# MarioCalvarro/circom_cvm

Measured on AMD Instinct MI355X. Metric: constraints simplified/sec (--O2) on 10M-constraint circuit; bit-exact .r1cs, higher is better.
Workload: dtype u64x4 (F_p, 256-bit Montgomery)

## Files before the change

### circom_cvm_amd/csrc/engine.hip

```cpp
#include <hip/hip_runtime.h>

#include <algorithm>
#include <atomic>
#include <chrono>
#include <condition_variable>
#include <cstdio>
#include <deque>
#include <mutex>
#include <map>
#include <memory>
#include <stdexcept>
#include <thread>
#include <string>
#include <unordered_map>
#include <unordered_set>
#include <functional>
#include <vector>

#include <cstring>
#include <fcntl.h>
#include <pthread.h>
#include <sched.h>
#include <unistd.h>
#include <rocprim/device/device_radix_sort.hpp>
// ... 120 lines not shown
static void launch(hipStream_t st, K kernel, uint64_t n, Args... args) {
  uint64_t blocks = (n + 255) / 256;
  if (blocks == 0) blocks = 1;
  if (blocks > 16384) blocks = 16384;
  hipLaunchKernelGGL(kernel, dim3((unsigned)blocks), dim3(256), 0, st, args...);
  HC(hipGetLastError());
}

struct KGroup {
  std::vector<hipEvent_t> ev;
  size_t n = 0;
  uint64_t bytes = 0;
  void mark(hipStream_t s) {
    if (n == ev.size()) {
      hipEvent_t e;
      HC(hipEventCreate(&e));
      ev.push_back(e);
    }
    HC(hipEventRecord(ev[n++], s));
  }
  template <class F>
  void run(hipStream_t s, uint64_t b, F &&f) {
    mark(s);
    f();
    mark(s);
    bytes += b;
  }
  void collect(double &ms, uint64_t &by, uint64_t &launches) {
    double t = 0;
    for (size_t i = 0; i + 1 < n; i += 2) {
      float m = 0;
      HC(hipEventSynchronize(ev[i + 1]));
      HC(hipEventElapsedTime(&m, ev[i], ev[i + 1]));
      t += m;
    }
    ms += t;
    by += bytes;
    launches += n ? 1 : 0;
    n = 0;
    bytes = 0;
  }
  void destroy() {
    for (hipEvent_t e : ev) (void)hipEventDestroy(e);
    ev.clear();
    n = 0;
  }
};

}
#include "comm.hpp"

using namespace rs;

enum Ev {
  kEvFill0, kEvFill1,
  kEvElim0, kEvElim1,
  kEvSmallFork,
  kEvTailPrep, kEvTailLoop,
  kEvTailEnd,
  kEvHead0, kEvHeadPrep, kEvHeadLoop, kEvHeadEnd,
  kEvHeadReady,
  kEvLane,
  kEvReplayFork, kEvReplayJoin,
  kEvNl0, kEvNl1,
  kEvCount
};
enum PinSlot {
  kPinPtr = 0,
  kPinCol = 3,
  kPinVal = 6,
  kPinL2w = 9,
  kPinWrite = 11,
  kPinLens = 13,
  kPinReplayMeta = 16,
  kPinReplayStage = 17,
  kPinRead = 18,
  kPinCluster = 19,
  kPinFlat = 20,
  kPinCount = 40
};

struct rs_engine {
  uint64_t pool_want = 0;
  int device = 0;
  uint32_t n_cu = 256;
  hipStream_t st = nullptr;
  hipStream_t srd = nullptr;
  hipStream_t st2 = nullptr;
  hipEvent_t ev[kEvCount] = {};
  Arena A;
  bool loaded = false;
  bool have_result = false;
  int fault_at = 0;
  FieldP F;
  uint64_t prime[4];
  uint32_t prime_id = 0;
  uint64_t S = 0, n_pub_out = 0, n_pub_in = 0, n_priv_in = 0;
  std::vector<uint32_t> forbidden;
  struct Blk {
    uint64_t *ptr = nullptr;
    uint32_t *key = nullptr;
    Fe *val = nullptr;
    uint64_t n = 0, nnz = 0;
  } ce, eq, lin, na, nb, nc;
  uint64_t out_n_dev = 0;
  uint64_t out_nnz[3] = {0, 0, 0};
  uint64_t n_wires = 0, npiw = 0;
  rs_stats stats{};
  std::unique_ptr<rs::Comm> comm;
  bool log_on = false;
  std::vector<uint32_t> log_from, log_key;
  std::vector<uint64_t> log_ptr, log_val;
  uint32_t *heap_k = nullptr;
  Fe *heap_v = nullptr;
  uint64_t heap_cap = 0;
  hipStream_t stc = nullptr;
  hipEvent_t ev_grp[4] = {};
  bool pending[4] = {false, false, false, false};
  int *h_vflag = nullptr;
  bool staged = false;
  const rs_input *hin = nullptr;
  unsigned long long *h_lvl = nullptr;
  hipEvent_t ev_lvl[4] = {};
  double h2d_wait_ms = 0;
  struct Pin {
    void *p = nullptr;
    size_t cap = 0;
  };
  Pin pin[kPinCount];
  rs_input flat_view{};
  rs_output view{};
  bool stream_out = false;
  bool snap_on = false;
  uint64_t snap_e[3] = {0, 0, 0};
  uint64_t out_ext[3] = {0, 0, 0};
  uint64_t nl_lo = 0, nl_hi = UINT64_MAX;
  uint64_t sh_cap[3] = {0, 0, 0};
  void *sh_ent = nullptr;
  bool sh_full = false;
  uint64_t sh_klo = 0, sh_khi = 0;
  uint64_t lc_snap_n = 0, lc_snap_base = 0;
  hipEvent_t ev_snap = nullptr, ev_snap0 = nullptr;
  uint64_t snap_cap[3] = {0, 0, 0};
  uint64_t snap_hint[3] = {0, 0, 0};
  void *snap_host[6] = {};
  struct SnapJob {
    void *dst;
    const void *src;
    size_t bytes;
    hipEvent_t ready;
  };
  hipEvent_t ev_snapq[6] = {};
  hipEvent_t ev_snaph[3] = {};
  hipEvent_t ev_fh[2] = {};
  hipEvent_t ev_nlc = nullptr;
  std::mutex snap_m;
  std::condition_variable snap_cv;
  std::deque<SnapJob> snap_q;
  bool snap_closed = true;
  std::thread snap_thread;
  cpu_set_t near_cpus;
  int near_n = 0;
  hipStream_t stx = nullptr;
  hipStream_t str = nullptr;
  hipStream_t ste = nullptr;
  hipStream_t stg = nullptr;
  hipEvent_t ev_gjoin = nullptr;
  hipEvent_t evt[2][5] = {};
  hipEvent_t evc[2] = {};
  hipEvent_t evgt[3] = {};
  hipEvent_t ev_sm[3] = {};
  hipEvent_t ev_chunk[8] = {};
  KGroup kg[3];
  int snap_rc = 0;
  bool csr_ready = false;
  DRows fin_parts[3] = {}, fin_xq[2][3] = {};
  uint64_t out_njump[3] = {0, 0, 0};
  const uint32_t *fin_keep_ids = nullptr, *fin_x_ids[2] = {nullptr, nullptr};
  uint64_t fin_keep = 0, fin_xn[2] = {0, 0}, fin_gen = 0;
};

namespace rs {

enum UpPart { kUpAll = 0, kUpKeys = 1, kUpVals = 2 };

struct RowSplit {
  std::vector<uint64_t> lo, e;
};
static RowSplit split_rows(const rs_lc &src, int W, const char *name) {
  RowSplit sp;
  const uint64_t n = src.n_rows, nnz = n ? src.nnz : 0;
  sp.lo.assign(W + 1, 0);
  sp.e.assign(W + 1, 0);
  sp.lo[W] = n;
  sp.e[W] = nnz;
  if (n && (src.ptr[0] != 0 || src.ptr[n] != nnz))
    throw RsError(RS_E_INVALID, std::string(name) + " block: bad row pointers (ptr[0] != 0 or ptr[n_rows] != nnz)");
  for (int q = 1; q < W; ++q) {
    const uint64_t want = (unsigned __int128)nnz * q / W;
    uint64_t a = sp.lo[q - 1], b = n;
    while (a < b) {
      const uint64_t m = a + (b - a) / 2;
      if (src.ptr[m] < want) a = m + 1; else b = m;
    }
    sp.lo[q] = a;
    sp.e[q] = src.ptr[a];
    if (sp.e[q] < sp.e[q - 1] || sp.e[q] > nnz)
      throw RsError(RS_E_INVALID, std::string(name) + " block: bad row pointers (decreasing)");
  }
  return sp;
}
static void upload_block(rs_engine *E, const rs_lc &src, rs_engine::Blk &dst, const char *name, int part = kUpAll) {
  if (src.n_rows && !src.ptr) throw RsError(RS_E_INVALID, std::string(name) + ": rows without a ptr array");
  if (src.nnz && (!src.col || !src.val)) throw RsError(RS_E_INVALID, std::string(name) + ": entries without col/val");
  if (src.n_rows > 0xfffffff0ull || src.nnz > (1ull << 40)) throw RsError(RS_E_INVALID, std::string(name) + ": block too large");
  dst.n = src.n_rows;
  dst.nnz = src.n_rows ? src.nnz : 0;
  std::string nm(name);
  dst.ptr = E->A.get<uint64_t>(nm + ".ptr", dst.n + 1);
  dst.key = E->A.get<uint32_t>(nm + ".key", dst.nnz);
  dst.val = E->A.get<Fe>(nm + ".val", dst.nnz);
  hipStream_t s = E->stc;
  Comm *CM = E->comm.get();
  const int W = CM ? CM->world : 1, r = CM ? CM->rank : 0;
  if (W == 1 || !dst.n) {
    if (part != kUpVals) {
      if (dst.n) HC(hipMemcpyAsync(dst.ptr, src.ptr, sizeof(uint64_t) * (dst.n + 1), hipMemcpyHostToDevice, s));
      else HC(hipMemsetAsync(dst.ptr, 0, sizeof(uint64_t), s));
      if (dst.nnz) HC(hipMemcpyAsync(dst.key, src.col, sizeof(uint32_t) * dst.nnz, hipMemcpyHostToDevice, s));
    }
    if (part != kUpKeys && dst.nnz) HC(hipMemcpyAsync(dst.val, src.val, 32 * dst.nnz, hipMemcpyHostToDevice, s));
    return;
  }
  const RowSplit sp = split_rows(src, W, name);
  const uint64_t r0 = sp.lo[r], r1 = sp.lo[r + 1] + (r == W - 1 ? 1 : 0), e0 = sp.e[r], e1 = sp.e[r + 1];
  std::vector<uint64_t> cp(W), ck(W), cv(W);
  for (int q = 0; q < W; ++q) {
    cp[q] = 8 * (sp.lo[q + 1] - sp.lo[q] + (q == W - 1 ? 1 : 0));
    ck[q] = 4 * (sp.e[q + 1] - sp.e[q]);
    cv[q] = 32 * (sp.e[q + 1] - sp.e[q]);
  }
  if (part != kUpVals) {
    if (r1 > r0) HC(hipMemcpyAsync(dst.ptr + r0, src.ptr + r0, 8 * (r1 - r0), hipMemcpyHostToDevice, s));
    if (e1 > e0) HC(hipMemcpyAsync(dst.key + e0, src.col + e0, 4 * (e1 - e0), hipMemcpyHostToDevice, s));
    CM->allgatherv(dst.ptr + r0, dst.ptr, cp, s);
    CM->allgatherv(dst.key + e0, dst.key, ck, s);
  }
  if (part != kUpKeys) {
    if (e1 > e0) HC(hipMemcpyAsync(dst.val + e0, src.val + 4 * e0, 32 * (e1 - e0), hipMemcpyHostToDevice, s));
    CM->allgatherv(dst.val + e0, dst.val, cv, s);
  }
}

static const char *kGroupName[4] = {"cons_eq/eq", "linear", "linear", "non-linear"};

static void load_enqueue(rs_engine *E, const rs_input *in, bool staged) {
  uint64_t p[4];
  if (!prime_of(in, p)) throw RsError(RS_E_INVALID, "unknown prime");
  if (in->max_signal == 0 || in->max_signal > 0x7fffffffull) throw RsError(RS_E_INVALID, "bad max_signal (label_to_wire is int32)");
  if (in->n_forbidden && !in->forbidden) throw RsError(RS_E_INVALID, "forbidden list missing");
  std::vector<uint32_t> forb(in->forbidden, in->forbidden + in->n_forbidden);
  bool has0 = false;
  for (uint32_t f : forb) {
    if (f >= in->max_signal) throw RsError(RS_E_INVALID, "forbidden signal out of range");
    has0 |= f == 0;
  }
  if (!has0) throw RsError(RS_E_INVALID, "signal 0 must be forbidden");
  if (in->nl_a.n_rows != in->nl_b.n_rows || in->nl_a.n_rows != in->nl_c.n_rows)
    throw RsError(RS_E_INVALID, "non-linear blocks differ in row count");
  HC(hipStreamSynchronize(E->stc));
  E->loaded = false;
  E->have_result = false;
  for (bool &pd : E->pending) pd = false;
  memcpy(E->prime, p, 32);
  E->prime_id = in->prime_id;
  E->F = make_field(p);
  E->S = in->max_signal;
  E->n_pub_out = in->n_pub_out;
  E->n_pub_in = in->n_pub_in;
  E->n_priv_in = in->n_priv_in;
  E->forbidden.swap(forb);
  E->h2d_wait_ms = 0;
  E->staged = staged;
  E->hin = staged ? in : nullptr;
  E->nl_lo = 0;
  E->nl_hi = UINT64_MAX;
  if (E->comm && E->comm->world > 1 && in->nl_a.n_rows) {
    const int W = E->comm->world, r = E->comm->rank;
    const rs_lc *b3[3] = {&in->nl_a, &in->nl_b, &in->nl_c};
    const uint64_t n = in->nl_a.n_rows;
    for (const rs_lc *L : b3)
      if (!L->ptr) throw RsError(RS_E_INVALID, "non-linear block: rows without a ptr array");
    auto cum = [&](uint64_t row) { return b3[0]->ptr[row] + b3[1]->ptr[row] + b3[2]->ptr[row]; };
    const uint64_t tot = cum(n);
    auto bound = [&](int q) -> uint64_t {
      if (q <= 0) return 0;
      if (q >= W) return n;
      const uint64_t want = (unsigned __int128)tot * q / W;
      uint64_t a = 0, b = n;
      while (a < b) {
        const uint64_t m = a + (b - a) / 2;
        if (cum(m) < want) a = m + 1; else b = m;
      }
      return a;
    };
    E->nl_lo = bound(r);
    E->nl_hi = std::max(E->nl_lo, bound(r + 1));
  }
  int *vf = E->A.get<int>("vflag", 10);
  HC(hipMemsetAsync(vf, 0, 40, E->stc));
  hipStream_t s = E->stc;
  KGroup &kg = E->kg[0];
  kg.n = 0;
  kg.bytes = 0;
  auto check = [&](const rs_engine::Blk &B, int g) {
    kg.run(s, 8 * (B.n + 1), [&] { launch(s, k_check_ptr, B.n + 1, (const uint64_t *)B.ptr, B.n, B.nnz, vf + 2 * g); });
  };
  auto check_keys = [&](const rs_engine::Blk &B, int pw, int ew, int *uw) {
    if (B.n)
      kg.run(s, 8 * (B.n + 1) + 4 * B.nnz, [&] {
        launch(s, k_check_keys, B.n, (const uint64_t *)B.ptr, (const uint32_t *)B.key, B.n, E->S, (const int *)(vf + pw), vf + ew, uw);
      });
  };
  auto sort_validate = [&](const rs_engine::Blk &B, int pw, int ew) {
    if (B.n)
      kg.run(s, 8 * (B.n + 1) + 36 * B.nnz, [&] {
        launch(s, k_sort_validate, B.n, E->F, (const uint64_t *)B.ptr, B.key, B.val, B.n, E->S, (const int *)(vf + pw), vf + ew);
      });
// ... 24 lines not shown
    sort_validate(E->lin, 2, 5);
    HC(hipMemcpyAsync(E->h_vflag + 4, vf + 2, 4, hipMemcpyDeviceToHost, s));
    HC(hipMemcpyAsync(E->h_vflag + 5, vf + 5, 4, hipMemcpyDeviceToHost, s));
    HC(hipEventRecord(E->ev_grp[2], s));
    E->pending[2] = true;
  } else {
    sort_validate(E->lin, 2, 3);
    E->h_vflag[8] = 0;
    verdict(1, 2);
  }
  const rs_lc *nl_src[3] = {&in->nl_a, &in->nl_b, &in->nl_c};
  rs_engine::Blk *nl_dst[3] = {&E->na, &E->nb, &E->nc};
  const char *nl_nm[3] = {"in.na", "in.nb", "in.nc"};
  for (int q = 0; q < 3; ++q) upload_block(E, *nl_src[q], *nl_dst[q], nl_nm[q]);
  for (int q = 0; q < 3; ++q) check(*nl_dst[q], 3);
  for (int q = 0; q < 3; ++q) sort_validate(*nl_dst[q], 6, 7);
  verdict(3, 2);
  E->loaded = true;
}

static void load_wait(rs_engine *E, int g) {
  if (!E->pending[g]) return;
  const double t0 = now_ms();
  HC(hipEventSynchronize(E->ev_grp[g]));
  E->pending[g] = false;
  E->h2d_wait_ms += now_ms() - t0;
  if (E->h_vflag[2 * g]) {
    E->loaded = false;
    throw RsError(RS_E_INVALID, std::string(kGroupName[g]) + " block: bad row pointers (ptr[0] != 0, decreasing, or ptr[n_rows] != nnz)");
  }
  if (E->h_vflag[2 * g + 1]) {
    E->loaded = false;
    throw RsError(RS_E_INVALID, std::string(kGroupName[g]) +
                                    " block: invalid rows (duplicate key, zero or non-canonical value, signal >= max_signal)");
  }
  HC(hipStreamWaitEvent(E->st, E->ev_grp[g], 0));
}
static void load_wait_all(rs_engine *E) {
  for (int g = 0; g < 4; ++g) load_wait(E, g);
}
static void load_order_collectives(rs_engine *E) {
  for (int g = 0; g < 4; ++g)
    if (E->pending[g]) HC(hipStreamWaitEvent(E->st, E->ev_grp[g], 0));
}
static void snap_join(rs_engine *E);
static void *pin_get(rs_engine *E, int slot, size_t bytes);
static void load_abort(rs_engine *E) {
  if (E->stc) (void)hipStreamSynchronize(E->stc);
  snap_join(E);
  for (bool &pd : E->pending) pd = false;
  if (E->comm) E->comm->fail();
}

static void rd(rs_engine *E, void *dst, const void *src, size_t bytes) {
  if (!bytes) return;
  HC(hipMemcpyAsync(dst, src, bytes, hipMemcpyDeviceToHost, E->srd));
  HC(hipStreamSynchronize(E->srd));
}
static void h2d(rs_engine *E, void *dst, const void *src, size_t bytes) {
  if (!bytes) return;
  HC(hipMemcpyAsync(dst, src, bytes, hipMemcpyHostToDevice, E->st));
  HC(hipStreamSynchronize(E->st));
}

constexpr size_t kPinRb = 128;
static uint64_t excl_scan_u64(rs_engine *E, const uint64_t *in, uint64_t *out, uint64_t n, const char *tag,
                              double *waited = nullptr) {
  if (n == 0) return 0;
  size_t tb = 0;
  HC(rocprim::exclusive_scan(nullptr, tb, in, out, (uint64_t)0, (size_t)n, rocprim::plus<uint64_t>(), E->st));
  void *tmp = E->A.get<uint8_t>(std::string("scan.tmp.") + tag, tb);
  HC(rocprim::exclusive_scan(tmp, tb, in, out, (uint64_t)0, (size_t)n, rocprim::plus<uint64_t>(), E->st));
  uint64_t *h = (uint64_t *)pin_get(E, kPinRead, kPinRb) + 4;
  HC(hipMemcpyAsync(h, in + n - 1, 8, hipMemcpyDeviceToHost, E->st));
  HC(hipMemcpyAsync(h + 1, out + n - 1, 8, hipMemcpyDeviceToHost, E->st));
  const double t0 = waited ? now_ms() : 0.0;
  HC(hipStreamSynchronize(E->st));
  if (waited) *waited += now_ms() - t0;
  return h[0] + h[1];
}

struct U3 {
  uint64_t a, b, c;
};
struct U3Plus {
  __host__ __device__ U3 operator()(const U3 &x, const U3 &y) const { return U3{x.a + y.a, x.b + y.b, x.c + y.c}; }
};
static U3 excl_scan_u3(rs_engine *E, const U3 *in, U3 *out, uint64_t n, const char *tag, const uint64_t *x_in = nullptr,
                       const uint64_t *x_out = nullptr, uint64_t *x_sum = nullptr) {
  if (n == 0 && !x_sum) return U3{0, 0, 0};
  uint64_t *h = (uint64_t *)pin_get(E, kPinRead, kPinRb) + 8;
  if (n) {
    size_t tb = 0;
    const U3 zero{0, 0, 0};
    HC(rocprim::exclusive_scan(nullptr, tb, in, out, zero, (size_t)n, U3Plus(), E->st));
    void *tmp = E->A.get<uint8_t>(std::string("scan3.tmp.") + tag, tb);
    HC(rocprim::exclusive_scan(tmp, tb, in, out, zero, (size_t)n, U3Plus(), E->st));
    HC(hipMemcpyAsync(h, in + n - 1, sizeof(U3), hipMemcpyDeviceToHost, E->st));
    HC(hipMemcpyAsync(h + 3, out + n - 1, sizeof(U3), hipMemcpyDeviceToHost, E->st));
  }
  if (x_sum) {
    HC(hipMemcpyAsync(h + 6, x_in, 8, hipMemcpyDeviceToHost, E->st));
    HC(hipMemcpyAsync(h + 7, x_out, 8, hipMemcpyDeviceToHost, E->st));
  }
  HC(hipStreamSynchronize(E->st));
  if (x_sum) *x_sum = h[6] + h[7];
  return n ? U3{h[0] + h[3], h[1] + h[4], h[2] + h[5]} : U3{0, 0, 0};
}
#include "flatten.hpp"
#include "output.hpp"
__global__ void k_pack3(const uint64_t *a, const uint64_t *b, const uint64_t *c, uint64_t n, U3 *out) {
  for (uint64_t i = gtid(); i < n; i += gstride()) out[i] = U3{a[i], b[i], c[i]};
}
__global__ void k_set_offsets_u3(const U3 *scan, uint64_t ba, uint64_t bb, uint64_t bc, uint64_t n, uint64_t *oa, uint64_t *ob,
                                 uint64_t *oc, const U3 *cap, const uint32_t *ids) {
  for (uint64_t i = gtid(); i < n; i += gstride()) {
    if (cap && cap[i].a == 0) continue;
    const uint64_t r = ids ? ids[i] : i;
    oa[r] = ba + scan[i].a;
    ob[r] = bb + scan[i].b;
    oc[r] = bc + scan[i].c;
  }
}

__global__ void k_mark_u8(const uint32_t *ids, uint64_t n, uint8_t *flag) {
  for (uint64_t i = gtid(); i < n; i += gstride()) flag[ids[i]] = 1;
}

__global__ void k_append_marks(const uint32_t *usig, const uint64_t *uoff, const uint32_t *ulen, uint64_t nU,
                               const uint32_t *pk, uint8_t *nlmap) {
  for (uint64_t i = gtid(); i < nU; i += gstride()) {
    if (!nlmap[usig[i]]) continue;
    for (uint32_t t = 0; t < ulen[i]; ++t) nlmap[pk[uoff[i] + t]] = 1;
  }
}

template <class K, class V>
static void sort_pairs(rs_engine *E, const K *kin, K *kout, const V *vin, V *vout, uint64_t n, int end_bit,
                       const char *tag, hipStream_t s = nullptr) {
  if (!n) return;
  if (!s) s = E->st;
  size_t tb = 0;
  HC(rocprim::radix_sort_pairs(nullptr, tb, kin, kout, vin, vout, (size_t)n, 0, end_bit, s));
  void *tmp = E->A.get<uint8_t>(std::string("sort.tmp.") + tag, tb);
  HC(rocprim::radix_sort_pairs(tmp, tb, kin, kout, vin, vout, (size_t)n, 0, end_bit, s));
}
static void dev_scan_u64(rs_engine *E, const uint64_t *in, uint64_t *out, uint64_t n, hipStream_t s, const char *tag) {
  if (!n) return;
  size_t tb = 0;
  HC(rocprim::exclusive_scan(nullptr, tb, in, out, (uint64_t)0, (size_t)n, rocprim::plus<uint64_t>(), s));
  void *tmp = E->A.get<uint8_t>(std::string("scan.tmp.") + tag, tb);
  HC(rocprim::exclusive_scan(tmp, tb, in, out, (uint64_t)0, (size_t)n, rocprim::plus<uint64_t>(), s));
}
static void dev_scan_u32(rs_engine *E, const uint32_t *in, uint32_t *out, uint64_t n, hipStream_t s, const char *tag) {
  if (!n) return;
  size_t tb = 0;
  HC(rocprim::exclusive_scan(nullptr, tb, in, out, (uint32_t)0, (size_t)n, rocprim::plus<uint32_t>(), s));
  void *tmp = E->A.get<uint8_t>(std::string("dscan.tmp.") + tag, tb);
  HC(rocprim::exclusive_scan(tmp, tb, in, out, (uint32_t)0, (size_t)n, rocprim::plus<uint32_t>(), s));
}

template <class K>
static void sort_keys(rs_engine *E, const K *kin, K *kout, uint64_t n, int end_bit, const char *tag) {
  if (!n) return;
  size_t tb = 0;
  HC(rocprim::radix_sort_keys(nullptr, tb, kin, kout, (size_t)n, 0, end_bit, E->st));
  void *tmp = E->A.get<uint8_t>(std::string("sortk.tmp.") + tag, tb);
  HC(rocprim::radix_sort_keys(tmp, tb, kin, kout, (size_t)n, 0, end_bit, E->st));
}

__global__ void k_u32_to_u64(const uint32_t *in, uint64_t *out, uint64_t n) {
  for (uint64_t i = gtid(); i < n; i += gstride()) out[i] = in[i];
}
__global__ void k_iota_u32(uint32_t *p, uint64_t n) {
  for (uint64_t i = gtid(); i < n; i += gstride()) p[i] = (uint32_t)i;
}
__global__ void k_make_ragged(FieldP F, const uint64_t *ptr, const uint32_t *key, const Fe *val, uint64_t n,
                              uint64_t extra, uint64_t *off, uint32_t *len, uint32_t *okey, Fe *oval) {
  for (uint64_t r = gtid(); r < n; r += gstride()) {
    uint64_t b = ptr[r], e = ptr[r + 1];
    uint64_t o = b + extra * r;
    off[r] = o;
    len[r] = (uint32_t)(e - b);
    for (uint64_t i = b; i < e; ++i) {
      okey[o + (i - b)] = key[i];
      oval[o + (i - b)] = fto_mont(F, val[i]);
    }
  }
}
__global__ void k_view_rows(const uint64_t *soff, const uint32_t *slen, const uint32_t *ids, uint64_t n,
                            uint64_t *off, uint32_t *len) {
  for (uint64_t i = gtid(); i < n; i += gstride()) {
    off[i] = soff[ids[i]];
    len[i] = slen[ids[i]];
  }
}
__global__ void k_set_offsets(const uint64_t *base_scan, uint64_t base, uint64_t *off, uint64_t n) {
  for (uint64_t i = gtid(); i < n; i += gstride()) off[i] = base + base_scan[i];
}
__global__ void k_eq_forb_info(const uint32_t *fl, uint64_t nf, const uint32_t *root, const uint8_t *in_eq, const uint32_t *cnt,
                               const uint32_t *minf, const int32_t *maxrow, uint32_t *out) {
  for (uint64_t i = gtid(); i < nf; i += gstride()) {
    const uint32_t f = fl[i], r = root[i];
    out[4 * i] = in_eq[f];
    out[4 * i + 1] = cnt[r];
    out[4 * i + 2] = minf[r];
    out[4 * i + 3] = (uint32_t)maxrow[r];
  }
}
__global__ void k_eq_bf_info(const uint32_t *bf, uint64_t n, const uint64_t *ptr, const uint32_t *key, const Fe *val,
                             const uint32_t *uf, const uint32_t *cnt, uint64_t *rec) {
  for (uint64_t q = gtid(); q < n; q += gstride()) {
    const uint32_t r = bf[q];
    const uint64_t p0 = ptr[r];
    const uint32_t k0 = key[p0], k1 = key[p0 + 1];
    uint32_t x = k0;
    while (uf[x] != x) x = uf[x];
    uint64_t *o = rec + 11 * q;
    o[0] = r;
    o[1] = ((uint64_t)k1 << 32) | k0;
    o[2] = cnt[x];
    for (int t = 0; t < 4; ++t) { o[3 + t] = val ? val[p0].l[t] : 0; o[7 + t] = val ? val[p0 + 1].l[t] : 0; }
  }
}
__global__ void k_flag_linear(const uint32_t *la, const uint32_t *lb, uint64_t n, uint64_t *flag_lin, uint64_t *flag_nl) {
  for (uint64_t i = gtid(); i < n; i += gstride()) {
    bool lin = la[i] == 0 && lb[i] == 0;
    flag_lin[i] = lin ? 1 : 0;
    flag_nl[i] = lin ? 0 : 1;
  }
}
__global__ void k_scatter_ids(const uint64_t *flag, const uint64_t *pos, uint64_t n, uint32_t *ids) {
  for (uint64_t i = gtid(); i < n; i += gstride())
    if (flag[i]) ids[pos[i]] = (uint32_t)i;
}
__global__ void k_set_rank(const uint32_t *sig, const int32_t *rank, uint64_t n, int32_t *rank_of) {
  for (uint64_t i = gtid(); i < n; i += gstride()) rank_of[sig[i]] = rank[i];
}
__global__ void k_turn_flags(const int32_t *turn, uint64_t n, uint64_t *flag) {
  for (uint64_t i = gtid(); i < n; i += gstride()) flag[i] = turn[i] >= 0 ? 1 : 0;
}
__global__ void k_commit_round(const uint8_t *touched, const int32_t *turn, uint64_t n, DRows a, DRows b, DRows c,
                               DRows oa, DRows ob, DRows oc) {
  for (uint64_t r = gtid(); r < n; r += gstride()) {
    if (!touched[r]) continue;
    if (turn[r] >= 0) {
      a.len[r] = 0;
      b.len[r] = 0;
      c.off[r] = oc.off[r];
      c.len[r] = oc.len[r];
      continue;
    }
    a.off[r] = oa.off[r]; a.len[r] = oa.len[r];
    b.off[r] = ob.off[r]; b.len[r] = ob.len[r];
    c.off[r] = oc.off[r]; c.len[r] = oc.len[r];
  }
}
__global__ void k_unmark_list(const uint32_t *sig, uint64_t n, uint8_t *bits) {
  for (uint64_t i = gtid(); i < n; i += gstride()) bits[sig[i]] = 0;
}
__global__ void k_zero_c(const uint32_t *ids, uint64_t n, uint32_t *clen) {
  for (uint64_t i = gtid(); i < n; i += gstride()) clen[ids[i]] = 0;
}
__global__ void k_nonempty_flags(const uint32_t *la, const uint32_t *lb, const uint32_t *lc, uint64_t n, uint64_t *flag) {
  for (uint64_t i = gtid(); i < n; i += gstride()) flag[i] = (la[i] | lb[i] | lc[i]) ? 1 : 0;
}

__device__ inline bool d_has_key(const uint32_t *k, uint32_t n, uint32_t s) {
  uint32_t lo = 0, hi = n;
  while (lo < hi) {
    uint32_t mid = (lo + hi) >> 1;
    if (k[mid] < s) lo = mid + 1; else hi = mid;
  }
  return lo < n && k[lo] == s;
}
__global__ void k_emit_pairs(DRows a, DRows b, DRows c, const uint8_t *flag, uint64_t *pairs, unsigned long long *cnt,
                             uint64_t cap) {
  for (uint64_t r = gtid(); r < a.n; r += gstride()) {
    const uint32_t *ka = a.key + a.off[r], *kb = b.key + b.off[r], *kc = c.key + c.off[r];
    uint32_t na = a.len[r], nb = b.len[r], nc = c.len[r];
    for (int part = 0; part < 3; ++part) {
      const uint32_t *k = part == 0 ? ka : part == 1 ? kb : kc;
      uint32_t n = part == 0 ? na : part == 1 ? nb : nc;
      for (uint32_t i = 0; i < n; ++i) {
        uint32_t s = k[i];
        if (!flag[s]) continue;
        if (part >= 1 && d_has_key(ka, na, s)) continue;
        if (part == 2 && d_has_key(kb, nb, s)) continue;
        unsigned long long o = atomicAdd(cnt, 1ull);
        if (o < cap) pairs[o] = ((uint64_t)s << 32) | (uint32_t)r;
      }
    }
  }
}

__global__ void k_sub_valid(const uint32_t *cid, const uint64_t *cl_off, const uint32_t *n_sub, uint64_t n, uint64_t *flag) {
  for (uint64_t s = gtid(); s < n; s += gstride()) {
    const uint32_t c = cid[s];
    flag[s] = s - cl_off[c] < n_sub[c] ? 1 : 0;
  }
}
__global__ void k_sub_keys(const uint32_t *cid, const uint64_t *flag, const uint64_t *pos, const uint32_t *h_sig, uint64_t n,
                           uint64_t *key, uint32_t *val) {
  for (uint64_t s = gtid(); s < n; s += gstride())
    if (flag[s]) {
      key[pos[s]] = ((uint64_t)cid[s] << 32) | h_sig[s];
      val[pos[s]] = (uint32_t)s;
    }
}
__global__ void k_sub_info(const uint64_t *key, const uint32_t *U, const uint64_t *h_off, const uint32_t *h_len, uint64_t n,
                           uint32_t *usig, uint64_t *uoff, uint32_t *ulen, int32_t *rank_of) {
  for (uint64_t i = gtid(); i < n; i += gstride()) {
    const uint32_t s = (uint32_t)key[i];
    usig[i] = s;
    uoff[i] = h_off[U[i]];
    ulen[i] = h_len[U[i]];
    rank_of[s] = (int32_t)i;
  }
}
__global__ void k_unset_rank(const uint32_t *sig, uint64_t n, int32_t *rank_of) {
  for (uint64_t i = gtid(); i < n; i += gstride()) rank_of[sig[i]] = -1;
}

__host__ __device__ inline int snake_rank(uint64_t pos, int W) {
  uint64_t p = pos % (2 * (uint64_t)W);
  return p < (uint64_t)W ? (int)p : (int)(2 * (uint64_t)W - 1 - p);
}
__global__ void k_fill_u8_ids(const uint32_t *ids, uint64_t n, uint8_t v, uint8_t *out) {
  for (uint64_t i = gtid(); i < n; i += gstride()) out[ids[i]] = v;
}
static uint64_t snake_count(uint64_t n, int W, int r) {
  uint64_t per = 2 * (uint64_t)W, k = n / per, rem = n % per;
  return 2 * k + (rem > (uint64_t)r ? 1 : 0) + (rem > per - 1 - r ? 1 : 0);
}
__global__ void k_shard_pick(const uint32_t *ids, uint64_t n_out, int W, int r, uint32_t *out) {
  const uint64_t per = 2 * (uint64_t)W;
  for (uint64_t j = gtid(); j < n_out; j += gstride())
    out[j] = ids[(j / 2) * per + ((j & 1) ? per - 1 - r : (uint64_t)r)];
}
__global__ void k_shard_owner(const uint32_t *ids, uint64_t n, int W, uint8_t *owner) {
  for (uint64_t i = gtid(); i < n; i += gstride()) owner[ids[i]] = (uint8_t)snake_rank(i, W);
}
struct XRec {
  uint32_t slot, sig, len, eoff;
};
__global__ void k_xpk_count(const uint32_t *cid, const uint64_t *cl_off, const uint8_t *owner, int r, const uint32_t *n_sub,
                            const uint32_t *n_left, const uint32_t *h_sig, const uint32_t *h_len, const uint32_t *l_len,
                            const uint8_t *need, uint64_t n_slots, uint64_t *sf, uint64_t *lf, uint64_t *se, uint64_t *le) {
  for (uint64_t s = gtid(); s < n_slots; s += gstride()) {
    const uint32_t c = cid[s];
    const uint64_t i = s - cl_off[c];
    const bool own = owner[c] == r;
    const bool is_sub = own && i < n_sub[c], is_left = own && i < n_left[c];
    sf[s] = is_sub;
    se[s] = is_sub && (!need || need[h_sig[s]]) ? h_len[s] : 0;
    lf[s] = is_left;
    le[s] = is_left ? l_len[s] : 0;
  }
}
__global__ void k_xpk_fill(const uint32_t *cid, const uint64_t *cl_off, const uint64_t *sf, const uint64_t *sp,
                           const uint64_t *se, const uint64_t *sep, const uint64_t *lf, const uint64_t *lp, const uint64_t *le,
                           const uint64_t *lep, uint64_t sub_ent, const uint32_t *h_sig, const uint64_t *h_off,
                           const uint64_t *l_off, const uint32_t *pk, const Fe *pv, uint64_t n_slots, XRec *srec, XRec *lrec,
                           uint32_t *ek, Fe *ev) {
  for (uint64_t s = gtid(); s < n_slots; s += gstride()) {
    if (sf[s]) {
      const uint64_t o = sep[s], m = se[s];
      srec[sp[s]] = XRec{(uint32_t)s, h_sig[s], (uint32_t)m, (uint32_t)o};
      for (uint64_t t = 0; t < m; ++t) { ek[o + t] = pk[h_off[s] + t]; ev[o + t] = pv[h_off[s] + t]; }
    }
    if (lf[s]) {
      const uint64_t o = sub_ent + lep[s], m = le[s];
      lrec[lp[s]] = XRec{(uint32_t)s, 0u, (uint32_t)m, (uint32_t)o};
      for (uint64_t t = 0; t < m; ++t) { ek[o + t] = pk[l_off[s] + t]; ev[o + t] = pv[l_off[s] + t]; }
    }
  }
}
__global__ void k_xunpack(const XRec *srec, uint64_t ns, const XRec *lrec, uint64_t nl, uint64_t base, const uint32_t *cid,
                          uint32_t *h_sig, uint64_t *h_off, uint32_t *h_len, uint64_t *l_off, uint32_t *l_len, uint32_t *n_sub,
                          uint32_t *n_left, int32_t *sub_of, uint8_t *deleted) {
  for (uint64_t j = gtid(); j < ns + nl; j += gstride()) {
    if (j < ns) {
      const XRec x = srec[j];
      h_sig[x.slot] = x.sig;
      h_len[x.slot] = x.len;
      h_off[x.slot] = base + x.eoff;
      sub_of[x.sig] = (int32_t)x.slot;
      deleted[x.sig] = 1;
      atomicAdd(&n_sub[cid[x.slot]], 1u);
    } else {
      const XRec x = lrec[j - ns];
      l_len[x.slot] = x.len;
      l_off[x.slot] = base + x.eoff;
      atomicAdd(&n_left[cid[x.slot]], 1u);
    }
  }
}
__global__ void k_mark_relevant(DRows R, const int32_t *eq_rep, const uint8_t *ce_has, uint8_t *need) {
  for (uint64_t r = gtid(); r < R.n; r += gstride())
    for (uint32_t i = 0; i < R.len[r]; ++i) {
      const uint32_t k = R.key[R.off[r] + i];
      const int32_t t = eq_rep[k];
      const uint32_t k1 = t >= 0 ? (uint32_t)t : k;
      if (!ce_has[k1]) need[k1] = 1;
    }
}

__global__ void k_lc_count(DRows src, const uint32_t *ids, uint64_t n, uint64_t *cnt) {
  for (uint64_t i = gtid(); i < n; i += gstride()) {
    const uint64_t r = ids ? ids[i] : i;
    const uint64_t o = src.off[r];
    uint64_t c = 0;
    for (uint32_t t = 0; t < src.len[r]; ++t) c += fe_is_zero(src.val[o + t]) ? 0 : 1;
    cnt[i] = c;
  }
}
__global__ void k_lc_copy(DRows src, const uint32_t *ids, uint64_t n, const uint64_t *pos, uint64_t base, uint64_t row0,
                          DRows lc) {
// ... 1128 lines not shown
  }
};

static void collect_leftovers(rs_engine *E, const ElimOut &eo, const Pool &P, LcHeap &lc) {
  const uint64_t n_slots = eo.n_slots, nl = eo.n_left;
  if (!nl || !n_slots) return;
  Arena &A = E->A;
  uint64_t *f = A.get<uint64_t>("lc.lf", n_slots), *fp = A.get<uint64_t>("lc.lp", n_slots);
  uint32_t *slots = A.get<uint32_t>("lc.slots", nl);
  launch(E->st, k_left_flags, n_slots, (const uint32_t *)A.get<uint32_t>("cl.cid", 1), (const uint64_t *)A.get<uint64_t>("el.cl", 1),
         (const uint32_t *)A.get<uint32_t>("el.n_left", 1), n_slots, f);
  const uint64_t m = excl_scan_u64(E, f, fp, n_slots, "lcl");
  if (m != nl) throw RsError(RS_E_INTERNAL, "leftover count mismatch");
  launch(E->st, k_scatter_ids, n_slots, (const uint64_t *)f, (const uint64_t *)fp, n_slots, slots);
  DRows src{};
  src.n = n_slots;
  src.off = A.get<uint64_t>("el.l_off", 1);
  src.len = A.get<uint32_t>("el.l_len", 1);
  src.key = P.pk;
  src.val = P.pv;
  lc.append(E, src, slots, m);
}

static void log_push(rs_engine *E, uint32_t from, const uint32_t *k, const uint64_t *v, uint64_t n) {
  E->log_from.push_back(from);
  E->log_key.insert(E->log_key.end(), k, k + n);
  E->log_val.insert(E->log_val.end(), v, v + 4 * n);
  E->log_ptr.push_back(E->log_key.size());
}
static void log_linear_round(rs_engine *E, const ElimOut &eo, const Pool &P) {
  Arena &A = E->A;
  hipStream_t st = E->st;
  const uint64_t n_slots = eo.n_slots;
  if (!n_slots) return;
  uint64_t *vf = A.get<uint64_t>("lg.vf", n_slots), *vp = A.get<uint64_t>("lg.vp", n_slots);
  const uint32_t *cid = A.get<uint32_t>("cl.cid", 1);
  launch(st, k_sub_valid, n_slots, cid, (const uint64_t *)A.get<uint64_t>("el.cl", 1),
         (const uint32_t *)A.get<uint32_t>("el.n_sub", 1), n_slots, vf);
  const uint64_t nU = excl_scan_u64(E, vf, vp, n_slots, "lgvf");
  if (!nU) return;
  uint64_t *uk = A.get<uint64_t>("lg.uk", nU), *uk2 = A.get<uint64_t>("lg.uk2", nU);
  uint32_t *uv = A.get<uint32_t>("lg.uv", nU), *U = A.get<uint32_t>("lg.U", nU);
  launch(st, k_sub_keys, n_slots, cid, (const uint64_t *)vf, (const uint64_t *)vp,
         (const uint32_t *)A.get<uint32_t>("el.h_sig", 1), n_slots, uk, uv);
  int cbits = 1;
  while (cbits < 32 && (1ull << cbits) <= eo.n_clusters) ++cbits;
  sort_pairs(E, (const uint64_t *)uk, uk2, (const uint32_t *)uv, U, nU, 32 + cbits, "lgus");
  std::vector<uint64_t> keys(nU), hoff(nU);
  std::vector<uint32_t> slots(nU), hlen(nU);
  uint64_t *d_off = A.get<uint64_t>("lg.off", nU);
  uint32_t *d_len = A.get<uint32_t>("lg.len", nU);
  launch(st, k_gather_u64, nU, (const uint64_t *)A.get<uint64_t>("el.h_off", 1), (const uint32_t *)U, d_off, nU);
  launch(st, k_gather_u32, nU, (const uint32_t *)A.get<uint32_t>("el.h_len", 1), (const uint32_t *)U, d_len, nU);
  HC(hipMemcpyAsync(keys.data(), uk2, 8 * nU, hipMemcpyDeviceToHost, st));
  HC(hipMemcpyAsync(hoff.data(), d_off, 8 * nU, hipMemcpyDeviceToHost, st));
  HC(hipMemcpyAsync(hlen.data(), d_len, 4 * nU, hipMemcpyDeviceToHost, st));
  HC(hipStreamSynchronize(st));
  std::vector<uint32_t> rk;
  std::vector<uint64_t> rv, rptr;
  fetch_pool_maps(E, hoff, hlen, P.pk, P.pv, rk, rv, rptr);
  for (uint64_t i = 0; i < nU; ++i)
    log_push(E, (uint32_t)keys[i], rk.data() + rptr[i], rv.data() + 4 * rptr[i], rptr[i + 1] - rptr[i]);
}

static void d2h_row(rs_engine *E, const DRows &R, uint64_t r, std::vector<uint32_t> &k, std::vector<Fe> &v) {
  uint64_t off = 0;
  uint32_t len = 0;
  HC(hipMemcpy(&off, R.off + r, 8, hipMemcpyDeviceToHost));
  HC(hipMemcpy(&len, R.len + r, 4, hipMemcpyDeviceToHost));
  k.resize(len);
  v.resize(len);
  if (len) {
    HC(hipMemcpy(k.data(), R.key + off, 4 * len, hipMemcpyDeviceToHost));
    HC(hipMemcpy(v.data(), R.val + off, 32 * len, hipMemcpyDeviceToHost));
  }
}
static void debug_check_round(rs_engine *E, const RoundArgs &ra, uint64_t n, uint64_t) {
  HC(hipStreamSynchronize(E->st));
  const FieldP &F = E->F;
  std::vector<uint8_t> touched(n);
  HC(hipMemcpy(touched.data(), ra.touched, n, hipMemcpyDeviceToHost));
  int shown = 0;
  for (uint64_t r = 0; r < n && shown < 3; ++r) {
    if (!touched[r]) continue;
    std::vector<uint32_t> ik[3], ok[3];
    std::vector<Fe> iv[3], ov[3];
    const DRows *in[3] = {&ra.a, &ra.b, &ra.c}, *out[3] = {&ra.oa, &ra.ob, &ra.oc};
    std::map<uint32_t, Fe> exp[3];
    for (int q = 0; q < 3; ++q) {
      d2h_row(E, *in[q], r, ik[q], iv[q]);
      d2h_row(E, *out[q], r, ok[q], ov[q]);
      for (size_t i = 0; i < ik[q].size(); ++i) {
        int32_t s = -1;
        HC(hipMemcpy(&s, ra.sub_of + ik[q][i], 4, hipMemcpyDeviceToHost));
        if (s < 0) {
          Fe &x = exp[q][ik[q][i]];
          if (!exp[q].count(ik[q][i])) x = fe_zero();
          x = fadd(F, x, iv[q][i]);
          continue;
        }
        uint64_t ho = 0;
        uint32_t hl = 0;
        HC(hipMemcpy(&ho, ra.h_off + s, 8, hipMemcpyDeviceToHost));
        HC(hipMemcpy(&hl, ra.h_len + s, 4, hipMemcpyDeviceToHost));
        std::vector<uint32_t> hk(hl);
        std::vector<Fe> hv(hl);
        HC(hipMemcpy(hk.data(), ra.pk + ho, 4 * hl, hipMemcpyDeviceToHost));
        HC(hipMemcpy(hv.data(), ra.pv + ho, 32 * hl, hipMemcpyDeviceToHost));
        for (uint32_t j = 0; j < hl; ++j) {
          auto it = exp[q].find(hk[j]);
          Fe add = fmul(F, iv[q][i], hv[j]);
          if (it == exp[q].end()) exp[q][hk[j]] = add;
          else it->second = fadd(F, it->second, add);
        }
      }
    }
    bool bad = false;
    for (int q = 0; q < 3; ++q) {
      std::vector<std::pair<uint32_t, Fe>> e;
      for (auto &kv : exp[q])
        if (!fe_is_zero(kv.second)) e.push_back(kv);
      bool same = e.size() == ok[q].size();
      for (size_t i = 0; same && i < e.size(); ++i) same = e[i].first == ok[q][i] && fe_eq(e[i].second, ov[q][i]);
      if (!same) {
        bad = true;
        fprintf(stderr, "[rs-debug] row %llu part %d: in=%zu out=%zu expected=%zu\n", (unsigned long long)r, q,
                ik[q].size(), ok[q].size(), e.size());
        for (size_t i = 0; i < ik[q].size(); ++i) {
          Fe c = ffrom_mont(F, iv[q][i]);
          fprintf(stderr, "   in  %u:%llu\n", ik[q][i], (unsigned long long)c.l[0]);
        }
        for (size_t i = 0; i < ok[q].size(); ++i) {
          Fe c = ffrom_mont(F, ov[q][i]);
          fprintf(stderr, "   out %u:%llu\n", ok[q][i], (unsigned long long)c.l[0]);
        }
        for (auto &kv : e) {
          Fe c = ffrom_mont(F, kv.second);
          fprintf(stderr, "   exp %u:%llu\n", kv.first, (unsigned long long)c.l[0]);
        }
      }
    }
    if (bad) ++shown;
  }
}

static void snap_join(rs_engine *E) {
  {
    std::lock_guard<std::mutex> lk(E->snap_m);
    E->snap_closed = true;
  }
  E->snap_cv.notify_all();
  if (E->snap_thread.joinable()) E->snap_thread.join();
  E->snap_q.clear();
}
static void snap_start(rs_engine *E);
static void snap_push(rs_engine *E, const rs_engine::SnapJob &j) {
  snap_start(E);
  {
    std::lock_guard<std::mutex> lk(E->snap_m);
    E->snap_q.push_back(j);
  }
  E->snap_cv.notify_all();
}
static void snap_start(rs_engine *E) {
  if (E->snap_thread.joinable()) return;
  E->snap_rc = 0;
  E->snap_closed = false;
  E->snap_thread = std::thread([E]() {
    static const size_t chunk = (size_t)env_u64("RS_SNAP_CHUNK_MB", 128, 1, 1ull << 20) << 20;
    static const int depth = (int)env_u64("RS_SNAP_DEPTH", 2, 1, 8);
    if (hipSetDevice(E->device) != hipSuccess) { E->snap_rc = RS_E_HIP; return; }
    int k = 0;
    double prof_ms = 0.0, prof_b = 0.0;
    for (;;) {
      rs_engine::SnapJob j;
      {
        std::unique_lock<std::mutex> lk(E->snap_m);
        E->snap_cv.wait(lk, [E] { return E->snap_closed || !E->snap_q.empty(); });
        if (E->snap_q.empty()) break;
        j = E->snap_q.front();
        E->snap_q.pop_front();
      }
      if (E->snap_rc) continue;
      if (hipEventSynchronize(j.ready) != hipSuccess) { E->snap_rc = RS_E_HIP; continue; }
      const double tj = g_prof_env ? now_ms() : 0.0;
      for (size_t o = 0; o < j.bytes; o += chunk, ++k) {
        const size_t n = std::min(chunk, j.bytes - o);
        if (k >= depth && hipEventSynchronize(E->ev_chunk[k % depth]) != hipSuccess) { E->snap_rc = RS_E_HIP; break; }
        if (hipMemcpyAsync((uint8_t *)j.dst + o, (const uint8_t *)j.src + o, n, hipMemcpyDeviceToHost, E->stx) != hipSuccess ||
            hipEventRecord(E->ev_chunk[k % depth], E->stx) != hipSuccess) {
          E->snap_rc = RS_E_HIP;
          break;
        }
      }
      if (g_prof_env) {
        if (hipStreamSynchronize(E->stx) != hipSuccess) E->snap_rc = RS_E_HIP;
        prof_ms += now_ms() - tj;
        prof_b += j.bytes;
      }
    }
    if (hipStreamSynchronize(E->stx) != hipSuccess) E->snap_rc = RS_E_HIP;
    if (g_prof_env && prof_b)
      fprintf(stderr, "[rs-prof] result stream: %.1f MB in %.2f ms of copying (%.1f GB/s)\n", prof_b / 1e6, prof_ms,
              prof_b / 1e6 / prof_ms);
  });
}

static void *pin_get(rs_engine *E, int slot, size_t bytes) {
  rs_engine::Pin &b = E->pin[slot];
  if (b.cap < bytes) {
    const size_t cap = std::max(bytes, b.cap + b.cap / 4);
    if (b.p) HC(hipHostFree(b.p));
    b.p = nullptr;
    b.cap = 0;
    HC(hipHostMalloc(&b.p, cap, hipHostMallocDefault));
    b.cap = cap;
  }
  return b.p;
}

static uint64_t sh_ent_bytes(rs_engine *E) {
  const uint64_t W = E->comm->world;
  return 36 * W * (E->sh_cap[0] + E->sh_cap[1] + E->sh_cap[2]);
}
static uint32_t *sh_col(rs_engine *E, int q) {
  const uint64_t W = E->comm->world;
  uint64_t off = 0;
  for (int p = 0; p < q; ++p) off += 4 * W * E->sh_cap[p];
  return (uint32_t *)((uint8_t *)E->sh_ent + off);
}
static uint64_t *sh_val(rs_engine *E, int q) {
  const uint64_t W = E->comm->world;
  uint64_t off = 4 * W * (E->sh_cap[0] + E->sh_cap[1] + E->sh_cap[2]);
  for (int p = 0; p < q; ++p) off += 32 * W * E->sh_cap[p];
  return (uint64_t *)((uint8_t *)E->sh_ent + off);
}

static void ensure_csr(rs_engine *E) {
  if (E->csr_ready) return;
  Arena &A = E->A;
  if (A.gen != E->fin_gen) throw RsError(RS_E_INTERNAL, "result views are stale: a buffer moved after the run");
  hipStream_t st = E->st;
  const char *nm[3] = {"out.a", "out.b", "out.c"};
  const uint64_t n_keep = E->fin_keep, n_out = E->out_n_dev;
  for (int q = 0; q < 3; ++q) {
    const uint64_t tot = E->out_nnz[q];
    const uint64_t *ptr = A.get<uint64_t>(std::string(nm[q]) + ".ptr", n_out + 1);
    uint32_t *col = A.get<uint32_t>(std::string(nm[q]) + ".col", tot);
    uint64_t *val = A.get<uint64_t>(std::string(nm[q]) + ".val", 4 * tot);
    E->kg[2].run(st, 24 * n_out + 72 * tot, [&] {
      if (n_keep) launch(st, k_gather_rows, n_keep, E->F, E->fin_parts[q], E->fin_keep_ids, n_keep, ptr, col, val);
      for (int x = 0; x < 2; ++x) {
        const uint64_t o = n_keep + (x ? E->fin_xn[0] : 0);
        if (E->fin_xn[x]) launch(st, k_gather_rows, E->fin_xn[x], E->F, E->fin_xq[x][q], E->fin_x_ids[x], E->fin_xn[x], ptr + o, col, val);
      }
    });
  }
  E->csr_ready = true;
}

#include "run.hpp"

}

namespace rs {
struct CallScope {
  rs_engine *E;
  bool ok = false;
  explicit CallScope(rs_engine *e) : E(e) {
    if (E->comm) E->comm->begin_call();
  }
  ~CallScope() {
    if (!E->comm) return;
    if (!ok) E->comm->fail();
    E->comm->end_call();
  }
};
}

extern "C" {

int rs_abi_version(void) { return RS_ABI_VERSION; }

namespace rs {
static int near_gpu_cpus(int device, cpu_set_t *want_out) {
  if (env_flag("RS_NO_CPU_BIND")) return 0;
  char bus[64] = {0};
  if (hipDeviceGetPCIBusId(bus, sizeof bus, device) != hipSuccess) return 0;
  for (char *c = bus; *c; ++c) *c = (char)tolower(*c);
  const std::string path = std::string("/sys/bus/pci/devices/") + bus + "/local_cpulist";
  FILE *f = fopen(path.c_str(), "r");
  if (!f) return 0;
  char buf[4096] = {0};
  const size_t got = fread(buf, 1, sizeof buf - 1, f);
  fclose(f);
  buf[got] = 0;
  cpu_set_t allowed, want;
  CPU_ZERO(&want);
  if (sched_getaffinity(0, sizeof allowed, &allowed) != 0) return 0;
  int n = 0;
  for (char *p = buf; *p && *p != '\n';) {
    char *e = nullptr;
    const long a = strtol(p, &e, 10);
    if (e == p) break;
    long b = a;
    p = e;
    if (*p == '-') b = strtol(p + 1, &p, 10);
    for (long c = a; c <= b && c < CPU_SETSIZE; ++c)
      if (c >= 0 && CPU_ISSET(c, &allowed)) { CPU_SET(c, &want); ++n; }
    if (*p == ',') ++p;
  }
  if (n == 0 || n == CPU_COUNT(&allowed)) return 0;
  *want_out = want;
  return n;
}
struct CpuNear {
  cpu_set_t old;
  bool set = false;
  explicit CpuNear(const rs_engine *E);
  ~CpuNear() {
    if (set) (void)pthread_setaffinity_np(pthread_self(), sizeof old, &old);
  }
};
CpuNear::CpuNear(const rs_engine *E) {
  if (!E || !E->near_n || pthread_getaffinity_np(pthread_self(), sizeof old, &old) != 0) return;
  cpu_set_t want;
  CPU_AND(&want, &old, &E->near_cpus);
  if (CPU_COUNT(&want) == 0 || CPU_EQUAL(&want, &old)) return;
  set = pthread_setaffinity_np(pthread_self(), sizeof want, &want) == 0;
}
}

int rs_engine_create(int device, rs_engine **eng) {
  try {
    int n = 0;
    if (hipGetDeviceCount(&n) != hipSuccess || n == 0) {
      set_error("no HIP device visible: librs_simplify runs only on a gfx950 GPU");
      return RS_E_NODEVICE;
    }
    if (device < 0 || device >= n) { set_error("bad device ordinal"); return RS_E_INVALID; }
    HC(hipSetDevice(device));
    hipDeviceProp_t prop;
    HC(hipGetDeviceProperties(&prop, device));
    if (std::string(prop.gcnArchName).find("gfx950") == std::string::npos) {
      set_error(std::string("device is ") + prop.gcnArchName + ", this build targets gfx950 only");
      return RS_E_NODEVICE;
    }
    std::unique_ptr<rs_engine> E(new rs_engine());
    E->device = device;
    CPU_ZERO(&E->near_cpus);
    E->near_n = near_gpu_cpus(device, &E->near_cpus);
    if (g_prof_env && E->near_n) fprintf(stderr, "[rs-prof] engine calls run on the GPU's %d local CPUs\n", E->near_n);
    E->n_cu = (uint32_t)prop.multiProcessorCount;
    const bool pooled = env_flag("RS_POOLED_STREAMS"), all_masked = env_flag("RS_CUMASK_STREAMS");
    std::vector<uint32_t> cu_mask((E->n_cu + 31) / 32, 0u);
    for (uint32_t c = 0; c < E->n_cu; ++c) cu_mask[c / 32] |= 1u << (c % 32);
    auto mk_stream = [&](hipStream_t *sp, bool dedicated) {
      if (pooled || !dedicated || hipExtStreamCreateWithCUMask(sp, (uint32_t)cu_mask.size(), cu_mask.data()) != hipSuccess)
        HC(hipStreamCreateWithFlags(sp, hipStreamNonBlocking));
    };
    mk_stream(&E->st, all_masked);
    HC(hipStreamCreateWithFlags(&E->srd, hipStreamNonBlocking));
    {
      int lo = 0, hi = 0;
      if (hipDeviceGetStreamPriorityRange(&lo, &hi) != hipSuccess ||
          hipStreamCreateWithPriority(&E->st2, hipStreamNonBlocking, hi) != hipSuccess)
        HC(hipStreamCreateWithFlags(&E->st2, hipStreamNonBlocking));
    }
    mk_stream(&E->stc, true);
    mk_stream(&E->stx, all_masked);
    mk_stream(&E->str, all_masked);
    {
      int lo = 0, hi = 0;
      if (env_flag("RS_STE_DEFAULT") || hipDeviceGetStreamPriorityRange(&lo, &hi) != hipSuccess ||
          hipStreamCreateWithPriority(&E->ste, hipStreamNonBlocking, lo) != hipSuccess)
        HC(hipStreamCreateWithFlags(&E->ste, hipStreamNonBlocking));
      if (g_prof_env) fprintf(stderr, "[rs-prof] stream priorities: least %d greatest %d\n", lo, hi);
    }
    mk_stream(&E->stg, all_masked);
    HC(hipEventCreateWithFlags(&E->ev_gjoin, hipEventDisableTiming));
    for (auto &g : E->evt)
      for (auto &ev : g) HC(hipEventCreate(&ev));
    for (auto &ev : E->evc) HC(hipEventCreate(&ev));
    for (auto &ev : E->evgt) HC(hipEventCreate(&ev));
    for (auto &ev : E->ev_sm) HC(hipEventCreate(&ev));
    for (auto &ev : E->ev) HC(hipEventCreate(&ev));
    for (auto &ev : E->ev_grp) HC(hipEventCreateWithFlags(&ev, hipEventDisableTiming));
    HC(hipHostMalloc((void **)&E->h_vflag, 10 * sizeof(int), hipHostMallocDefault));
    memset(E->h_vflag, 0, 10 * sizeof(int));
    HC(hipHostMalloc((void **)&E->h_lvl, 8 * sizeof(unsigned long long), hipHostMallocDefault));
    for (auto &ev : E->ev_lvl) HC(hipEventCreateWithFlags(&ev, hipEventDisableTiming));
    HC(hipEventCreateWithFlags(&E->ev_snap, hipEventDisableTiming));
    HC(hipEventCreateWithFlags(&E->ev_snap0, hipEventDisableTiming));
    for (auto &ev : E->ev_chunk) HC(hipEventCreateWithFlags(&ev, hipEventDisableTiming));
    for (auto &ev : E->ev_snapq) HC(hipEventCreateWithFlags(&ev, hipEventDisableTiming));
    for (auto &ev : E->ev_snaph) HC(hipEventCreateWithFlags(&ev, hipEventDisableTiming));
    for (auto &ev : E->ev_fh) HC(hipEventCreate(&ev));
// ... 768 lines not shown
```

### circom_cvm_amd/csrc/kernels.hpp

```cpp
#pragma once
#include <hip/hip_runtime.h>

#include "field.hpp"

namespace rs {

#define RS_NONE 0xffffffffu
constexpr uint64_t kProfWords = 24;

struct DRows {
  uint64_t *off;
  uint32_t *len;
  uint32_t *key;
  Fe *val;
  uint64_t n;
};

__device__ __forceinline__ uint64_t gtid() { return (uint64_t)blockIdx.x * blockDim.x + threadIdx.x; }
__device__ __forceinline__ uint64_t gstride() { return (uint64_t)gridDim.x * blockDim.x; }
__device__ __forceinline__ void wave_atomic_add(unsigned long long *p, unsigned long long x) {
#pragma unroll
  for (int d = 32; d >= 1; d >>= 1) x += __shfl_xor(x, d);
  if ((threadIdx.x & 63) == 0 && x) atomicAdd(p, x);
}
// ... 3154 lines not shown
  return fr;
}

__global__ void k_round_fill(RoundArgs A) {
  const FieldP &F = A.F;
  unsigned long long bytes = 0;
  const uint64_t n = A.rlist ? *A.n_rlist : A.n_ids;
  for (uint64_t i = gtid(); i < n; i += gstride()) {
    const uint64_t r = A.rlist ? A.rlist[i] : A.ids[i];
    A.touched[r] = 1;
    const FrameArgs fr = d_round_frames(A);
    uint64_t oa = A.oa.off[r], ob = A.ob.off[r], oc = A.oc.off[r];
    uint32_t capa = (uint32_t)A.cap_a[r], capb = (uint32_t)A.cap_b[r], capc = (uint32_t)A.cap_c[r];
    uint32_t mx = capa > capb ? capa : capb;
    uint32_t cc = (capc - mx) / 2;
    uint32_t na, nb;
    if (A.pre_expanded) {
      na = A.oa.len[r];
      nb = A.ob.len[r];
    } else {
      na = d_apply_frames(fr, A.a.key + A.a.off[r], A.a.val + A.a.off[r], A.a.len[r], A.oa.key + oa, A.oa.val + oa, capa);
      nb = d_apply_frames(fr, A.b.key + A.b.off[r], A.b.val + A.b.off[r], A.b.len[r], A.ob.key + ob, A.ob.val + ob, capb);
    }
    if (d_const_or_empty(A.oa.key + oa, na) || d_const_or_empty(A.ob.key + ob, nb)) {
      d_round_turn(A, r);
      na = d_apply_frames(fr, A.a.key + A.a.off[r], A.a.val + A.a.off[r], A.a.len[r], A.oa.key + oa, A.oa.val + oa, capa);
      nb = d_apply_frames(fr, A.b.key + A.b.off[r], A.b.val + A.b.off[r], A.b.len[r], A.ob.key + ob, A.ob.val + ob, capb);
    }
    uint32_t nc = A.pre_expanded ? A.oc.len[r]
                                       : d_apply_frames(fr, A.c.key + A.c.off[r], A.c.val + A.c.off[r], A.c.len[r], A.oc.key + oc,
                                                        A.oc.val + oc, cc);
    d_fix(F, A.oa.key + oa, A.oa.val + oa, na, A.ob.key + ob, A.ob.val + ob, nb, A.oc.key + oc, A.oc.val + oc, nc,
          A.oc.key + oc + cc, A.oc.val + oc + cc);
    A.oa.len[r] = na;
    A.ob.len[r] = nb;
    A.oc.len[r] = nc;
    bytes += 36ull * ((capa - 1) + (capb - 1) + (cc - 1) - A.a.len[r] - A.b.len[r] - A.c.len[r]) +
             36ull * (na + nb + nc);
  }
  wave_atomic_add(A.bytes, bytes);
}

__device__ __forceinline__ const DRows &d_part(const RoundArgs &A, uint32_t p) { return p == 0 ? A.a : (p == 1 ? A.b : A.c); }
__global__ void k_xrow_count(RoundArgs A, uint64_t nseg, uint64_t *cnt) {
  for (uint64_t sg = gtid(); sg < nseg; sg += gstride()) {
    const uint64_t r = A.rlist[sg / 3];
    const DRows &P = d_part(A, (uint32_t)(sg % 3));
    uint64_t c = 0;
    for (uint32_t i = 0; i < P.len[r]; ++i) {
      const int32_t s = A.sub_of[P.key[P.off[r] + i]];
      c += s >= 0 ? A.h_len[s] : 1;
    }
    cnt[sg] = c;
  }
}
__global__ __launch_bounds__(256) void k_xrow_expand(RoundArgs A, uint64_t nseg, const uint64_t *soff, uint64_t *xk, Fe *xv,
                                                     uint32_t *xi) {
  const FieldP &F = A.F;
  const uint32_t lane = threadIdx.x & 63;
  for (uint64_t sg = gtid() >> 6; sg < nseg; sg += gstride() >> 6) {
    const uint64_t r = A.rlist[sg / 3];
    const DRows &P = d_part(A, (uint32_t)(sg % 3));
    const uint64_t ro = P.off[r];
    const uint32_t n = P.len[r];
    uint64_t base = soff[sg];
    for (uint32_t c0 = 0; c0 < n; c0 += 64) {
      const uint32_t i = c0 + lane;
      uint32_t k = 0, m = 0;
      int32_t s = -1;
      if (i < n) {
        k = P.key[ro + i];
        s = A.sub_of[k];
        m = s >= 0 ? A.h_len[s] : 1;
      }
      uint32_t x = m;
#pragma unroll
      for (int d = 1; d < 64; d <<= 1) {
        const uint32_t y = __shfl_up(x, d);
        if (lane >= (uint32_t)d) x += y;
      }
      const uint64_t o = base + x - m;
      if (i < n) {
        const Fe vv = P.val[ro + i];
        if (s < 0) {
          xk[o] = ((uint64_t)sg << 32) | k;
          xv[o] = vv;
          xi[o] = (uint32_t)(o - soff[sg]);
        } else {
          const uint64_t hb = A.h_off[s];
          for (uint32_t t = 0; t < m; ++t) {
            xk[o + t] = ((uint64_t)sg << 32) | A.pk[hb + t];
            xv[o + t] = fmul(F, vv, A.pv[hb + t]);
            xi[o + t] = (uint32_t)(o + t - soff[sg]);
          }
        }
      }
      base += __shfl(x, 63);
    }
  }
}
__global__ __launch_bounds__(256) void k_xrow_combine(RoundArgs A, uint64_t nseg, const uint64_t *soff, const uint64_t *xk,
                                                      const uint32_t *xi, const Fe *xv) {
  const FieldP &F = A.F;
  const uint32_t lane = threadIdx.x & 63;
  for (uint64_t sg = gtid() >> 6; sg < nseg; sg += gstride() >> 6) {
    const uint64_t r = A.rlist[sg / 3];
    const uint32_t p = (uint32_t)(sg % 3);
    const DRows &O = p == 0 ? A.oa : (p == 1 ? A.ob : A.oc);
    uint32_t *ok = O.key + O.off[r];
    Fe *ov = O.val + O.off[r];
    const uint64_t b = soff[sg], e = soff[sg + 1];
    uint32_t w = 0;
    for (uint64_t q0 = b; q0 < e; q0 += 64) {
      const uint64_t q = q0 + lane;
      bool keep = false;
      uint32_t key = 0;
      Fe sum = fe_zero();
      if (q < e) {
        key = (uint32_t)xk[q];
        if (q == b || (uint32_t)xk[q - 1] != key) {
          sum = xv[b + xi[q]];
          for (uint64_t t = q + 1; t < e && (uint32_t)xk[t] == key; ++t) sum = fadd(F, sum, xv[b + xi[t]]);
          keep = !fe_is_zero(sum);
        }
      }
      const uint64_t km = __ballot(keep);
      if (keep) {
        const uint32_t at = w + (uint32_t)__popcll(km & ((1ull << lane) - 1ull));
        ok[at] = key;
        ov[at] = sum;
      }
      w += (uint32_t)__popcll(km);
    }
    if (lane == 0) {
      if (p == 0) A.oa.len[r] = w;
      else if (p == 1) A.ob.len[r] = w;
      else A.oc.len[r] = w;
    }
  }
}

__global__ void k_round_turn(RoundArgs A) {
  const uint64_t n = *A.n_rlist;
  for (uint64_t i = gtid(); i < n; i += gstride()) d_round_turn(A, A.rlist[i]);
}

__global__ void k_mark_keys(DRows R, uint8_t *bits) {
  for (uint64_t r = gtid(); r < R.n; r += gstride())
    for (uint32_t i = 0; i < R.len[r]; ++i) bits[R.key[R.off[r] + i]] = 1;
}
__global__ void k_mark_list(const uint32_t *sig, uint64_t n, uint8_t *bits) {
  for (uint64_t i = gtid(); i < n; i += gstride()) bits[sig[i]] = 1;
}
__global__ void k_kept(const uint8_t *deleted, const uint8_t *forb, const uint8_t *nlmap, uint32_t *kept, uint64_t S) {
  for (uint64_t s = gtid(); s < S; s += gstride()) kept[s] = (!deleted[s] && (forb[s] || nlmap[s])) ? 1u : 0u;
}
__global__ void k_l2w(const uint32_t *kept, const uint64_t *rank, int32_t *l2w, uint64_t S) {
  for (uint64_t s = gtid(); s < S; s += gstride()) l2w[s] = kept[s] ? (int32_t)rank[s] : -1;
}
__global__ void k_gather_rows(FieldP F, DRows R, const uint32_t *ids, uint64_t n, const uint64_t *optr,
                              uint32_t *ocol, uint64_t *oval) {
  for (uint64_t i = gtid(); i < n; i += gstride()) {
    uint32_t r = ids[i];
    uint64_t o = optr[i];
    for (uint32_t t = 0; t < R.len[r]; ++t) {
      ocol[o + t] = R.key[R.off[r] + t];
      Fe c = ffrom_mont(F, R.val[R.off[r] + t]);
      oval[4 * (o + t) + 0] = c.l[0];
      oval[4 * (o + t) + 1] = c.l[1];
      oval[4 * (o + t) + 2] = c.l[2];
      oval[4 * (o + t) + 3] = c.l[3];
    }
  }
}
__global__ void k_row_lens(DRows R, const uint32_t *ids, uint64_t n, uint64_t *lens) {
  for (uint64_t i = gtid(); i < n; i += gstride()) lens[i] = R.len[ids[i]];
}
__global__ void k_pool_to_canon(FieldP F, const uint64_t *off, const uint32_t *len, const uint64_t *optr, uint64_t n,
                                const uint32_t *pk, const Fe *pv, uint32_t *ok, uint64_t *ov) {
  for (uint64_t i = gtid(); i < n; i += gstride()) {
    uint64_t o = optr[i];
    for (uint32_t t = 0; t < len[i]; ++t) {
      ok[o + t] = pk[off[i] + t];
      Fe c = ffrom_mont(F, pv[off[i] + t]);
      for (int q = 0; q < 4; ++q) ov[4 * (o + t) + q] = c.l[q];
    }
  }
}

__global__ __launch_bounds__(256) void k_pool_keys(const uint64_t *off, const uint32_t *len, const uint64_t *optr, uint64_t n,
                                                   const uint32_t *pk, uint32_t *ok) {
  const uint32_t lane = threadIdx.x & 63;
  for (uint64_t i = gtid() >> 6; i < n; i += gstride() >> 6) {
    const uint64_t o = optr[i], b = off[i];
    for (uint32_t t = lane; t < len[i]; t += 64) ok[o + t] = pk[b + t];
  }
}

__global__ void k_eq_log_keys(const int32_t *eq_rep, uint32_t *uf, const uint32_t *cnt, const int32_t *maxrow, uint64_t S,
                              uint64_t *key, uint32_t *rep, unsigned long long *n) {
  for (uint64_t s = gtid(); s < S; s += gstride()) {
    const int32_t r = eq_rep[s];
    if (r < 0) continue;
    const uint32_t root = uf_find(uf, (uint32_t)s);
    const unsigned long long i = atomicAdd(n, 1ull);
    key[i] = ((uint64_t)(cnt[root] > 1) << 63) | ((uint64_t)(uint32_t)maxrow[root] << 32) | s;
    rep[i] = (uint32_t)r;
  }
}
__global__ void k_const_log(FieldP F, DRows R, const uint8_t *forb, uint32_t *sig, uint64_t *val) {
  for (uint64_t r = gtid(); r < R.n; r += gstride()) {
    const uint32_t *k = R.key + R.off[r];
    const Fe *v = R.val + R.off[r];
    const uint32_t n = R.len[r];
    const uint32_t s = n ? k[n - 1] : 0;
    sig[r] = (n == 0 || forb[s]) ? RS_NONE : s;
    Fe x = fe_zero();
    if (n && !forb[s] && n == 2 && k[0] == 0) x = ffrom_mont(F, fmul(F, v[0], finv(F, fneg(F, v[n - 1]))));
    for (int q = 0; q < 4; ++q) val[4 * r + q] = x.l[q];
  }
}

}
```

### circom_cvm_amd/csrc/output.hpp

```cpp
#pragma once

__device__ __forceinline__ uint64_t u3_sel(const U3 &x, int q) { return q == 0 ? x.a : (q == 1 ? x.b : x.c); }

struct ViewCopy {
  uint64_t *off[3];
  uint32_t *len[3];
};
__device__ __forceinline__ void view_copy(const ViewCopy &v, const DRows &a, const DRows &b, const DRows &c, uint64_t i,
                                          uint32_t la, uint32_t lb, uint32_t lc) {
  v.off[0][i] = a.off[i];
  v.off[1][i] = b.off[i];
  v.off[2][i] = c.off[i];
  v.len[0][i] = la;
  v.len[1][i] = lb;
  v.len[2][i] = lc;
}

__global__ void k_snap_flags(DRows a, DRows b, DRows c, const uint64_t *late, uint64_t n, uint64_t lo, uint64_t hi, uint8_t *early,
                             U3 *elen, ViewCopy vc) {
  for (uint64_t i = gtid(); i < n; i += gstride()) {
    const bool done = (!late || !late[i]) && i >= lo && i < hi;
    const uint32_t la = done ? a.len[i] : 0, lb = done ? b.len[i] : 0, lc = done ? c.len[i] : 0;
    const bool ok = (la | lb) != 0;
    early[i] = ok ? 1 : 0;
    elen[i] = ok ? U3{la, lb, lc} : U3{0, 0, 0};
    if (ok) view_copy(vc, a, b, c, i, la, lb, lc);
  }
}

__global__ void k_snap_lens2(DRows a, DRows b, DRows c, const uint64_t *late, uint64_t n, U3 *elen, ViewCopy vc) {
  for (uint64_t i = gtid(); i < n; i += gstride()) {
    const bool ok = late[i] && (a.len[i] | b.len[i]) != 0;
    elen[i] = ok ? U3{a.len[i], b.len[i], c.len[i]} : U3{0, 0, 0};
    if (ok) view_copy(vc, a, b, c, i, a.len[i], b.len[i], c.len[i]);
  }
}
__global__ void k_snap_mark2(const uint64_t *late, const U3 *elen, const U3 *eoff2, U3 base, uint64_t n, uint8_t *early,
                             U3 *eoff) {
  for (uint64_t i = gtid(); i < n; i += gstride()) {
    if (!late[i] || (elen[i].a | elen[i].b) == 0) continue;
    early[i] = 1;
    eoff[i] = U3{base.a + eoff2[i].a, base.b + eoff2[i].b, base.c + eoff2[i].c};
  }
}

__global__ void k_snap_lens_rng(DRows a, DRows b, DRows c, const uint64_t *late, uint64_t lo, uint64_t hi, uint64_t n, U3 *elen,
                                ViewCopy vc) {
  for (uint64_t i = gtid(); i < n; i += gstride()) {
    const bool ok = i >= lo && i < hi && !(late && late[i]) && (a.len[i] | b.len[i]) != 0;
    elen[i] = ok ? U3{a.len[i], b.len[i], c.len[i]} : U3{0, 0, 0};
    if (ok) view_copy(vc, a, b, c, i, a.len[i], b.len[i], c.len[i]);
  }
}
__global__ void k_snap_mark_sel(const U3 *elen, const U3 *eoff2, U3 base, uint64_t n, uint8_t *early, U3 *eoff) {
  for (uint64_t i = gtid(); i < n; i += gstride()) {
    if ((elen[i].a | elen[i].b) == 0) continue;
    early[i] = 1;
    eoff[i] = U3{base.a + eoff2[i].a, base.b + eoff2[i].b, base.c + eoff2[i].c};
  }
}

__global__ void k_snap_gather(FieldP F, DRows R, const uint8_t *early, const U3 *eoff, int q, uint64_t n, uint32_t *col,
                              uint64_t *val, const uint64_t *only, uint64_t lo) {
  for (uint64_t r = lo + gtid(); r < n; r += gstride()) {
    if (!early[r] || (only && !only[r])) continue;
    const uint64_t o = u3_sel(eoff[r], q), s = R.off[r];
    const uint32_t len = R.len[r];
    for (uint32_t t = 0; t < len; ++t) {
      col[o + t] = R.key[s + t];
      const Fe c = ffrom_mont(F, R.val[s + t]);
      val[4 * (o + t) + 0] = c.l[0];
      val[4 * (o + t) + 1] = c.l[1];
      val[4 * (o + t) + 2] = c.l[2];
      val[4 * (o + t) + 3] = c.l[3];
    }
  }
}

__global__ void k_snap_lens_round(DRows a, DRows b, DRows c, const uint8_t *touched, const int32_t *turn, const uint32_t *nl_of,
                                  const uint8_t *early, uint64_t n, U3 *elen, ViewCopy vc) {
  for (uint64_t r = gtid(); r < n; r += gstride()) {
    const bool ok = (touched[r] || !early[nl_of[r]]) && turn[r] < 0 && (a.len[r] | b.len[r]) != 0;
    elen[r] = ok ? U3{a.len[r], b.len[r], c.len[r]} : U3{0, 0, 0};
    if (ok) view_copy(vc, a, b, c, r, a.len[r], b.len[r], c.len[r]);
  }
}
__global__ void k_snap_mark_round(const uint32_t *nl_of, const U3 *elen, const U3 *eoff3, U3 base, uint64_t n, uint8_t *early,
                                  U3 *eoff, uint8_t *dirty) {
  for (uint64_t r = gtid(); r < n; r += gstride()) {
    if ((elen[r].a | elen[r].b) == 0) continue;
    const uint32_t i = nl_of[r];
    early[i] = 1;
    eoff[i] = U3{base.a + eoff3[r].a, base.b + eoff3[r].b, base.c + eoff3[r].c};
    dirty[r] = 0;
  }
}
__global__ void k_snap_gather_st(FieldP F, DRows R, const U3 *elen, const U3 *eoff3, uint64_t base, int q, uint64_t n,
                                 uint32_t *col, uint64_t *val) {
  for (uint64_t r = gtid(); r < n; r += gstride()) {
    if ((elen[r].a | elen[r].b) == 0) continue;
    const uint64_t o = base + u3_sel(eoff3[r], q), s = R.off[r];
    const uint32_t len = R.len[r];
    for (uint32_t t = 0; t < len; ++t) {
      col[o + t] = R.key[s + t];
      const Fe c = ffrom_mont(F, R.val[s + t]);
      val[4 * (o + t) + 0] = c.l[0];
      val[4 * (o + t) + 1] = c.l[1];
      val[4 * (o + t) + 2] = c.l[2];
      val[4 * (o + t) + 3] = c.l[3];
    }
  }
}

__global__ void k_or_u8(const uint8_t *x, uint64_t n, uint8_t *acc) {
  for (uint64_t i = gtid(); i < n; i += gstride())
    if (x[i]) acc[i] = 1;
}

__device__ __forceinline__ bool d_reused(const uint8_t *early, const uint8_t *dirty, const uint32_t *nl_of, uint32_t r) {
  return early && early[nl_of[r]] && !dirty[r];
}

__global__ void k_out_late_lens(DRows R, const uint32_t *ids, uint64_t n, const uint32_t *nl_of, const uint8_t *early,
                                const uint8_t *dirty, uint64_t *late) {
  for (uint64_t i = gtid(); i < n; i += gstride()) {
    const uint32_t r = ids[i];
    late[i] = d_reused(early, dirty, nl_of, r) ? 0 : R.len[r];
  }
}

__global__ void k_out_extent(DRows R, const uint32_t *ids, uint64_t n, const uint32_t *nl_of, const uint8_t *early,
                             const uint8_t *dirty, const U3 *eoff, int q, uint64_t base, const uint64_t *lptr, uint64_t *beg,
                             uint64_t *end) {
  for (uint64_t i = gtid(); i < n; i += gstride()) {
    const uint32_t r = ids[i];
    const uint64_t b = d_reused(early, dirty, nl_of, r) ? u3_sel(eoff[nl_of[r]], q) : base + lptr[i];
    beg[i] = b;
    end[i] = b + R.len[r];
  }
}

__global__ void k_lc_late_lens(DRows R, const uint32_t *ids, uint64_t n, uint64_t n_snap, uint64_t *late) {
  for (uint64_t i = gtid(); i < n; i += gstride()) {
    const uint32_t r = ids[i];
    late[i] = r < n_snap ? 0 : R.len[r];
  }
}
__global__ void k_lc_extent(DRows R, const uint32_t *ids, uint64_t n, uint64_t n_snap, uint64_t c_base, int q, uint64_t base,
                            const uint64_t *lptr, uint64_t *beg, uint64_t *end) {
  for (uint64_t i = gtid(); i < n; i += gstride()) {
    const uint32_t r = ids[i];
    const uint64_t b = r < n_snap && q == 2 ? c_base + R.off[r] : base + lptr[i];
    beg[i] = b;
    end[i] = b + R.len[r];
  }
}
__global__ void k_lc_gather_late(FieldP F, DRows R, const uint32_t *ids, uint64_t n, uint64_t n_snap, const uint64_t *lptr,
                                 uint32_t *col, uint64_t *val) {
  for (uint64_t i = gtid(); i < n; i += gstride()) {
    const uint32_t r = ids[i];
    if (r < n_snap) continue;
    const uint64_t o = lptr[i], s = R.off[r];
    for (uint32_t t = 0; t < R.len[r]; ++t) {
      col[o + t] = R.key[s + t];
      const Fe c = ffrom_mont(F, R.val[s + t]);
      val[4 * (o + t) + 0] = c.l[0];
      val[4 * (o + t) + 1] = c.l[1];
      val[4 * (o + t) + 2] = c.l[2];
      val[4 * (o + t) + 3] = c.l[3];
    }
  }
}
__global__ void k_lc_snap(FieldP F, const uint32_t *key, const Fe *v, uint64_t n, uint32_t *col, uint64_t *val) {
  for (uint64_t t = gtid(); t < n; t += gstride()) {
    col[t] = key[t];
    const Fe c = ffrom_mont(F, v[t]);
    val[4 * t + 0] = c.l[0];
    val[4 * t + 1] = c.l[1];
    val[4 * t + 2] = c.l[2];
    val[4 * t + 3] = c.l[3];
  }
}

__global__ void k_gather_late(FieldP F, DRows R, const uint32_t *ids, uint64_t n, const uint32_t *nl_of, const uint8_t *early,
                              const uint8_t *dirty, const uint64_t *lptr, uint32_t *col, uint64_t *val) {
  for (uint64_t i = gtid(); i < n; i += gstride()) {
    const uint32_t r = ids[i];
    if (d_reused(early, dirty, nl_of, r)) continue;
    const uint64_t o = lptr[i], s = R.off[r];
    const uint32_t len = R.len[r];
    for (uint32_t t = 0; t < len; ++t) {
      col[o + t] = R.key[s + t];
      const Fe c = ffrom_mont(F, R.val[s + t]);
      val[4 * (o + t) + 0] = c.l[0];
      val[4 * (o + t) + 1] = c.l[1];
      val[4 * (o + t) + 2] = c.l[2];
      val[4 * (o + t) + 3] = c.l[3];
    }
  }
}

__global__ void k_to_host(const uint4 *src, uint4 *dst, uint64_t n16) {
  for (uint64_t i = gtid(); i < n16; i += gstride()) dst[i] = src[i];
}

__global__ void k_set_u64(uint64_t *p, uint64_t v) {
  if (gtid() == 0) *p = v;
}

__global__ void k_keep_range(const uint32_t *keep, uint64_t n_keep, const uint32_t *nl_of, uint64_t lo, uint64_t hi, uint64_t *out) {
  const uint64_t t = gtid();
  if (t >= 2) return;
  const uint64_t bound = t ? hi : lo;
  uint64_t a = 0, b = n_keep;
  while (a < b) {
    const uint64_t m = (a + b) / 2;
    if (nl_of[keep[m]] < bound) a = m + 1; else b = m;
  }
  out[t] = a;
}
__global__ void k_add_u64(const uint64_t *in, uint64_t n, uint64_t add, uint64_t *out) {
  for (uint64_t i = gtid(); i < n; i += gstride()) out[i] = in[i] + add;
}

__global__ void k_out_jumps(const uint64_t *beg, const uint64_t *end, uint64_t m, int first_jump, uint32_t *len, uint64_t *jf) {
  for (uint64_t i = gtid(); i < m; i += gstride()) {
    const uint64_t b = beg[i], l = end[i] - b;
    const bool j = i == 0 ? (first_jump || b != 0) : b != end[i - 1];
    len[i] = (uint32_t)l | (j ? RS_ROW_JUMP : 0u);
    jf[i] = j ? 1 : 0;
  }
}
__global__ void k_out_jtab(const uint64_t *beg, const uint64_t *jf, const uint64_t *jpos, uint64_t m, uint64_t add, uint64_t *jtab) {
  for (uint64_t i = gtid(); i < m; i += gstride())
    if (jf[i]) jtab[jpos[i]] = beg[i] + add;
}
```

### circom_cvm_amd/csrc/run.hpp

```cpp
#pragma once

static std::string part_name(const char *pre, int q, const char *suf) { return std::string(pre) + "abc"[q] + suf; }

struct Run {
  rs_engine *const E;
  const rs_flags *const fl;
  Arena &A;
  const hipStream_t st;
  const uint64_t S;
  KGroup &kg1;
  const bool apply_linear;
  uint64_t no_rounds;
  double T0 = 0, Tf = 0;
  int *d_err = nullptr;
  uint8_t *d_forb = nullptr, *d_deleted = nullptr;
  int32_t *sub_of = nullptr, *eq_rep = nullptr;
  uint8_t *ce_has = nullptr;
  Fe *ce_val = nullptr;
  LcHeap lc;
  DRows ce{}, lin{};
  bool keys_first = false;
  uint8_t *lin_fixed = nullptr;
  const uint64_t n_nl;
  DRows nl_in[3] = {};
// ... 361 lines not shown
  void mk_in(rs_engine::Blk &B, DRows &R, const char *nm, hipStream_t ms) {
    R.n = B.n;
    R.off = A.get<uint64_t>(std::string(nm) + ".off", R.n);
    R.len = A.get<uint32_t>(std::string(nm) + ".len", R.n);
    R.key = A.get<uint32_t>(std::string(nm) + ".key", B.nnz);
    R.val = A.get<Fe>(std::string(nm) + ".val", B.nnz);
    if (R.n)
      kg1.run(ms, 72 * B.nnz + 20 * R.n + 8, [&] {
        launch(ms, k_make_ragged, R.n, E->F, (const uint64_t *)B.ptr, (const uint32_t *)B.key, (const Fe *)B.val, R.n, (uint64_t)0,
               R.off, R.len, R.key, R.val);
      });
  }
  void stage_nl() {
    if (nl_staged) return;
    load_wait(E, 3);
    static const bool on_main = env_flag("RS_NLC_MAIN");
    hipStream_t cs = on_main ? st : E->stc;
    rs_engine::Blk *blk[3] = {&E->na, &E->nb, &E->nc};
    const char *nm[3] = {"nla", "nlb", "nlc"};
    for (int q = 0; q < 3; ++q) mk_in(*blk[q], nl_in[q], nm[q], cs);
    HC(hipEventRecord(E->ev_nlc, cs));
    HC(hipStreamWaitEvent(st, E->ev_nlc, 0));
    nl_staged = true;
  }
  void heap_reserve(uint64_t need) {
    if (heap_top + need <= E->heap_cap && E->heap_k) return;
    uint64_t ncap = std::max<uint64_t>(heap_top + need + (heap_top + need) / 16, E->heap_cap + E->heap_cap / 4);
    ncap = std::max<uint64_t>(ncap, 1 << 16);
    uint32_t *nk = nullptr;
    Fe *nv = nullptr;
    HC(hipStreamSynchronize(st));
    HC(hipMalloc((void **)&nk, 4 * ncap));
    HC(hipMalloc((void **)&nv, 32 * ncap));
    if (heap_top) {
      HC(hipMemcpyAsync(nk, E->heap_k, 4 * heap_top, hipMemcpyDeviceToDevice, st));
      HC(hipMemcpyAsync(nv, E->heap_v, 32 * heap_top, hipMemcpyDeviceToDevice, st));
      HC(hipStreamSynchronize(st));
    }
    if (E->snap_on) HC(hipStreamSynchronize(E->stc));
    if (E->heap_k) { HC(hipFree(E->heap_k)); HC(hipFree(E->heap_v)); }
    E->heap_k = heap_k = nk;
    E->heap_v = heap_v = nv;
    E->heap_cap = ncap;
  }

  void setup_non_linear() {
    heap_top = 0;
    heap_k = E->heap_k;
    heap_v = E->heap_v;
    d_bytes = A.get<unsigned long long>("nl.bytes", 1);
    HC(hipMemsetAsync(d_bytes, 0, 8, st));
    d_fw_err = A.get<int>("fw.err", 1);
    HC(hipMemsetAsync(d_fw_err, 0, 4, st));
    fr.F = E->F;
    fr.eq_rep = eq_rep;
    fr.ce_has = ce_has;
    fr.ce_val = ce_val;
    fr.sub_of = sub_of;
    for (int q = 0; q < 3; ++q) {
      stor[q].n = n_nl;
      stor[q].off = A.get<uint64_t>(part_name("st.", q, ".off"), n_nl);
      stor[q].len = A.get<uint32_t>(part_name("st.", q, ".len"), n_nl);
    }
    if (n_nl) {
      for (int q = 0; q < 3; ++q) cap[q] = A.get<uint64_t>(part_name("nl.cap", q, ""), n_nl);
      cap3 = A.get<U3>("nl.c3", n_nl); sc3 = A.get<U3>("nl.s3", n_nl);
    }
  }

  void snap_views(const DRows (&src)[3], const char *pre, DRows (&cp)[3], ViewCopy &vc) {
    for (int q = 0; q < 3; ++q) {
      cp[q] = src[q];
      cp[q].off = vc.off[q] = A.get<uint64_t>(part_name(pre, q, ".off"), src[q].n);
      cp[q].len = vc.len[q] = A.get<uint32_t>(part_name(pre, q, ".len"), src[q].n);
    }
  }
  template <class G>
  void snap_tail(const uint64_t n[3], hipEvent_t *evs, const char *what, const char *when, G &&gather) {
    for (int q = 0; q < 3; ++q) {
      const uint64_t b = E->snap_e[q];
      const std::string xn = std::string("out.") + "abc"[q];
      uint32_t *col = A.get<uint32_t>(xn + ".xcol", 1);
      uint64_t *val = A.get<uint64_t>(xn + ".xval", 1);
      if (!n[q]) continue;
      gather(q, col, val, b);
      HC(hipEventRecord(evs[q], E->stc));
      snap_push(E, {(uint32_t *)E->snap_host[2 * q] + b, col + b, 4 * n[q], evs[q]});
      snap_push(E, {(uint64_t *)E->snap_host[2 * q + 1] + 4 * b, val + 4 * b, 32 * n[q], evs[q]});
      E->snap_e[q] = b + n[q];
    }
    HC(hipEventRecord(E->ev_snap, E->stc));
    if (g_prof_env)
      fprintf(stderr, "[rs-prof] stream: %s %llu / %llu / %llu entries (%.1f MB)%s\n", what, (unsigned long long)n[0],
              (unsigned long long)n[1], (unsigned long long)n[2], 36e-6 * (n[0] + n[1] + n[2]), when);
  }
  void snap_take(const uint64_t *late, uint64_t hi_rows) {
    if (!E->stream_out || !n_nl) return;
    so_early = A.get<uint8_t>("so.early", n_nl);
    so_eoff = A.get<U3>("so.eoff", n_nl);
    U3 *elen = A.get<U3>("so.elen", n_nl);
    Comm *CM = E->comm.get();
    const bool shard = CM && CM->world > 1;
    DRows cp[3];
    ViewCopy vc;
    snap_views(stor, "so.", cp, vc);
    launch(st, k_snap_flags, n_nl, stor[0], stor[1], stor[2], late, n_nl, shard ? E->nl_lo : (uint64_t)0, shard ? E->nl_hi : hi_rows, so_early, elen,
           vc);
    const U3 et = excl_scan_u3(E, elen, so_eoff, n_nl, "so");
    E->lc_snap_n = shard ? 0 : lc.n;
    E->lc_snap_base = et.c;
    const uint64_t lc_e = shard ? 0 : lc.top;
    const uint64_t ev[3] = {et.a, et.b, et.c + lc_e};
    E->sh_full = false;
    if (shard) {
      for (int q = 0; q < 3; ++q) E->sh_cap[q] = CM->max_u64(std::max<uint64_t>(ev[q] + ev[q] / 4 + 65536, E->sh_cap[q]), st);
      E->sh_ent = CM->shared_host(0, sh_ent_bytes(E), st);
      if (!E->sh_ent) {
        if (g_prof_env) fprintf(stderr, "[rs-prof] no shared host memory: unstreamed per-rank result\n");
        E->stream_out = false;
        return;
      }
    }
    HC(hipEventRecord(E->ev_snap0, st));
    HC(hipStreamWaitEvent(E->stc, E->ev_snap0, 0));
    for (int q = 0; q < 3; ++q) {
      E->snap_e[q] = 0;
      E->snap_hint[q] = std::max(E->snap_hint[q], ev[q]);
      const uint64_t est = hi_rows < n_nl && hi_rows ? (uint64_t)((double)ev[q] * n_nl / hi_rows) : ev[q];
      const uint64_t cap = std::max<uint64_t>(est + std::max<uint64_t>(est / 4, 1 << 16), E->snap_hint[q]);
      const std::string xn = std::string("out.") + "abc"[q];
      (void)A.get<uint32_t>(xn + ".xcol", cap);
      (void)A.get<uint64_t>(xn + ".xval", 4 * cap);
      E->snap_cap[q] = cap;
      E->snap_host[2 * q] = shard ? (void *)(sh_col(E, q) + CM->rank * E->sh_cap[q]) : pin_get(E, kPinCol + q, 4 * cap);
      E->snap_host[2 * q + 1] = shard ? (void *)(sh_val(E, q) + 4 * CM->rank * E->sh_cap[q]) : pin_get(E, kPinVal + q, 32 * cap);
    }
    snap_tail(ev, E->ev_snapq, "early region", late ? " after the first pass" : "", [&](int q, uint32_t *col, uint64_t *val, uint64_t) {
      E->kg[2].run(E->stc, 13 * n_nl + 72 * ev[q], [&] {
        launch(E->stc, k_snap_gather, n_nl, E->F, cp[q], (const uint8_t *)so_early, (const U3 *)so_eoff, q, n_nl, col, val,
               (const uint64_t *)nullptr, (uint64_t)0);
      });
      if (q == 2 && lc_e) {
        const DRows lcv = lc.view(A);
        E->kg[2].run(E->stc, 72 * lc_e, [&] {
          launch(E->stc, k_lc_snap, lc_e, E->F, (const uint32_t *)lcv.key, (const Fe *)lcv.val, lc_e, col + et.c, val + 4 * et.c);
        });
      }
    });
    E->snap_on = true;
  }
  void snap_take2() {
    if (!E->snap_on || !nl_late || !n_late || (E->comm && E->comm->world > 1)) return;
    HC(hipStreamWaitEvent(st, E->ev_snap, 0));
    U3 *elen = A.get<U3>("so.elen", n_nl), *eoff2 = A.get<U3>("so.eoff2", n_nl);
    DRows cp[3];
    ViewCopy vc;
    snap_views(stor, "so2.", cp, vc);
    launch(st, k_snap_lens2, n_nl, stor[0], stor[1], stor[2], (const uint64_t *)nl_late, n_nl, elen, vc);
    const U3 et = excl_scan_u3(E, elen, eoff2, n_nl, "so2");
    const uint64_t e2[3] = {et.a, et.b, et.c};
    for (int q = 0; q < 3; ++q) E->snap_hint[q] = std::max(E->snap_hint[q], E->snap_e[q] + e2[q]);
    for (int q = 0; q < 3; ++q)
      if (E->snap_e[q] + e2[q] > E->snap_cap[q]) return;
    launch(st, k_snap_mark2, n_nl, (const uint64_t *)nl_late, (const U3 *)elen, (const U3 *)eoff2,
           U3{E->snap_e[0], E->snap_e[1], E->snap_e[2]}, n_nl, so_early, so_eoff);
    HC(hipEventRecord(E->ev_snap0, st));
    HC(hipStreamWaitEvent(E->stc, E->ev_snap0, 0));
    snap_tail(e2, E->ev_snapq + 3, "second snapshot", "", [&](int q, uint32_t *col, uint64_t *val, uint64_t) {
      E->kg[2].run(E->stc, 21 * n_nl + 72 * e2[q], [&] {
        launch(E->stc, k_snap_gather, n_nl, E->F, cp[q], (const uint8_t *)so_early, (const U3 *)so_eoff, q, n_nl, col, val,
               (const uint64_t *)nl_late, (uint64_t)0);
      });
    });
  }
  void snap_take_h2(uint64_t h) {
    if (!E->snap_on || (E->comm && E->comm->world > 1)) return;
    HC(hipStreamWaitEvent(st, E->ev_snap, 0));
    U3 *elen = A.get<U3>("so.elenh", n_nl), *eoffh = A.get<U3>("so.eoffh", n_nl);
    DRows cp[3];
    ViewCopy vc;
    snap_views(stor, "soh.", cp, vc);
    launch(st, k_snap_lens_rng, n_nl, stor[0], stor[1], stor[2], (const uint64_t *)nl_late, h, n_nl, n_nl, elen, vc);
    const U3 et = excl_scan_u3(E, elen, eoffh, n_nl, "soh");
    const uint64_t e2[3] = {et.a, et.b, et.c};
    for (int q = 0; q < 3; ++q) E->snap_hint[q] = std::max(E->snap_hint[q], E->snap_e[q] + e2[q]);
    for (int q = 0; q < 3; ++q)
      if (E->snap_e[q] + e2[q] > E->snap_cap[q]) return;
    launch(st, k_snap_mark_sel, n_nl, (const U3 *)elen, (const U3 *)eoffh, U3{E->snap_e[0], E->snap_e[1], E->snap_e[2]}, n_nl,
           so_early, so_eoff);
    HC(hipEventRecord(E->ev_snap0, st));
    HC(hipStreamWaitEvent(E->stc, E->ev_snap0, 0));
    snap_tail(e2, E->ev_snaph, "the first pass's second half", "", [&](int q, uint32_t *col, uint64_t *val, uint64_t) {
      E->kg[2].run(E->stc, 13 * (n_nl - h) + 72 * e2[q], [&] {
        launch(E->stc, k_snap_gather, n_nl - h, E->F, cp[q], (const uint8_t *)so_early, (const U3 *)so_eoff, q, n_nl, col, val,
               (const uint64_t *)nullptr, h);
      });
    });
  }
  void nl_phase(int phase, const uint32_t *ids, uint64_t n, hipEvent_t e0, hipEvent_t e1, uint64_t split = ~0ull,
                const std::function<void()> &between = {}) {
    stage_nl();
    NLArgs a{};
    a.fr = fr;
    a.a = nl_in[0]; a.b = nl_in[1]; a.c = nl_in[2];
    a.cap_a = cap[0]; a.cap_b = cap[1]; a.cap_c = cap[2];
    a.bytes = d_bytes;
    a.ids = ids;
    a.n = n;
    a.phase = phase;
    a.hmark = hmark;
    a.late = nl_late;
    launch(st, k_nl_count, n, a);
    const bool lists = phase == 1 && n_nl;
    if (lists) {
      dev_scan_u64(E, nl_late, nl_lpos, n_nl, st, "nll");
      launch(st, k_scatter_ids, n_nl, (const uint64_t *)nl_late, (const uint64_t *)nl_lpos, n_nl, nl_lids);
    }
    launch(st, k_pack3, n, (const uint64_t *)cap[0], (const uint64_t *)cap[1], (const uint64_t *)cap[2], n, cap3);
    const U3 t3 = lists ? excl_scan_u3(E, cap3, sc3, n, "nl", nl_late + n_nl - 1, nl_lpos + n_nl - 1, &n_late)
                        : excl_scan_u3(E, cap3, sc3, n, "nl");
    if (g_prof_env) fprintf(stderr, "[rs-prof] nl phase %d: %llu rows, %llu heap entries\n", phase, (unsigned long long)n,
                            (unsigned long long)(t3.a + t3.b + t3.c));
    heap_reserve(t3.a + t3.b + t3.c);
    launch(st, k_set_offsets_u3, n, (const U3 *)sc3, heap_top, heap_top + t3.a, heap_top + t3.a + t3.b, n, stor[0].off, stor[1].off,
           stor[2].off, phase == 1 ? (const U3 *)cap3 : nullptr, ids);
    heap_top += t3.a + t3.b + t3.c;
    for (DRows &R : stor) { R.key = heap_k; R.val = heap_v; }
    a.oa = stor[0]; a.ob = stor[1]; a.oc = stor[2];
    FrameWaveArgs w{};
    w.fr = fr;
    for (int q = 0; q < 3; ++q) { w.in[q] = nl_in[q]; w.out[q] = stor[q]; w.cap[q] = cap[q]; }
    w.ids = ids;
    w.n = n;
    w.late = phase == 1 ? nl_late : nullptr;
    w.big = A.get<uint32_t>(phase == 1 ? "nl.big1" : "nl.big2", n);
    w.n_big = A.get<unsigned>(phase == 1 ? "nl.nbig1" : "nl.nbig2", 1);
    w.err = d_fw_err;
    w.bytes = d_bytes;
    HC(hipMemsetAsync(w.n_big, 0, 4, st));
#ifdef RS_FWCLK
    w.clk = A.get<unsigned long long>(phase == 1 ? "fw.clk1" : "fw.clk2", 32 + 8 * 64);
    HC(hipMemsetAsync(w.clk, 0, 8 * (32 + 8 * 64), st));
#endif
    a.xlist = w.big;
    a.n_xlist = w.n_big;
    HC(hipEventRecord(e0, st));
    fh_split = split < n;
    if (fh_split) {
      w.n = split;
      launch_capped(st, k_frames_wave<0>, split, kFwBlocks, w);
      launch(st, k_nl_fill, n, a);
      HC(hipEventRecord(E->ev_fh[0], st));
      between();
      HC(hipMemsetAsync(w.n_big, 0, 4, st));
      HC(hipEventRecord(E->ev_fh[1], st));
      w.x0 = split;
      w.n = n;
      launch_capped(st, k_frames_wave<0>, n - split, kFwBlocks, w);
    } else {
      launch_capped(st, k_frames_wave<0>, n, kFwBlocks, w);
    }
    launch(st, k_nl_fill, n, a);
    HC(hipEventRecord(e1, st));
    if (g_prof_env) {
      unsigned nb = 0;
      HC(hipMemcpyAsync(&nb, w.n_big, 4, hipMemcpyDeviceToHost, st));
      HC(hipStreamSynchronize(st));
      fprintf(stderr, "[rs-prof] nl phase %d: %u rows over a wave batch\n", phase, nb);
      if (w.clk) {
        unsigned long long c[32 + 8 * 64];
        HC(hipMemcpy(c, w.clk, sizeof c, hipMemcpyDeviceToHost));
        fprintf(stderr, "[rs-prof] frames clocks (Mcycles summed over waves): groups %.1f entries %.1f terms %.1f rank %.1f "
                "heads %.1f emit %.1f rows %.1f plan %.1f | batches %llu, wave total %.1f over %llu waves\n",
                c[0] / 1e6, c[1] / 1e6, c[2] / 1e6, c[3] / 1e6, c[4] / 1e6, c[5] / 1e6, c[6] / 1e6, c[7] / 1e6, c[8],
                c[9] / 1e6, c[10]);
        fprintf(stderr, "[rs-prof] frames fallbacks: A const %llu, B const %llu | emit: loads %.1f values %.1f sync %.1f stores %.1f\n",
                c[12], c[13], c[16] / 1e6, c[17] / 1e6, c[18] / 1e6, c[19] / 1e6);
      }
    }
    E->stats.apply_kernel_launches++;
  }
  void nl_ms(hipEvent_t e0, hipEvent_t e1) {
    float ms = 0;
    HC(hipEventSynchronize(e1));
    if (fh_split) {
      float m2 = 0;
      HC(hipEventElapsedTime(&ms, e0, E->ev_fh[0]));
      HC(hipEventElapsedTime(&m2, E->ev_fh[1], e1));
      ms += m2;
      fh_split = false;
    } else {
      HC(hipEventElapsedTime(&ms, e0, e1));
    }
    E->stats.apply_kernel_ms += ms;
  }
  void head_overlap(const uint32_t *ids, uint64_t n_head, const ElimArgs &ea) {
    hmark = A.get<uint8_t>("nl.hmark", E->S);
    nl_late = A.get<uint64_t>("nl.late", n_nl);
    nl_lpos = A.get<uint64_t>("nl.lpos", n_nl);
    nl_lids = A.get<uint32_t>("nl.lids", n_nl);
    HC(hipMemsetAsync(hmark, 0, E->S, st));
    hipLaunchKernelGGL(k_mark_head_keys, dim3(16, (unsigned)n_head), dim3(256), 0, st, ea.rows, (const uint32_t *)ea.perm,
                       (const uint64_t *)ea.cl_off, ids, hmark);
    HC(hipGetLastError());
    fr.h_off = ea.h_off; fr.h_len = ea.h_len; fr.pk = ea.pk; fr.pv = ea.pv;
    const bool halves = E->stream_out && !(E->comm && E->comm->world > 1) &&
                        n_nl >= env_u64("RS_HALVES_MIN", 1ull << 20, 0, UINT64_MAX) && !env_flag("RS_NO_HALVES");
    const double frac = env_f64("RS_HALF_FRAC", 0.5, 0.0, 1.0);
    const uint64_t h = halves ? std::max<uint64_t>(1, std::min<uint64_t>(n_nl - 1, (uint64_t)(n_nl * frac))) : n_nl;
    nl_phase(1, nullptr, n_nl, E->ev[kEvNl0], E->ev[kEvNl1], h, [&] { snap_take(nl_late, h); });
    if (!halves) snap_take(nl_late, n_nl);
    else snap_take_h2(h);
    nl_split = true;
  }

  void linear_round1() {
    P = get_pool(E, 1 << 20);
    const HeadOverlap overlap = [this](const uint32_t *ids, uint64_t n_head, const ElimArgs &ea) { head_overlap(ids, n_head, ea); };
    const std::function<void()> values = [this] { linear_values(); };
    if (apply_linear) {
      uint8_t *relevant = nullptr;
      if (E->comm && E->comm->world > 1 && !E->log_on) {
        relevant = A.get<uint8_t>("x.relevant", S);
        HC(hipMemsetAsync(relevant, 0, S, st));
        if (n_nl) {
          stage_nl();
          for (const DRows &R : nl_in)
            launch(st, k_mark_relevant, R.n, R,(const int32_t *)eq_rep, (const uint8_t *)ce_has, relevant);
        }
      }
      if (E->comm && E->comm->world > 1) load_order_collectives(E);
      run_linear_simplification(E, lin, fl->use_old_heuristics, eo, P, d_err, d_forb, sub_of, d_deleted,
                                n_nl ? &overlap : nullptr, keys_first ? &values : nullptr, relevant);
      if (E->log_on) log_linear_round(E, eo, P);
      collect_leftovers(E, eo, P, lc);
      E->stats.rounds++;
    } else {
      if (!keys_first) lc.append(E, lin, nullptr, lin.n);
      else throw RsError(RS_E_INTERNAL, "--O1 with keys-first linear rows");
    }
  }

  void non_linear_frames() {
    double Ts = now_ms();
    fr.h_off = A.get<uint64_t>("el.h_off", 1);
    fr.h_len = A.get<uint32_t>("el.h_len", 1);
    fr.pk = P.pk;
    fr.pv = P.pv;
    if (n_nl) {
      if (nl_split) nl_ms(E->ev[kEvNl0], E->ev[kEvNl1]);
      if (!nl_split) {
        nl_phase(0, nullptr, n_nl, E->ev[kEvFill0], E->ev[kEvFill1]);
        snap_take(nullptr, n_nl);
        nl_ms(E->ev[kEvFill0], E->ev[kEvFill1]);
      } else if (n_late) {
        nl_phase(2, nl_lids, n_late, E->ev[kEvFill0], E->ev[kEvFill1]);
        snap_take2();
        nl_ms(E->ev[kEvFill0], E->ev[kEvFill1]);
      }
    }
    unsigned long long bytes = 0;
    HC(hipMemcpyAsync(&bytes, d_bytes, 8, hipMemcpyDeviceToHost, st));
    st_ids = A.get<uint32_t>("st.ids", n_nl);
    wl_ids = A.get<uint32_t>("wl.ids", n_nl);
    if (n_nl) {
      uint64_t *fl_lin = A.get<uint64_t>("fl.lin", n_nl), *fl_nl = A.get<uint64_t>("fl.nl", n_nl);
      uint64_t *p_lin = A.get<uint64_t>("fl.plin", n_nl), *p_nl = A.get<uint64_t>("fl.pnl", n_nl);
      launch(st, k_flag_linear, n_nl, (const uint32_t *)stor[0].len, (const uint32_t *)stor[1].len, n_nl, fl_lin, fl_nl);
      n_wl = excl_scan_u64(E, fl_lin, p_lin, n_nl, "fl");
      n_st = excl_scan_u64(E, fl_nl, p_nl, n_nl, "fn");
      launch(st, k_scatter_ids, n_nl, (const uint64_t *)fl_lin, (const uint64_t *)p_lin, n_nl, wl_ids);
      launch(st, k_scatter_ids, n_nl, (const uint64_t *)fl_nl, (const uint64_t *)p_nl, n_nl, st_ids);
    }
    HC(hipStreamSynchronize(st));
    E->stats.apply_bytes += bytes;
    if (no_rounds > 0) no_rounds--;

    for (int q = 0; q < 3; ++q) {
      sv[q].n = n_st;
      sv[q].key = heap_k;
      sv[q].val = heap_v;
      sv[q].off = A.get<uint64_t>(part_name("sv.", q, ".off"), n_st);
      sv[q].len = A.get<uint32_t>(part_name("sv.", q, ".len"), n_st);
    }
    if (n_st)
      for (int q = 0; q < 3; ++q)
        launch(st, k_view_rows, n_st, (const uint64_t *)stor[q].off, (const uint32_t *)stor[q].len, (const uint32_t *)st_ids, n_st,
               sv[q].off, sv[q].len);
    nlmap = A.get<uint8_t>("nlmap", S);
    HC(hipMemsetAsync(nlmap, 0, S, st));
    if (n_st)
      for (const DRows &R : sv) launch(st, k_mark_keys, n_st, R, nlmap);
    lv.n = n_wl;
    lv.key = heap_k;
    lv.val = heap_v;
    lv.off = A.get<uint64_t>("lv.off", n_wl);
    lv.len = A.get<uint32_t>("lv.len", n_wl);
    if (n_wl) launch(st, k_view_rows, n_wl, (const uint64_t *)stor[2].off, (const uint32_t *)stor[2].len, (const uint32_t *)wl_ids, n_wl, lv.off, lv.len);
    HC(hipStreamSynchronize(st));
    E->stats.subst_ms += now_ms() - Ts;
    E->stats.nl_ms += now_ms() - Ts;
  }

  void snap_round(const uint8_t *touched, const int32_t *turn) {
    if (!so_dirty || !n_st || (E->comm && E->comm->world > 1)) return;
    HC(hipStreamWaitEvent(st, E->ev_snap, 0));
    U3 *elen = A.get<U3>("so.rlen", n_st), *eoff3 = A.get<U3>("so.roff", n_st);
    DRows cp[3];
    ViewCopy vc;
    snap_views(sv, "sor.", cp, vc);
    launch(st, k_snap_lens_round, n_st, sv[0], sv[1], sv[2], touched, turn, (const uint32_t *)st_ids, (const uint8_t *)so_early, n_st, elen, vc);
    const U3 et = excl_scan_u3(E, elen, eoff3, n_st, "sor");
    const uint64_t e3[3] = {et.a, et.b, et.c};
    if (!(e3[0] | e3[1] | e3[2])) return;
    for (int q = 0; q < 3; ++q) E->snap_hint[q] = std::max(E->snap_hint[q], E->snap_e[q] + e3[q]);
    for (int q = 0; q < 3; ++q)
      if (E->snap_e[q] + e3[q] > E->snap_cap[q]) return;
    launch(st, k_snap_mark_round, n_st, (const uint32_t *)st_ids, (const U3 *)elen, (const U3 *)eoff3,
           U3{E->snap_e[0], E->snap_e[1], E->snap_e[2]}, n_st, so_early, so_eoff, so_dirty);
    HC(hipEventRecord(E->ev_snap0, st));
    HC(hipStreamWaitEvent(E->stc, E->ev_snap0, 0));
    snap_tail(e3, E->ev_snapq + 3, "round snapshot", "", [&](int q, uint32_t *col, uint64_t *val, uint64_t b) {
      E->kg[2].run(E->stc, 24 * n_st + 72 * e3[q], [&] {
        launch(E->stc, k_snap_gather_st, n_st, E->F, cp[q], (const U3 *)elen, (const U3 *)eoff3, b, q, n_st, col, val);
      });
    });
  }

  void rounds() {
    apply_round = apply_linear && no_rounds > 0 && n_wl > 0;
    if (so_early) {
      so_dirty = A.get<uint8_t>("so.dirty", n_st ? n_st : 1);
      if (n_st) HC(hipMemsetAsync(so_dirty, 0, n_st, st));
    }
    if (env_flag("RS_DEBUG")) {
      HC(hipStreamSynchronize(st));
      fprintf(stderr, "[rs-debug] heap %p cap %llu top %llu n_st %llu n_wl %llu\n", (void *)heap_k,
              (unsigned long long)E->heap_cap, (unsigned long long)heap_top, (unsigned long long)n_st, (unsigned long long)n_wl);
      for (uint64_t r = 0; r < std::min<uint64_t>(n_st, 3); ++r) {
        uint64_t o = 0; uint32_t l = 0;
        HC(hipMemcpy(&o, sv[2].off + r, 8, hipMemcpyDeviceToHost));
        HC(hipMemcpy(&l, sv[2].len + r, 4, hipMemcpyDeviceToHost));
        std::vector<uint32_t> kk; std::vector<Fe> vv;
        d2h_row(E, sv[2], r, kk, vv);
        fprintf(stderr, "[rs-debug]  st %llu C off %llu len %u:", (unsigned long long)r, (unsigned long long)o, l);
        for (size_t i = 0; i < kk.size(); ++i) fprintf(stderr, " %u:%llu", kk[i], (unsigned long long)ffrom_mont(E->F, vv[i]).l[0]);
        fprintf(stderr, "\n");
      }
    }
    if (apply_round) {
      double Tm = now_ms();
      for (int q = 0; q < 3; ++q) {
        m0[q] = sv[q];
        m0[q].off = A.get<uint64_t>(part_name("m0.", q, ".off"), n_st);
        m0[q].len = A.get<uint32_t>(part_name("m0.", q, ".len"), n_st);
      }
      if (n_st)
        for (int q = 0; q < 3; ++q) {
          HC(hipMemcpyAsync(m0[q].off, sv[q].off, 8 * n_st, hipMemcpyDeviceToDevice, st));
          HC(hipMemcpyAsync(m0[q].len, sv[q].len, 4 * n_st, hipMemcpyDeviceToDevice, st));
        }
      qflag = A.get<uint8_t>("m.qflag", S);
      HC(hipMemsetAsync(qflag, 0, S, st));
      E->stats.subst_ms += now_ms() - Tm;
      E->stats.map_ms += now_ms() - Tm;
      rank_of = A.get<int32_t>("rank_of", S);
      HC(hipMemsetAsync(rank_of, 0xff, 4 * S, st));
      r_sub_of = A.get<int32_t>("r.sub_of", S);
      HC(hipMemsetAsync(r_sub_of, 0xff, 4 * S, st));
      while (apply_round) round_once();
    }
  }
  void query_initial(const std::vector<uint32_t> &sigs) {
    auto &minit = ML.minit;
    std::vector<uint32_t> q;
    for (uint32_t s : sigs)
      if (!minit.count(s)) { minit[s]; q.push_back(s); }
    if (q.empty() || n_st == 0) return;
    uint32_t *d_q = A.get<uint32_t>("m.q", q.size());
    h2d(E, d_q, q.data(), 4 * q.size());
    launch(st, k_mark_list, q.size(), (const uint32_t *)d_q, (uint64_t)q.size(), qflag);
    unsigned long long *d_cnt = A.get<unsigned long long>("m.cnt", 1);
    uint64_t cap = std::max<uint64_t>(4 * q.size(), 1 << 16);
    for (;;) {
      uint64_t *d_pairs = A.get<uint64_t>("m.pairs", cap);
      HC(hipMemsetAsync(d_cnt, 0, 8, st));
      for (DRows &R : m0) { R.key = heap_k; R.val = heap_v; }
      launch(st, k_emit_pairs, n_st, m0[0], m0[1], m0[2], (const uint8_t *)qflag, d_pairs, d_cnt, cap);
      unsigned long long cnt = 0;
      HC(hipMemcpyAsync(&cnt, d_cnt, 8, hipMemcpyDeviceToHost, st));
      HC(hipStreamSynchronize(st));
      if (cnt > cap) { cap = cnt; continue; }
      std::vector<uint64_t> pairs(cnt);
      if (cnt) {
        HC(hipMemcpyAsync(pairs.data(), d_pairs, 8 * cnt, hipMemcpyDeviceToHost, st));
        HC(hipStreamSynchronize(st));
      }
      std::sort(pairs.begin(), pairs.end());
      for (uint64_t x : pairs) minit[(uint32_t)(x >> 32)].push_back((uint32_t)x);
      break;
    }
    launch(st, k_unmark_list, q.size(), (const uint32_t *)d_q, (uint64_t)q.size(), qflag);
  }
  void need_usig() {
    if (usig.size() == nU) return;
    usig.resize(nU);
    HC(hipMemcpyAsync(usig.data(), d_us, 4 * nU, hipMemcpyDeviceToHost, st));
    HC(hipStreamSynchronize(st));
  }

  void round_once() {
    er = ElimOut{};
    MK = Marks{};
    nU = 0;
    usig.clear();
    turned.clear();
    HC(hipMemsetAsync(r_sub_of, 0xff, 4 * S, st));
    run_linear_simplification(E, lv, fl->use_old_heuristics, er, P, d_err, d_forb, r_sub_of, d_deleted, nullptr, nullptr,
                              E->comm && E->comm->world > 1 && !E->log_on ? nlmap : nullptr);
    if (E->log_on) log_linear_round(E, er, P);
    E->stats.rounds++;
    MK.st = st;
    MK.mark("start");
    collect_leftovers(E, er, P, lc);
    MK.mark("leftovers");
    const double Tr = now_ms();
    round_order();
    MK.mark("order");
    if (n_st && nU) round_apply();
    MK.mark("appends");
    const uint64_t nn = round_next();
    MK.mark("next");
    MK.dump();
    if (g_prof_env) fprintf(stderr, "[rs-prof] round: nU %llu n_st %llu next %llu\n", (unsigned long long)nU, (unsigned long long)n_st, (unsigned long long)nn);
    E->stats.subst_ms += now_ms() - Tr;
    E->stats.rounds_ms += now_ms() - Tr;
    if (no_rounds > 0) no_rounds--;
    apply_round = nn > 0 && no_rounds > 0;
  }
  void round_order() {
    const uint64_t n_slots = er.n_slots;
    d_us = A.get<uint32_t>("r.us", 1);
    uint32_t *d_U = A.get<uint32_t>("r.U", 1);
    d_ulen = A.get<uint32_t>("r.ulen", 1);
    d_uoff = A.get<uint64_t>("r.uoff", 1);
    if (n_slots) {
      uint64_t *vf = A.get<uint64_t>("r.vf", n_slots), *vp = A.get<uint64_t>("r.vp", n_slots);
      launch(st, k_sub_valid, n_slots, (const uint32_t *)A.get<uint32_t>("cl.cid", 1), (const uint64_t *)A.get<uint64_t>("el.cl", 1),
             (const uint32_t *)A.get<uint32_t>("el.n_sub", 1), n_slots, vf);
      nU = excl_scan_u64(E, vf, vp, n_slots, "vf");
      if (nU) {
        uint64_t *uk = A.get<uint64_t>("r.uk", nU), *uk2 = A.get<uint64_t>("r.uk2", nU);
        uint32_t *uv = A.get<uint32_t>("r.uv", nU);
        d_U = A.get<uint32_t>("r.U", nU);
        d_us = A.get<uint32_t>("r.us", nU);
        d_uoff = A.get<uint64_t>("r.uoff", nU);
        d_ulen = A.get<uint32_t>("r.ulen", nU);
        launch(st, k_sub_keys, n_slots, (const uint32_t *)A.get<uint32_t>("cl.cid", 1), (const uint64_t *)vf,
               (const uint64_t *)vp, (const uint32_t *)A.get<uint32_t>("el.h_sig", 1), n_slots, uk, uv);
        int cbits = 1;
        while (cbits < 32 && (1ull << cbits) <= er.n_clusters) ++cbits;
        sort_pairs(E, (const uint64_t *)uk, uk2, (const uint32_t *)uv, d_U, nU, 32 + cbits, "us");
        launch(st, k_sub_info, nU, (const uint64_t *)uk2, (const uint32_t *)d_U, (const uint64_t *)A.get<uint64_t>("el.h_off", 1),
               (const uint32_t *)A.get<uint32_t>("el.h_len", 1), nU, d_us, d_uoff, d_ulen, rank_of);
      }
    }
  }
  void round_apply() {
    RoundArgs ra{};
    ra.F = E->F;
    ra.a = sv[0]; ra.b = sv[1]; ra.c = sv[2];
    uint64_t *rcap[3];
    for (int q = 0; q < 3; ++q) rcap[q] = A.get<uint64_t>(part_name("r.cap", q, ""), n_st);
    ra.cap_a = rcap[0]; ra.cap_b = rcap[1]; ra.cap_c = rcap[2];
    ra.sub_of = r_sub_of;
    ra.rank_of = rank_of;
    ra.h_off = A.get<uint64_t>("el.h_off", 1);
    ra.h_len = A.get<uint32_t>("el.h_len", 1);
    ra.pk = P.pk;
    ra.pv = P.pv;
    ra.turn = A.get<int32_t>("r.turn", n_st);
    ra.touched = A.get<uint8_t>("r.touched", n_st);
    launch(st, k_round_count, n_st, ra);
    U3 *rcap3 = A.get<U3>("r.c3", n_st), *rsc3 = A.get<U3>("r.s3", n_st);
    launch(st, k_pack3, n_st, (const uint64_t *)rcap[0], (const uint64_t *)rcap[1], (const uint64_t *)rcap[2], n_st, rcap3);
    const U3 q3 = excl_scan_u3(E, rcap3, rsc3, n_st, "r");
    const uint64_t qt = q3.a + q3.b + q3.c;
    heap_reserve(qt);
    for (DRows *R : {&sv[0], &sv[1], &sv[2], &lv}) { R->key = heap_k; R->val = heap_v; }
    ra.a = sv[0]; ra.b = sv[1]; ra.c = sv[2];
    DRows out[3];
    for (int q = 0; q < 3; ++q) {
      out[q] = sv[q];
      out[q].off = A.get<uint64_t>(part_name("r.o", q, ".off"), n_st);
      out[q].len = A.get<uint32_t>(part_name("r.o", q, ".len"), n_st);
    }
    launch(st, k_set_offsets_u3, n_st, (const U3 *)rsc3, heap_top, heap_top + q3.a, heap_top + q3.a + q3.b, n_st, out[0].off,
           out[1].off, out[2].off, (const U3 *)nullptr, (const uint32_t *)nullptr);
    heap_top += qt;
    ra.c_base = heap_top - q3.c;
    ra.oa = out[0]; ra.ob = out[1]; ra.oc = out[2];
    ra.tmpk = A.get<uint32_t>("r.tmpk", 2 * (q3.c + 1));
    ra.tmpv = A.get<Fe>("r.tmpv", 2 * (q3.c + 1));
    MK.mark("count");
    {
      uint64_t *tfl = A.get<uint64_t>("r.tfl", n_st), *tfp = A.get<uint64_t>("r.tfp", n_st);
      uint32_t *tids = A.get<uint32_t>("r.touch_ids", n_st);
      launch(st, k_touch_flags, n_st, (const uint64_t *)rcap[2], n_st, tfl);
      ra.n_ids = excl_scan_u64(E, tfl, tfp, n_st, "tfl");
      if (ra.n_ids) launch(st, k_scatter_ids, n_st, (const uint64_t *)tfl, (const uint64_t *)tfp, n_st, tids);
      ra.ids = tids;
      HC(hipMemsetAsync(ra.turn, 0xff, 4 * n_st, st));
      HC(hipMemsetAsync(ra.touched, 0, n_st, st));
    }
    ra.bytes = A.get<unsigned long long>("r.bytes", 1);
    HC(hipMemsetAsync(ra.bytes, 0, 8, st));
    if (ra.n_ids) {
      FrameWaveArgs w{};
      w.fr.F = E->F;
      w.fr.sub_of = r_sub_of;
      w.fr.h_off = ra.h_off; w.fr.h_len = ra.h_len; w.fr.pk = ra.pk; w.fr.pv = ra.pv;
      for (int q = 0; q < 3; ++q) { w.in[q] = sv[q]; w.out[q] = out[q]; w.cap[q] = rcap[q]; }
      w.cap_by_row = 1;
      w.ids = ra.ids;
      w.n = ra.n_ids;
      w.big = A.get<uint32_t>("r.big", ra.n_ids);
      w.n_big = A.get<unsigned>("r.nbig", 2);
      w.round = 1;
      w.touched = ra.touched;
      w.turn_list = A.get<uint32_t>("r.turnlist", ra.n_ids);
      w.n_turn = w.n_big + 1;
      w.err = d_fw_err;
      w.bytes = ra.bytes;
      HC(hipMemsetAsync(w.n_big, 0, 8, st));
#ifdef RS_FWCLK
      w.clk = A.get<unsigned long long>("fw.clkr", 32);
      HC(hipMemsetAsync(w.clk, 0, 8 * 32, st));
#endif
      RoundArgs rb = ra, rt = ra;
      rb.rlist = w.big; rb.n_rlist = w.n_big;
      rt.rlist = w.turn_list; rt.n_rlist = w.n_turn;
      HC(hipEventRecord(E->ev[kEvFill0], st));
      launch_capped(st, k_frames_wave<1>, ra.n_ids, kFwBlocks, w);
      {
        unsigned nbig = 0;
        HC(hipMemcpyAsync(&nbig, w.n_big, 4, hipMemcpyDeviceToHost, st));
        HC(hipStreamSynchronize(st));
#ifdef RS_FWCLK
        if (g_prof_env) {
          unsigned long long c[32];
          HC(hipMemcpy(c, w.clk, sizeof c, hipMemcpyDeviceToHost));
          fprintf(stderr, "[rs-prof] round frames clocks (Mcycles summed over waves): groups %.1f entries %.1f terms %.1f "
                  "rank %.1f emit %.1f rows %.1f plan %.1f | batches %llu, wave total %.1f over %llu waves | emit: loads %.1f "
                  "values %.1f sync %.1f stores %.1f | %u rows over a batch of %llu\n", c[0] / 1e6, c[1] / 1e6, c[2] / 1e6,
                  c[3] / 1e6, c[5] / 1e6, c[6] / 1e6, c[7] / 1e6, c[8], c[9] / 1e6, c[10], c[16] / 1e6, c[17] / 1e6,
                  c[18] / 1e6, c[19] / 1e6, nbig, (unsigned long long)ra.n_ids);
        }
#endif
        if (nbig) {
          const uint64_t nseg = 3ull * nbig;
          uint64_t *xc = A.get<uint64_t>("x.cnt", nseg), *xo = A.get<uint64_t>("x.off", nseg + 1);
          launch(st, k_xrow_count, nseg, rb, nseg, xc);
          const uint64_t T = excl_scan_u64(E, xc, xo, nseg, "xrow");
          h2d(E, xo + nseg, &T, 8);
          if (T) {
            uint64_t *xk = A.get<uint64_t>("x.k", T), *xk2 = A.get<uint64_t>("x.k2", T);
            uint32_t *xi = A.get<uint32_t>("x.i", T), *xi2 = A.get<uint32_t>("x.i2", T);
            Fe *xv = A.get<Fe>("x.v", T);
            launch(st, k_xrow_expand, 64 * nseg, rb, nseg, (const uint64_t *)xo, xk, xv, xi);
            int sbits = 1;
            while (sbits < 32 && (1ull << sbits) <= nseg) ++sbits;
            sort_pairs(E, (const uint64_t *)xk, xk2, (const uint32_t *)xi, xi2, T, 32 + sbits, "xrow");
            launch(st, k_xrow_combine, 64 * nseg, rb, nseg, (const uint64_t *)xo, (const uint64_t *)xk2,
                   (const uint32_t *)xi2, (const Fe *)xv);
          } else {
            launch(st, k_xrow_combine, 64 * nseg, rb, nseg, (const uint64_t *)xo, (const uint64_t *)nullptr,
                   (const uint32_t *)nullptr, (const Fe *)nullptr);
          }
          rb.pre_expanded = 1;
        }
      }
      launch(st, k_round_fill, ra.n_ids, rb);
      launch(st, k_round_turn, ra.n_ids, rt);
      HC(hipEventRecord(E->ev[kEvFill1], st));
      if (g_prof_env) {
        unsigned nb[2] = {0, 0};
        HC(hipMemcpyAsync(nb, w.n_big, 8, hipMemcpyDeviceToHost, st));
        HC(hipStreamSynchronize(st));
        fprintf(stderr, "[rs-prof] round: %llu rows, %u over a wave batch, %u turn\n", (unsigned long long)ra.n_ids, nb[0], nb[1]);
      }
      float fm = 0;
      unsigned long long fb = 0;
      HC(hipMemcpyAsync(&fb, ra.bytes, 8, hipMemcpyDeviceToHost, st));
      HC(hipEventSynchronize(E->ev[kEvFill1]));
      HC(hipStreamSynchronize(st));
      HC(hipEventElapsedTime(&fm, E->ev[kEvFill0], E->ev[kEvFill1]));
      E->stats.round_fill_ms += fm;
      E->stats.round_fill_bytes += fb;
      E->stats.round_fill_launches++;
    }
    MK.mark("fill");
    if (env_flag("RS_DEBUG")) debug_check_round(E, ra, n_st, qt);
    launch(st, k_commit_round, n_st, (const uint8_t *)ra.touched, (const int32_t *)ra.turn, n_st, sv[0], sv[1], sv[2], out[0], out[1],
           out[2]);
    if (so_dirty) launch(st, k_or_u8, n_st, (const uint8_t *)ra.touched, n_st, so_dirty);
    snap_round(ra.touched, ra.turn);
    uint64_t *tf = A.get<uint64_t>("r.tf", n_st), *tp = A.get<uint64_t>("r.tp", n_st);
    launch(st, k_turn_flags, n_st, (const int32_t *)ra.turn, n_st, tf);
    uint64_t n_turn = excl_scan_u64(E, tf, tp, n_st, "tf");
    uint32_t *tids = A.get<uint32_t>("r.tids", n_turn);
    launch(st, k_scatter_ids, n_st, (const uint64_t *)tf, (const uint64_t *)tp, n_st, tids);
    std::vector<uint32_t> htids(n_turn);
    std::vector<int32_t> hturn(n_turn);
    if (n_turn) {
      int32_t *d_tt = A.get<int32_t>("r.tturn", n_turn);
      launch(st, k_gather_u32, n_turn, (const uint32_t *)ra.turn, (const uint32_t *)tids, (uint32_t *)d_tt, n_turn);
      HC(hipMemcpyAsync(htids.data(), tids, 4 * n_turn, hipMemcpyDeviceToHost, st));
      HC(hipMemcpyAsync(hturn.data(), d_tt, 4 * n_turn, hipMemcpyDeviceToHost, st));
      HC(hipStreamSynchronize(st));
      need_usig();
    }
    std::unordered_map<uint32_t, std::vector<uint32_t>> ext;
    {
      double Tq = now_ms();
      std::vector<uint32_t> qs;
      for (uint64_t i = 0; i < n_turn; ++i) qs.push_back(usig[hturn[i]]);
      std::sort(qs.begin(), qs.end());
      qs.erase(std::unique(qs.begin(), qs.end()), qs.end());
      query_initial(qs);
      ext = ML.resolve(qs, [this](const std::vector<uint32_t> &sigs) { query_initial(sigs); });
      E->stats.map_ms += now_ms() - Tq;
    }
    for (uint64_t ti = 0; ti < n_turn; ++ti) {
      const uint32_t r = htids[ti];
      int32_t q = hturn[ti];
      uint32_t from = usig[q];
      uint64_t pos = UINT64_MAX;
      const std::vector<uint32_t> &L0 = ML.minit[from];
      auto lb = std::lower_bound(L0.begin(), L0.end(), r);
      if (lb != L0.end() && *lb == r) pos = lb - L0.begin();
      if (pos == UINT64_MAX) {
        auto it = ext.find(from);
        if (it != ext.end())
          for (uint64_t t = 0; t < it->second.size(); ++t)
            if (it->second[t] == r) { pos = L0.size() + t; break; }
      }
      if (pos == UINT64_MAX) throw RsError(RS_E_INTERNAL, "substituted row missing from the signal map");
      turned.push_back({((uint64_t)q << 32) | (pos & 0xffffffffu), r});
    }
    std::sort(turned.begin(), turned.end());
    MK.mark("turned");
    if (env_flag("RS_DEBUG")) {
      std::vector<uint8_t> tch(n_st);
      HC(hipMemcpy(tch.data(), ra.touched, n_st, hipMemcpyDeviceToHost));
      uint64_t nt = 0;
      for (auto x : tch) nt += x;
      fprintf(stderr, "[rs-debug] round: nU=%llu touched=%llu turned=%llu:", (unsigned long long)nU,
              (unsigned long long)nt, (unsigned long long)n_turn);
      for (auto &t : turned) fprintf(stderr, " %u(q%llu)", t.second, (unsigned long long)(t.first >> 32));
      fprintf(stderr, "\n");
    }
  }
  uint64_t round_next() {
    if (nU) launch(st, k_unset_rank, nU, (const uint32_t *)d_us, nU, rank_of);
    std::vector<uint32_t> next_ids;
    {
      if (!turned.empty()) {
        std::vector<uint32_t> tid_(turned.size()), tlen(turned.size());
        for (size_t i = 0; i < turned.size(); ++i) tid_[i] = turned[i].second;
        uint32_t *d_t = A.get<uint32_t>("r.tid", tid_.size()), *d_tl = A.get<uint32_t>("r.tlen", tid_.size());
        h2d(E, d_t, tid_.data(), 4 * tid_.size());
        launch(st, k_gather_u32, tid_.size(), (const uint32_t *)sv[2].len, (const uint32_t *)d_t, d_tl, (uint64_t)tid_.size());
        HC(hipMemcpyAsync(tlen.data(), d_tl, 4 * tlen.size(), hipMemcpyDeviceToHost, st));
        HC(hipStreamSynchronize(st));
        for (size_t i = 0; i < turned.size(); ++i)
          if (tlen[i]) next_ids.push_back(turned[i].second);
      }
    }
    uint64_t nn = next_ids.size();
    if (nU) {
      launch(st, k_append_marks, nU, (const uint32_t *)d_us, (const uint64_t *)d_uoff, (const uint32_t *)d_ulen, nU,
             (const uint32_t *)P.pk, nlmap);
    }
    const bool another = nn > 0 && (no_rounds > 0 ? no_rounds - 1 : 0) > 0;
    if (another) {
      double Tq = now_ms();
      need_usig();
      MapLists::Batch B;
      B.from = usig;
      const size_t bi = ML.batches.size();
      const std::string bn = "ml." + std::to_string(bi);
      uint64_t *d_optr = A.get<uint64_t>(bn + ".ptr", nU + 1);
      uint64_t *d_len64 = A.get<uint64_t>(bn + ".len", nU + 1);
      launch(st, k_u32_to_u64, nU, (const uint32_t *)d_ulen, d_len64, nU);
      HC(hipMemsetAsync(d_len64 + nU, 0, 8, st));
      const uint64_t tot = excl_scan_u64(E, d_len64, d_optr, nU + 1, "mlb");
      uint32_t *d_keys = A.get<uint32_t>(bn + ".keys", std::max<uint64_t>(tot, 1));
      if (tot)
        launch(st, k_pool_keys, 64 * nU, (const uint64_t *)d_uoff, (const uint32_t *)d_ulen, (const uint64_t *)d_optr, nU,
               (const uint32_t *)P.pk, d_keys);
      B.load = [E = E, d_optr, d_keys, nU = nU, tot](MapLists::Batch &Bt) {
        Bt.ptr.resize(nU + 1);
        Bt.keys.resize(tot);
        HC(hipMemcpyAsync(Bt.ptr.data(), d_optr, 8 * (nU + 1), hipMemcpyDeviceToHost, E->st));
        if (tot) HC(hipMemcpyAsync(Bt.keys.data(), d_keys, 4 * tot, hipMemcpyDeviceToHost, E->st));
        HC(hipStreamSynchronize(E->st));
      };
      ML.add_batch(std::move(B));
      E->stats.map_ms += now_ms() - Tq;
    }
    MK.mark("appends2");
    lv.n = nn;
    lv.off = A.get<uint64_t>("lv.off", nn);
    lv.len = A.get<uint32_t>("lv.len", nn);
    lv.key = heap_k;
    lv.val = heap_v;
    if (nn) {
      uint32_t *d_ids = A.get<uint32_t>("lv.ids", nn);
      h2d(E, d_ids, next_ids.data(), 4 * nn);
      launch(st, k_view_rows, nn, (const uint64_t *)sv[2].off, (const uint32_t *)sv[2].len, (const uint32_t *)d_ids, nn, lv.off, lv.len);
    }
    if (!turned.empty()) {
      std::vector<uint32_t> all;
      for (auto &t : turned) all.push_back(t.second);
      uint32_t *d_all = A.get<uint32_t>("r.all", all.size());
      h2d(E, d_all, all.data(), 4 * all.size());
      launch(st, k_zero_c, all.size(), (const uint32_t *)d_all, (uint64_t)all.size(), sv[2].len);
    }
    HC(hipStreamSynchronize(st));
    if (env_flag("RS_DEBUG")) {
      for (uint64_t r = 0; r < std::min<uint64_t>(n_st, 24); ++r) {
        uint32_t la = 0, lb = 0, lc = 0;
        HC(hipMemcpy(&la, sv[0].len + r, 4, hipMemcpyDeviceToHost));
        HC(hipMemcpy(&lb, sv[1].len + r, 4, hipMemcpyDeviceToHost));
        HC(hipMemcpy(&lc, sv[2].len + r, 4, hipMemcpyDeviceToHost));
        std::vector<uint32_t> kk;
        std::vector<Fe> vv;
        d2h_row(E, sv[2], r, kk, vv);
        fprintf(stderr, "[rs-debug] storage %llu lens %u %u %u C:", (unsigned long long)r, la, lb, lc);
        for (size_t i = 0; i < kk.size(); ++i) fprintf(stderr, " %u:%llu", kk[i], (unsigned long long)ffrom_mont(E->F, vv[i]).l[0]);
        fprintf(stderr, "\n");
      }
    }
    return nn;
  }

  void assemble() {
    Tf = now_ms();
    const DRows lcv = lc.view(A);
    if (lv.n) launch(st, k_mark_keys, lv.n, lv, nlmap);
    if (lcv.n) launch(st, k_mark_keys, lcv.n, lcv, nlmap);
    HC(hipMemsetAsync(nlmap, 0, 1, st));
    uint32_t *kept = A.get<uint32_t>("fin.kept", S);
    uint64_t *kept64 = A.get<uint64_t>("fin.kept64", S);
    uint64_t *rank = A.get<uint64_t>("fin.rank", S);
    int32_t *l2w = A.get<int32_t>("fin.l2w", S);
    launch(st, k_kept, S, (const uint8_t *)d_deleted, (const uint8_t *)d_forb, (const uint8_t *)nlmap, kept, S);
    launch(st, k_u32_to_u64, S, (const uint32_t *)kept, kept64, S);
    E->n_wires = excl_scan_u64(E, kept64, rank, S, "kept");
    launch(st, k_l2w, S, (const uint32_t *)kept, (const uint64_t *)rank, l2w, S);
    {
      uint64_t lo = E->n_pub_out + 1, hi = E->n_pub_out + E->n_pub_in + E->n_priv_in;
      uint64_t del_in = 0;
      if (hi >= lo && lo < S) {
        uint64_t cnt = std::min<uint64_t>(hi, S - 1) - lo + 1;
        std::vector<uint32_t> k(cnt);
        HC(hipMemcpyAsync(k.data(), kept + lo, 4 * cnt, hipMemcpyDeviceToHost, st));
        HC(hipStreamSynchronize(st));
        for (uint32_t x : k) del_in += x ? 0 : 1;
      }
      E->npiw = E->n_priv_in - del_in;
    }
    {
      uint64_t *nef = A.get<uint64_t>("fin.nef", n_st), *nep = A.get<uint64_t>("fin.nep", n_st);
      uint64_t n_keep = 0;
      if (n_st) {
        launch(st, k_nonempty_flags, n_st, (const uint32_t *)sv[0].len, (const uint32_t *)sv[1].len, (const uint32_t *)sv[2].len, n_st, nef);
        n_keep = excl_scan_u64(E, nef, nep, n_st, "ne");
      }
      uint32_t *keep_ids = A.get<uint32_t>("fin.keep", n_keep);
      if (n_keep) launch(st, k_scatter_ids, n_st, (const uint64_t *)nef, (const uint64_t *)nep, n_st, keep_ids);
      const DRows xsrc[2] = {lv, lcv};
      const uint64_t zn = std::max<uint64_t>(lv.n, lcv.n);
      uint32_t *zero_len = A.get<uint32_t>("fin.zlen", zn);
      if (zn) HC(hipMemsetAsync(zero_len, 0, 4 * zn, st));
      uint32_t *x_ids[2];
      uint64_t n_x[2] = {0, 0}, x_at[2];
      for (int x = 0; x < 2; ++x) {
        const DRows &V = xsrc[x];
        x_ids[x] = A.get<uint32_t>(x ? "fin.lcids" : "fin.lvids", V.n);
        if (!V.n) continue;
        uint64_t *lf = A.get<uint64_t>("fin.xf", V.n), *lp = A.get<uint64_t>("fin.xp", V.n);
        launch(st, k_nonempty_flags, V.n, (const uint32_t *)zero_len, (const uint32_t *)zero_len, (const uint32_t *)V.len, V.n, lf);
        n_x[x] = excl_scan_u64(E, lf, lp, V.n, "xf");
        launch(st, k_scatter_ids, V.n, (const uint64_t *)lf, (const uint64_t *)lp, V.n, x_ids[x]);
      }
      x_at[0] = n_keep;
      x_at[1] = n_keep + n_x[0];
      const uint64_t n_out = n_keep + n_x[0] + n_x[1];
      if (n_keep > n_st || n_x[0] > lv.n || n_x[1] > lcv.n) throw RsError(RS_E_INTERNAL, "final assembly: row counts out of range");
      E->out_n_dev = n_out;
      const DRows *parts[3] = {&sv[0], &sv[1], &sv[2]};
      const char *nm[3] = {"out.a", "out.b", "out.c"};
      Comm *CMf = E->comm.get();
      const bool shard = E->snap_on && CMf && CMf->world > 1;
      uint64_t k_lo = 0, k_hi = n_keep;
      bool with_x = true;
      if (shard) {
        uint64_t kr[2] = {0, 0};
        if (n_keep) {
          uint64_t *d_kr = A.get<uint64_t>("fin.krange", 2);
          launch(st, k_keep_range, 2, (const uint32_t *)keep_ids, n_keep, (const uint32_t *)st_ids, E->nl_lo, E->nl_hi, d_kr);
          HC(hipMemcpyAsync(kr, d_kr, 16, hipMemcpyDeviceToHost, st));
          HC(hipStreamSynchronize(st));
        }
        k_lo = kr[0];
        k_hi = std::max(kr[0], kr[1]);
        with_x = CMf->rank == CMf->world - 1;
      }
      E->sh_klo = k_lo;
      E->sh_khi = k_hi;
      const uint64_t own = k_hi - k_lo;
      const uint32_t *own_ids = keep_ids + k_lo;
      const uint64_t xl_at[2] = {own, own + (with_x ? n_x[0] : 0)};
      const uint64_t xl_n[2] = {with_x ? n_x[0] : 0, with_x ? n_x[1] : 0};
      const uint64_t m_loc = own + xl_n[0] + xl_n[1];
      for (int q = 0; q < 3; ++q) {
        uint64_t *lens = A.get<uint64_t>(std::string(nm[q]) + ".lens", n_out + 1);
        uint64_t *ptr = A.get<uint64_t>(std::string(nm[q]) + ".ptr", n_out + 1);
        if (n_keep) launch(st, k_row_lens, n_keep, *parts[q], (const uint32_t *)keep_ids, n_keep, lens);
        DRows xq[2];
        for (int x = 0; x < 2; ++x) {
          xq[x] = xsrc[x];
          if (q < 2) xq[x].len = zero_len;
          if (n_x[x]) launch(st, k_row_lens, n_x[x], xq[x], (const uint32_t *)x_ids[x], n_x[x], lens + x_at[x]);
          E->fin_xq[x][q] = xq[x];
        }
        HC(hipMemsetAsync(lens + n_out, 0, 8, st));
        uint64_t tot = excl_scan_u64(E, lens, ptr, n_out + 1, nm[q]);
        E->out_nnz[q] = tot;
        E->fin_parts[q] = *parts[q];
        if (!E->snap_on) continue;
        uint64_t *late = A.get<uint64_t>(std::string(nm[q]) + ".late", m_loc + 1);
        uint64_t *lptr = A.get<uint64_t>(std::string(nm[q]) + ".lptr", m_loc + 1);
        if (own) launch(st, k_out_late_lens, own, *parts[q], own_ids, own, (const uint32_t *)st_ids, (const uint8_t *)so_early,
                        (const uint8_t *)so_dirty, late);
        if (xl_n[0]) launch(st, k_row_lens, xl_n[0], xq[0], (const uint32_t *)x_ids[0], xl_n[0], late + xl_at[0]);
        if (xl_n[1]) launch(st, k_lc_late_lens, xl_n[1], xq[1], (const uint32_t *)x_ids[1], xl_n[1], E->lc_snap_n, late + xl_at[1]);
        HC(hipMemsetAsync(late + m_loc, 0, 8, st));
        const uint64_t L = excl_scan_u64(E, late, lptr, m_loc + 1, "late");
        const uint64_t base = E->snap_e[q], ext = base + L;
        E->out_ext[q] = ext;
        uint64_t *beg = A.get<uint64_t>(std::string(nm[q]) + ".beg", m_loc + 1);
        uint64_t *end = A.get<uint64_t>(std::string(nm[q]) + ".end", m_loc + 1);

        if (own) launch(st, k_out_extent, own, *parts[q], own_ids, own, (const uint32_t *)st_ids, (const uint8_t *)so_early,
                        (const uint8_t *)so_dirty, (const U3 *)so_eoff, q, base, (const uint64_t *)lptr, beg, end);
        if (xl_n[0])
          launch(st, k_out_extent, xl_n[0], xq[0], (const uint32_t *)x_ids[0], xl_n[0], (const uint32_t *)nullptr, (const uint8_t *)nullptr,
                 (const uint8_t *)nullptr, (const U3 *)nullptr, q, base, (const uint64_t *)(lptr + xl_at[0]), beg + xl_at[0], end + xl_at[0]);
        if (xl_n[1])
          launch(st, k_lc_extent, xl_n[1], xq[1], (const uint32_t *)x_ids[1], xl_n[1], E->lc_snap_n, E->lc_snap_base, q, base,
                 (const uint64_t *)(lptr + xl_at[1]), beg + xl_at[1], end + xl_at[1]);
        launch(st, k_set_u64, 1, beg + m_loc, ext);
        {
          uint32_t *len32 = A.get<uint32_t>(std::string(nm[q]) + ".len32", m_loc + 1);
          uint64_t *jf = A.get<uint64_t>(std::string(nm[q]) + ".jf", m_loc + 1);
          uint64_t *jpos = A.get<uint64_t>(std::string(nm[q]) + ".jpos", m_loc + 1);
          uint64_t nj = 0;
          if (m_loc) {
            launch(st, k_out_jumps, m_loc, (const uint64_t *)beg, (const uint64_t *)end, m_loc, shard ? 1 : 0, len32, jf);
            nj = excl_scan_u64(E, jf, jpos, m_loc, "jump");
          }
          uint64_t *jtab = A.get<uint64_t>(std::string(nm[q]) + ".jtab", nj + 1);
          if (nj) launch(st, k_out_jtab, m_loc, (const uint64_t *)beg, (const uint64_t *)jf, (const uint64_t *)jpos, m_loc, (uint64_t)0, jtab);
          E->out_njump[q] = nj;
          if (shard) (void)A.get<uint64_t>(std::string(nm[q]) + ".jtabx", nj + 1);
        }
        const std::string xc = std::string(nm[q]) + ".xcol", xv = std::string(nm[q]) + ".xval";
        if (A.cap_bytes(xc) < 4 * ext || A.cap_bytes(xv) < 32 * ext) snap_join(E);
        A.grow_keep<uint32_t>(xc, ext, base, E->stc, st);
        A.grow_keep<uint64_t>(xv, 4 * ext, 4 * base, E->stc, st);
        uint32_t *col = A.get<uint32_t>(xc, ext);
        uint64_t *val = A.get<uint64_t>(xv, 4 * ext);
        E->kg[2].run(st, 30 * (own + xl_n[0] + xl_n[1]) + 72 * L, [&] {
          if (own) launch(st, k_gather_late, own, E->F, *parts[q], own_ids, own, (const uint32_t *)st_ids, (const uint8_t *)so_early,
                          (const uint8_t *)so_dirty, (const uint64_t *)lptr, col + base, val + 4 * base);
          if (xl_n[0])
            launch(st, k_gather_late, xl_n[0], E->F, xq[0], (const uint32_t *)x_ids[0], xl_n[0], (const uint32_t *)nullptr,
                   (const uint8_t *)nullptr, (const uint8_t *)nullptr, (const uint64_t *)(lptr + xl_at[0]), col + base, val + 4 * base);
          if (xl_n[1])
            launch(st, k_lc_gather_late, xl_n[1], E->F, xq[1], (const uint32_t *)x_ids[1], xl_n[1], E->lc_snap_n,
                   (const uint64_t *)(lptr + xl_at[1]), col + base, val + 4 * base);
        });
      }
      if (shard) {
        uint64_t over = 0;
        for (int q = 0; q < 3; ++q) over |= E->out_ext[q] > E->sh_cap[q];
        if (CMf->max_u64(over, st)) {
          snap_join(E);
          for (int q = 0; q < 3; ++q) E->sh_cap[q] = CMf->max_u64(E->out_ext[q] + E->out_ext[q] / 4 + 65536, st);
          E->sh_ent = CMf->shared_host(0, sh_ent_bytes(E), st);
          if (!E->sh_ent) throw RsError(RS_E_RCCL, "no shared host memory for the sharded result");
          E->sh_full = true;
        }
      }
      E->fin_keep = n_keep;
      E->fin_keep_ids = keep_ids;
      for (int x = 0; x < 2; ++x) {
        E->fin_xn[x] = n_x[x];
        E->fin_x_ids[x] = x_ids[x];
      }
      E->fin_gen = A.gen;
      if (!E->snap_on) ensure_csr(E);
    }
  }

  void finish() {
    load_wait_all(E);
    int err = 0, fw_err = 0;
    HC(hipMemcpyAsync(&err, d_err, 4, hipMemcpyDeviceToHost, st));
    HC(hipMemcpyAsync(&fw_err, d_fw_err, 4, hipMemcpyDeviceToHost, st));
    HC(hipStreamSynchronize(st));
    if (err) throw RsError(RS_E_INVALID, "input rejected by the device checks (code " + std::to_string(err) + ")");
    if (fw_err) throw RsError(RS_E_INTERNAL, "frames batch over its bounds (code " + std::to_string(fw_err) + ")");
    E->stats.final_ms = now_ms() - Tf;
    E->stats.total_ms = now_ms() - T0;
    if (g_prof_env) {
      size_t fr = 0, tot = 0;
      if (hipMemGetInfo(&fr, &tot) == hipSuccess)
        fprintf(stderr, "[rs-prof] device memory in use after the run: %.1f of %.1f GB (heap %.1f GB)\n", (tot - fr) / 1e9, tot / 1e9,
                36e-9 * E->heap_cap);
      std::vector<std::pair<size_t, std::string>> big;
      size_t sum = 0;
      for (auto &kv : A.bufs) {
        big.push_back({kv.second.cap, kv.first});
        sum += kv.second.cap;
      }
      std::sort(big.rbegin(), big.rend());
      fprintf(stderr, "[rs-prof] arena %.1f GB in %zu buffers; largest:", sum / 1e9, big.size());
      for (size_t i = 0; i < big.size() && i < 16; ++i) fprintf(stderr, " %s %.2f", big[i].second.c_str(), big[i].first / 1e9);
      fprintf(stderr, "\n");
    }
    E->stats.h2d_wait_ms = E->h2d_wait_ms;
    E->kg[0].collect(E->stats.check_ms, E->stats.check_bytes, E->stats.check_launches);
    E->kg[1].collect(E->stats.ragged_ms, E->stats.ragged_bytes, E->stats.ragged_launches);
    E->kg[2].collect(E->stats.gather_ms, E->stats.gather_bytes, E->stats.gather_launches);
    {
      const uint64_t z_in = E->ce.nnz + E->eq.nnz + E->lin.nnz + E->na.nnz + E->nb.nnz + E->nc.nnz;
      const uint64_t r_in = E->ce.n + E->eq.n + E->lin.n + E->na.n;
      const uint64_t z_out = E->out_nnz[0] + E->out_nnz[1] + E->out_nnz[2], r_out = E->out_n_dev;
      const rs_stats &s = E->stats;
      E->stats.alg_bytes = s.elim_bytes + s.big_main_bytes + s.big_finish_bytes + s.apply_bytes + s.round_fill_bytes +
                           s.cluster_bytes + 36 * (z_in + z_out) + 8 * (r_in + r_out) + 8 * S;
    }
    E->have_result = true;
  }
};

static void engine_run(rs_engine *E, const rs_flags *fl) {
  Run R(E, fl);
  R.init();
  R.eq_simplification();
  R.constant_eq();
  R.setup_non_linear();
  R.linear_round1();
  R.non_linear_frames();
  R.rounds();
  R.assemble();
  R.finish();
}
```

Before: 234.9 million.

## Fuse final assembly into combined kernels and batch host readbacks

Final assembly is restructured. Kept-wire counting, the deleted-input count and the non-empty flags for all three row groups now run in combined kernels, and their totals come back in one pinned readback. This replaces several sync-and-copy round trips, including a host-side loop over the input-wire range. In the single-device snapshot path, a fused assembly builds layout, jump tables and late gathers over all output rows with U3 scans, and the per-part CSR row pointers are deferred to ensure_csr. The late snapshot pass now runs over a compacted id list instead of all nonlinear rows, and profiling counters for the result stream are added. The cost is more complex kernels and an extra code path that must stay bit-exact.

Result: faster. 239.2 million, median of 6 (+1.8%).

```diff
diff --git a/circom_cvm_amd/csrc/engine.hip b/circom_cvm_amd/csrc/engine.hip
--- a/circom_cvm_amd/csrc/engine.hip
+++ b/circom_cvm_amd/csrc/engine.hip
@@ -296,6 +296,8 @@
   };
   hipEvent_t ev_snapq[6] = {};
   hipEvent_t ev_snaph[3] = {};
+  double asm_t0_ms = 0, asm_end_ms = 0, snap_last_ms = 0;
+  int snap_open = 0, asm_open = 0;
   hipEvent_t ev_fh[2] = {};
   hipEvent_t ev_nlc = nullptr;
   std::mutex snap_m;
@@ -318,6 +320,7 @@
   KGroup kg[3];
   int snap_rc = 0;
   bool csr_ready = false;
+  bool csr_rows_ready = false;
   DRows fin_parts[3] = {}, fin_xq[2][3] = {};
   uint64_t out_njump[3] = {0, 0, 0};
   const uint32_t *fin_keep_ids = nullptr, *fin_x_ids[2] = {nullptr, nullptr};
@@ -648,6 +651,14 @@
   void *tmp = E->A.get<uint8_t>(std::string("scan.tmp.") + tag, tb);
   HC(rocprim::exclusive_scan(tmp, tb, in, out, (uint64_t)0, (size_t)n, rocprim::plus<uint64_t>(), s));
 }
+static void dev_scan_u3(rs_engine *E, const U3 *in, U3 *out, uint64_t n, hipStream_t s, const char *tag) {
+  if (!n) return;
+  size_t tb = 0;
+  const U3 zero{0, 0, 0};
+  HC(rocprim::exclusive_scan(nullptr, tb, in, out, zero, (size_t)n, U3Plus(), s));
+  void *tmp = E->A.get<uint8_t>(std::string("scan3.tmp.") + tag, tb);
+  HC(rocprim::exclusive_scan(tmp, tb, in, out, zero, (size_t)n, U3Plus(), s));
+}
 static void dev_scan_u32(rs_engine *E, const uint32_t *in, uint32_t *out, uint64_t n, hipStream_t s, const char *tag) {
   if (!n) return;
   size_t tb = 0;
@@ -719,16 +730,43 @@
     for (int t = 0; t < 4; ++t) { o[3 + t] = val ? val[p0].l[t] : 0; o[7 + t] = val ? val[p0 + 1].l[t] : 0; }
   }
 }
-__global__ void k_flag_linear(const uint32_t *la, const uint32_t *lb, uint64_t n, uint64_t *flag_lin, uint64_t *flag_nl) {
-  for (uint64_t i = gtid(); i < n; i += gstride()) {
-    bool lin = la[i] == 0 && lb[i] == 0;
-    flag_lin[i] = lin ? 1 : 0;
-    flag_nl[i] = lin ? 0 : 1;
-  }
-}
 __global__ void k_scatter_ids(const uint64_t *flag, const uint64_t *pos, uint64_t n, uint32_t *ids) {
   for (uint64_t i = gtid(); i < n; i += gstride())
     if (flag[i]) ids[pos[i]] = (uint32_t)i;
+}
+__global__ void k_flag_lin(const uint32_t *la, const uint32_t *lb, uint64_t n, uint64_t *flag_lin) {
+  for (uint64_t i = gtid(); i < n; i += gstride()) flag_lin[i] = (la[i] == 0 && lb[i] == 0) ? 1 : 0;
+}
+__global__ void k_split_ids(const uint64_t *flag_lin, const uint64_t *pos, uint64_t n, uint32_t *wl, uint32_t *st) {
+  for (uint64_t i = gtid(); i < n; i += gstride()) {
+    if (flag_lin[i]) wl[pos[i]] = (uint32_t)i;
+    else st[i - pos[i]] = (uint32_t)i;
+  }
+}
+__global__ void k_view_rows4(DRows a, DRows b, DRows c, const uint32_t *st_ids, uint64_t n_st, const uint32_t *wl_ids, uint64_t n_wl,
+                             DRows va, DRows vb, DRows vc, DRows lv) {
+  for (uint64_t i = gtid(); i < n_st + n_wl; i += gstride()) {
+    if (i < n_st) {
+      const uint32_t r = st_ids[i];
+      va.off[i] = a.off[r];
+      va.len[i] = a.len[r];
+      vb.off[i] = b.off[r];
+      vb.len[i] = b.len[r];
+      vc.off[i] = c.off[r];
+      vc.len[i] = c.len[r];
+    } else {
+      const uint32_t r = wl_ids[i - n_st];
+      lv.off[i - n_st] = c.off[r];
+      lv.len[i - n_st] = c.len[r];
+    }
+  }
+}
+__global__ void k_mark_keys3(DRows a, DRows b, DRows c, uint64_t n, uint8_t *bits) {
+  for (uint64_t r = gtid(); r < n; r += gstride()) {
+    for (uint32_t i = 0; i < a.len[r]; ++i) bits[a.key[a.off[r] + i]] = 1;
+    for (uint32_t i = 0; i < b.len[r]; ++i) bits[b.key[b.off[r] + i]] = 1;
+    for (uint32_t i = 0; i < c.len[r]; ++i) bits[c.key[c.off[r] + i]] = 1;
+  }
 }
 __global__ void k_set_rank(const uint32_t *sig, const int32_t *rank, uint64_t n, int32_t *rank_of) {
   for (uint64_t i = gtid(); i < n; i += gstride()) rank_of[sig[i]] = rank[i];
@@ -757,9 +795,6 @@
 }
 __global__ void k_zero_c(const uint32_t *ids, uint64_t n, uint32_t *clen) {
   for (uint64_t i = gtid(); i < n; i += gstride()) clen[ids[i]] = 0;
-}
-__global__ void k_nonempty_flags(const uint32_t *la, const uint32_t *lb, const uint32_t *lc, uint64_t n, uint64_t *flag) {
-  for (uint64_t i = gtid(); i < n; i += gstride()) flag[i] = (la[i] | lb[i] | lc[i]) ? 1 : 0;
 }
 
 __device__ inline bool d_has_key(const uint32_t *k, uint32_t n, uint32_t s) {
@@ -2194,6 +2229,7 @@
   E->snap_cv.notify_all();
   if (E->snap_thread.joinable()) E->snap_thread.join();
   E->snap_q.clear();
+  E->snap_open = 0;
 }
 static void snap_start(rs_engine *E);
 static void snap_push(rs_engine *E, const rs_engine::SnapJob &j) {
@@ -2201,6 +2237,7 @@
   {
     std::lock_guard<std::mutex> lk(E->snap_m);
     E->snap_q.push_back(j);
+    ++E->snap_open;
   }
   E->snap_cv.notify_all();
 }
@@ -2237,7 +2274,10 @@
       }
       if (g_prof_env) {
         if (hipStreamSynchronize(E->stx) != hipSuccess) E->snap_rc = RS_E_HIP;
-        prof_ms += now_ms() - tj;
+        std::lock_guard<std::mutex> lk(E->snap_m);
+        E->snap_last_ms = now_ms();
+        --E->snap_open;
+        prof_ms += E->snap_last_ms - tj;
         prof_b += j.bytes;
       }
     }
@@ -2285,6 +2325,18 @@
   hipStream_t st = E->st;
   const char *nm[3] = {"out.a", "out.b", "out.c"};
   const uint64_t n_keep = E->fin_keep, n_out = E->out_n_dev;
+  for (int q = 0; q < 3 && !E->csr_rows_ready; ++q) {
+    uint64_t *lens = A.get<uint64_t>(std::string(nm[q]) + ".lens", n_out + 1);
+    uint64_t *ptr = A.get<uint64_t>(std::string(nm[q]) + ".ptr", n_out + 1);
+    if (n_keep) launch(st, k_row_lens, n_keep, E->fin_parts[q], E->fin_keep_ids, n_keep, lens);
+    for (int x = 0; x < 2; ++x) {
+      const uint64_t o = n_keep + (x ? E->fin_xn[0] : 0);
+      if (E->fin_xn[x]) launch(st, k_row_lens, E->fin_xn[x], E->fin_xq[x][q], E->fin_x_ids[x], E->fin_xn[x], lens + o);
+    }
+    HC(hipMemsetAsync(lens + n_out, 0, 8, st));
+    dev_scan_u64(E, lens, ptr, n_out + 1, st, nm[q]);
+  }
+  E->csr_rows_ready = true;
   for (int q = 0; q < 3; ++q) {
     const uint64_t tot = E->out_nnz[q];
     const uint64_t *ptr = A.get<uint64_t>(std::string(nm[q]) + ".ptr", n_out + 1);
diff --git a/circom_cvm_amd/csrc/kernels.hpp b/circom_cvm_amd/csrc/kernels.hpp
--- a/circom_cvm_amd/csrc/kernels.hpp
+++ b/circom_cvm_amd/csrc/kernels.hpp
@@ -3330,9 +3330,6 @@
 __global__ void k_mark_list(const uint32_t *sig, uint64_t n, uint8_t *bits) {
   for (uint64_t i = gtid(); i < n; i += gstride()) bits[sig[i]] = 1;
 }
-__global__ void k_kept(const uint8_t *deleted, const uint8_t *forb, const uint8_t *nlmap, uint32_t *kept, uint64_t S) {
-  for (uint64_t s = gtid(); s < S; s += gstride()) kept[s] = (!deleted[s] && (forb[s] || nlmap[s])) ? 1u : 0u;
-}
 __global__ void k_l2w(const uint32_t *kept, const uint64_t *rank, int32_t *l2w, uint64_t S) {
   for (uint64_t s = gtid(); s < S; s += gstride()) l2w[s] = kept[s] ? (int32_t)rank[s] : -1;
 }
diff --git a/circom_cvm_amd/csrc/output.hpp b/circom_cvm_amd/csrc/output.hpp
--- a/circom_cvm_amd/csrc/output.hpp
+++ b/circom_cvm_amd/csrc/output.hpp
@@ -28,19 +28,21 @@
   }
 }
 
-__global__ void k_snap_lens2(DRows a, DRows b, DRows c, const uint64_t *late, uint64_t n, U3 *elen, ViewCopy vc) {
-  for (uint64_t i = gtid(); i < n; i += gstride()) {
-    const bool ok = late[i] && (a.len[i] | b.len[i]) != 0;
-    elen[i] = ok ? U3{a.len[i], b.len[i], c.len[i]} : U3{0, 0, 0};
-    if (ok) view_copy(vc, a, b, c, i, a.len[i], b.len[i], c.len[i]);
-  }
-}
-__global__ void k_snap_mark2(const uint64_t *late, const U3 *elen, const U3 *eoff2, U3 base, uint64_t n, uint8_t *early,
-                             U3 *eoff) {
-  for (uint64_t i = gtid(); i < n; i += gstride()) {
-    if (!late[i] || (elen[i].a | elen[i].b) == 0) continue;
-    early[i] = 1;
-    eoff[i] = U3{base.a + eoff2[i].a, base.b + eoff2[i].b, base.c + eoff2[i].c};
+__global__ void k_snap_lens2_l(DRows a, DRows b, DRows c, const uint32_t *ids, uint64_t n, U3 *elen, ViewCopy vc) {
+  for (uint64_t i = gtid(); i < n; i += gstride()) {
+    const uint32_t r = ids[i];
+    const uint32_t la = a.len[r], lb = b.len[r], lc = c.len[r];
+    const bool ok = (la | lb) != 0;
+    elen[i] = ok ? U3{la, lb, lc} : U3{0, 0, 0};
+    if (ok) view_copy(vc, a, b, c, r, la, lb, lc);
+  }
+}
+__global__ void k_snap_mark2_l(const uint32_t *ids, const U3 *elen, const U3 *eoff2, U3 base, uint64_t n, uint8_t *early, U3 *eoff) {
+  for (uint64_t i = gtid(); i < n; i += gstride()) {
+    if ((elen[i].a | elen[i].b) == 0) continue;
+    const uint32_t r = ids[i];
+    early[r] = 1;
+    eoff[r] = U3{base.a + eoff2[i].a, base.b + eoff2[i].b, base.c + eoff2[i].c};
   }
 }
 
@@ -77,6 +79,24 @@
   }
 }
 
+__global__ void k_snap_gather_l(FieldP F, DRows R, const uint32_t *ids, const U3 *elen, const U3 *eoff, int q, uint64_t n,
+                                uint32_t *col, uint64_t *val) {
+  for (uint64_t i = gtid(); i < n; i += gstride()) {
+    if ((elen[i].a | elen[i].b) == 0) continue;
+    const uint32_t r = ids[i];
+    const uint64_t o = u3_sel(eoff[r], q), s = R.off[r];
+    const uint32_t len = R.len[r];
+    for (uint32_t t = 0; t < len; ++t) {
+      col[o + t] = R.key[s + t];
+      const Fe c = ffrom_mont(F, R.val[s + t]);
+      val[4 * (o + t) + 0] = c.l[0];
+      val[4 * (o + t) + 1] = c.l[1];
+      val[4 * (o + t) + 2] = c.l[2];
+      val[4 * (o + t) + 3] = c.l[3];
+    }
+  }
+}
+
 __global__ void k_snap_lens_round(DRows a, DRows b, DRows c, const uint8_t *touched, const int32_t *turn, const uint32_t *nl_of,
                                   const uint8_t *early, uint64_t n, U3 *elen, ViewCopy vc) {
   for (uint64_t r = gtid(); r < n; r += gstride()) {
@@ -235,3 +255,171 @@
   for (uint64_t i = gtid(); i < m; i += gstride())
     if (jf[i]) jtab[jpos[i]] = beg[i] + add;
 }
+
+struct OutRows {
+  DRows st[3];
+  DRows xl, xc;
+  const uint32_t *keep, *xl_ids, *xc_ids;
+  uint64_t n_keep, n_xl, n_xc;
+  const uint32_t *nl_of;
+  const uint8_t *early, *dirty;
+  const U3 *eoff;
+  uint64_t lc_snap_n, lc_snap_base;
+  U3 base;
+};
+__device__ __forceinline__ void out_row(const OutRows &R, uint64_t i, uint32_t (&len)[3], bool (&reuse)[3], uint64_t (&at)[3]) {
+  if (i < R.n_keep) {
+    const uint32_t r = R.keep[i];
+    const bool ru = d_reused(R.early, R.dirty, R.nl_of, r);
+    U3 e{0, 0, 0};
+    if (ru) e = R.eoff[R.nl_of[r]];
+#pragma unroll
+    for (int q = 0; q < 3; ++q) {
+      len[q] = R.st[q].len[r];
+      reuse[q] = ru;
+      at[q] = u3_sel(e, q);
+    }
+    return;
+  }
+  len[0] = len[1] = 0;
+  reuse[0] = reuse[1] = reuse[2] = false;
+  at[0] = at[1] = at[2] = 0;
+  if (i < R.n_keep + R.n_xl) {
+    len[2] = R.xl.len[R.xl_ids[i - R.n_keep]];
+  } else {
+    const uint32_t r = R.xc_ids[i - R.n_keep - R.n_xl];
+    len[2] = R.xc.len[r];
+    if (r < R.lc_snap_n) {
+      reuse[2] = true;
+      at[2] = R.lc_snap_base + R.xc.off[r];
+    }
+  }
+}
+__global__ void k_out_late3(OutRows R, uint64_t m, U3 *late, unsigned long long *nnz) {
+  unsigned long long s[3] = {0, 0, 0};
+  for (uint64_t i = gtid(); i < m; i += gstride()) {
+    uint32_t len[3];
+    bool reuse[3];
+    uint64_t at[3];
+    out_row(R, i, len, reuse, at);
+    late[i] = U3{reuse[0] ? 0u : len[0], reuse[1] ? 0u : len[1], reuse[2] ? 0u : len[2]};
+    s[0] += len[0];
+    s[1] += len[1];
+    s[2] += len[2];
+  }
+  wave_atomic_add(nnz + 0, s[0]);
+  wave_atomic_add(nnz + 1, s[1]);
+  wave_atomic_add(nnz + 2, s[2]);
+}
+__global__ void k_out_layout3(OutRows R, uint64_t m, const U3 *lptr, uint32_t *len_a, uint32_t *len_b, uint32_t *len_c, U3 *beg,
+                              U3 *jf) {
+  for (uint64_t i = gtid(); i < m; i += gstride()) {
+    uint32_t len[3], plen[3] = {0, 0, 0};
+    bool reuse[3], preuse[3] = {false, false, false};
+    uint64_t at[3], pat[3] = {0, 0, 0};
+    out_row(R, i, len, reuse, at);
+    const U3 lp = lptr[i];
+    U3 plp{0, 0, 0};
+    if (i) {
+      out_row(R, i - 1, plen, preuse, pat);
+      plp = lptr[i - 1];
+    }
+    uint64_t b[3], j[3];
+#pragma unroll
+    for (int q = 0; q < 3; ++q) {
+      b[q] = reuse[q] ? at[q] : u3_sel(R.base, q) + u3_sel(lp, q);
+      const uint64_t pend = (preuse[q] ? pat[q] : u3_sel(R.base, q) + u3_sel(plp, q)) + plen[q];
+      j[q] = (i == 0 ? b[q] != 0 : b[q] != pend) ? 1 : 0;
+    }
+    len_a[i] = len[0] | (j[0] ? RS_ROW_JUMP : 0u);
+    len_b[i] = len[1] | (j[1] ? RS_ROW_JUMP : 0u);
+    len_c[i] = len[2] | (j[2] ? RS_ROW_JUMP : 0u);
+    beg[i] = U3{b[0], b[1], b[2]};
+    jf[i] = U3{j[0], j[1], j[2]};
+  }
+}
+__global__ void k_out_jtab3(const U3 *beg, const U3 *jf, const U3 *jpos, uint64_t m, uint64_t *ja, uint64_t *jb, uint64_t *jc) {
+  for (uint64_t i = gtid(); i < m; i += gstride()) {
+    const U3 f = jf[i];
+    if (f.a) ja[jpos[i].a] = beg[i].a;
+    if (f.b) jb[jpos[i].b] = beg[i].b;
+    if (f.c) jc[jpos[i].c] = beg[i].c;
+  }
+}
+__global__ void k_gather_late_all(FieldP F, OutRows R, int q, uint64_t m, const U3 *lptr, uint32_t *col, uint64_t *val) {
+  for (uint64_t i = gtid(); i < m; i += gstride()) {
+    const uint32_t *key;
+    const Fe *v;
+    uint64_t s;
+    uint32_t len;
+    if (i < R.n_keep) {
+      const uint32_t r = R.keep[i];
+      if (d_reused(R.early, R.dirty, R.nl_of, r)) continue;
+      const DRows &P = R.st[q];
+      key = P.key, v = P.val, s = P.off[r], len = P.len[r];
+    } else {
+      if (q != 2) continue;
+      const bool l = i < R.n_keep + R.n_xl;
+      const DRows &P = l ? R.xl : R.xc;
+      const uint32_t r = l ? R.xl_ids[i - R.n_keep] : R.xc_ids[i - R.n_keep - R.n_xl];
+      if (!l && r < R.lc_snap_n) continue;
+      key = P.key, v = P.val, s = P.off[r], len = P.len[r];
+    }
+    const uint64_t o = u3_sel(lptr[i], q);
+    for (uint32_t t = 0; t < len; ++t) {
+      col[o + t] = key[s + t];
+      const Fe c = ffrom_mont(F, v[s + t]);
+      val[4 * (o + t) + 0] = c.l[0];
+      val[4 * (o + t) + 1] = c.l[1];
+      val[4 * (o + t) + 2] = c.l[2];
+      val[4 * (o + t) + 3] = c.l[3];
+    }
+  }
+}
+__global__ void k_scan_total_u64(const uint64_t *in, const uint64_t *out, uint64_t n, uint64_t *dst) {
+  if (gtid() == 0) *dst = n ? in[n - 1] + out[n - 1] : 0;
+}
+__global__ void k_scan_total_u3(const U3 *in, const U3 *out, uint64_t n, uint64_t *dst) {
+  if (gtid() != 0) return;
+  const U3 z{0, 0, 0};
+  const U3 a = n ? in[n - 1] : z, b = n ? out[n - 1] : z;
+  dst[0] = a.a + b.a;
+  dst[1] = a.b + b.b;
+  dst[2] = a.c + b.c;
+}
+__global__ void k_kept_count(const uint8_t *deleted, const uint8_t *forb, const uint8_t *nlmap, uint32_t *kept, uint64_t *kept64,
+                             uint64_t S, uint64_t lo, uint64_t hi, unsigned long long *n_del) {
+  unsigned long long d = 0;
+  for (uint64_t s = gtid(); s < S; s += gstride()) {
+    const uint32_t k = (!deleted[s] && (forb[s] || nlmap[s])) ? 1u : 0u;
+    kept[s] = k;
+    kept64[s] = k;
+    if (s >= lo && s <= hi && !k) ++d;
+  }
+  wave_atomic_add(n_del, d);
+}
+__global__ void k_nonempty_flags3(DRows a, DRows b, DRows c, uint64_t n_st, DRows xl, DRows xc, uint64_t *f_st, uint64_t *f_xl,
+                                  uint64_t *f_xc) {
+  const uint64_t n = n_st + xl.n + xc.n;
+  for (uint64_t i = gtid(); i < n; i += gstride()) {
+    if (i < n_st) f_st[i] = (a.len[i] | b.len[i] | c.len[i]) ? 1 : 0;
+    else if (i < n_st + xl.n) f_xl[i - n_st] = xl.len[i - n_st] ? 1 : 0;
+    else f_xc[i - n_st - xl.n] = xc.len[i - n_st - xl.n] ? 1 : 0;
+  }
+}
+__global__ void k_scatter_ids3(const uint64_t *f_st, const uint64_t *p_st, uint64_t n_st, const uint64_t *f_xl, const uint64_t *p_xl,
+                               uint64_t n_xl, const uint64_t *f_xc, const uint64_t *p_xc, uint64_t n_xc, uint32_t *i_st, uint32_t *i_xl,
+                               uint32_t *i_xc) {
+  const uint64_t n = n_st + n_xl + n_xc;
+  for (uint64_t i = gtid(); i < n; i += gstride()) {
+    if (i < n_st) {
+      if (f_st[i]) i_st[p_st[i]] = (uint32_t)i;
+    } else if (i < n_st + n_xl) {
+      const uint64_t k = i - n_st;
+      if (f_xl[k]) i_xl[p_xl[k]] = (uint32_t)k;
+    } else {
+      const uint64_t k = i - n_st - n_xl;
+      if (f_xc[k]) i_xc[p_xc[k]] = (uint32_t)k;
+    }
+  }
+}
diff --git a/circom_cvm_amd/csrc/run.hpp b/circom_cvm_amd/csrc/run.hpp
--- a/circom_cvm_amd/csrc/run.hpp
+++ b/circom_cvm_amd/csrc/run.hpp
@@ -537,24 +537,24 @@
   void snap_take2() {
     if (!E->snap_on || !nl_late || !n_late || (E->comm && E->comm->world > 1)) return;
     HC(hipStreamWaitEvent(st, E->ev_snap, 0));
-    U3 *elen = A.get<U3>("so.elen", n_nl), *eoff2 = A.get<U3>("so.eoff2", n_nl);
+    U3 *elen = A.get<U3>("so.elen2", n_late), *eoff2 = A.get<U3>("so.eoff2", n_late);
     DRows cp[3];
     ViewCopy vc;
     snap_views(stor, "so2.", cp, vc);
-    launch(st, k_snap_lens2, n_nl, stor[0], stor[1], stor[2], (const uint64_t *)nl_late, n_nl, elen, vc);
-    const U3 et = excl_scan_u3(E, elen, eoff2, n_nl, "so2");
+    launch(st, k_snap_lens2_l, n_late, stor[0], stor[1], stor[2], (const uint32_t *)nl_lids, n_late, elen, vc);
+    const U3 et = excl_scan_u3(E, elen, eoff2, n_late, "so2");
     const uint64_t e2[3] = {et.a, et.b, et.c};
     for (int q = 0; q < 3; ++q) E->snap_hint[q] = std::max(E->snap_hint[q], E->snap_e[q] + e2[q]);
     for (int q = 0; q < 3; ++q)
       if (E->snap_e[q] + e2[q] > E->snap_cap[q]) return;
-    launch(st, k_snap_mark2, n_nl, (const uint64_t *)nl_late, (const U3 *)elen, (const U3 *)eoff2,
-           U3{E->snap_e[0], E->snap_e[1], E->snap_e[2]}, n_nl, so_early, so_eoff);
+    launch(st, k_snap_mark2_l, n_late, (const uint32_t *)nl_lids, (const U3 *)elen, (const U3 *)eoff2,
+           U3{E->snap_e[0], E->snap_e[1], E->snap_e[2]}, n_late, so_early, so_eoff);
     HC(hipEventRecord(E->ev_snap0, st));
     HC(hipStreamWaitEvent(E->stc, E->ev_snap0, 0));
     snap_tail(e2, E->ev_snapq + 3, "second snapshot", "", [&](int q, uint32_t *col, uint64_t *val, uint64_t) {
-      E->kg[2].run(E->stc, 21 * n_nl + 72 * e2[q], [&] {
-        launch(E->stc, k_snap_gather, n_nl, E->F, cp[q], (const uint8_t *)so_early, (const U3 *)so_eoff, q, n_nl, col, val,
-               (const uint64_t *)nl_late, (uint64_t)0);
+      E->kg[2].run(E->stc, 28 * n_late + 72 * e2[q], [&] {
+        launch(E->stc, k_snap_gather_l, n_late, E->F, cp[q], (const uint32_t *)nl_lids, (const U3 *)elen, (const U3 *)so_eoff, q, n_late,
+               col, val);
       });
     });
   }
@@ -748,16 +748,22 @@
     HC(hipMemcpyAsync(&bytes, d_bytes, 8, hipMemcpyDeviceToHost, st));
     st_ids = A.get<uint32_t>("st.ids", n_nl);
     wl_ids = A.get<uint32_t>("wl.ids", n_nl);
+    uint64_t *h_wl = (uint64_t *)pin_get(E, kPinRead, kPinRb);
     if (n_nl) {
-      uint64_t *fl_lin = A.get<uint64_t>("fl.lin", n_nl), *fl_nl = A.get<uint64_t>("fl.nl", n_nl);
-      uint64_t *p_lin = A.get<uint64_t>("fl.plin", n_nl), *p_nl = A.get<uint64_t>("fl.pnl", n_nl);
-      launch(st, k_flag_linear, n_nl, (const uint32_t *)stor[0].len, (const uint32_t *)stor[1].len, n_nl, fl_lin, fl_nl);
-      n_wl = excl_scan_u64(E, fl_lin, p_lin, n_nl, "fl");
-      n_st = excl_scan_u64(E, fl_nl, p_nl, n_nl, "fn");
-      launch(st, k_scatter_ids, n_nl, (const uint64_t *)fl_lin, (const uint64_t *)p_lin, n_nl, wl_ids);
-      launch(st, k_scatter_ids, n_nl, (const uint64_t *)fl_nl, (const uint64_t *)p_nl, n_nl, st_ids);
+      uint64_t *fl_lin = A.get<uint64_t>("fl.lin", n_nl), *p_lin = A.get<uint64_t>("fl.plin", n_nl);
+      uint64_t *d_wl = A.get<uint64_t>("fl.tot", 1);
+      launch(st, k_flag_lin, n_nl, (const uint32_t *)stor[0].len, (const uint32_t *)stor[1].len, n_nl, fl_lin);
+      dev_scan_u64(E, fl_lin, p_lin, n_nl, st, "fl");
+      launch(st, k_scan_total_u64, 1, (const uint64_t *)fl_lin, (const uint64_t *)p_lin, n_nl, d_wl);
+      launch(st, k_split_ids, n_nl, (const uint64_t *)fl_lin, (const uint64_t *)p_lin, n_nl, wl_ids, st_ids);
+      HC(hipMemcpyAsync(h_wl, d_wl, 8, hipMemcpyDeviceToHost, st));
     }
     HC(hipStreamSynchronize(st));
+    if (n_nl) {
+      n_wl = h_wl[0];
+      if (n_wl > n_nl) throw RsError(RS_E_INTERNAL, "non-linear split: row counts out of range");
+      n_st = n_nl - n_wl;
+    }
     E->stats.apply_bytes += bytes;
     if (no_rounds > 0) no_rounds--;
 
@@ -768,20 +774,17 @@
       sv[q].off = A.get<uint64_t>(part_name("sv.", q, ".off"), n_st);
       sv[q].len = A.get<uint32_t>(part_name("sv.", q, ".len"), n_st);
     }
-    if (n_st)
-      for (int q = 0; q < 3; ++q)
-        launch(st, k_view_rows, n_st, (const uint64_t *)stor[q].off, (const uint32_t *)stor[q].len, (const uint32_t *)st_ids, n_st,
-               sv[q].off, sv[q].len);
-    nlmap = A.get<uint8_t>("nlmap", S);
-    HC(hipMemsetAsync(nlmap, 0, S, st));
-    if (n_st)
-      for (const DRows &R : sv) launch(st, k_mark_keys, n_st, R, nlmap);
     lv.n = n_wl;
     lv.key = heap_k;
     lv.val = heap_v;
     lv.off = A.get<uint64_t>("lv.off", n_wl);
     lv.len = A.get<uint32_t>("lv.len", n_wl);
-    if (n_wl) launch(st, k_view_rows, n_wl, (const uint64_t *)stor[2].off, (const uint32_t *)stor[2].len, (const uint32_t *)wl_ids, n_wl, lv.off, lv.len);
+    if (n_st + n_wl)
+      launch(st, k_view_rows4, n_st + n_wl, stor[0], stor[1], stor[2], (const uint32_t *)st_ids, n_st, (const uint32_t *)wl_ids, n_wl,
+             sv[0], sv[1], sv[2], lv);
+    nlmap = A.get<uint8_t>("nlmap", S);
+    HC(hipMemsetAsync(nlmap, 0, S, st));
+    if (n_st) launch(st, k_mark_keys3, n_st, sv[0], sv[1], sv[2], n_st, nlmap);
     HC(hipStreamSynchronize(st));
     E->stats.subst_ms += now_ms() - Ts;
     E->stats.nl_ms += now_ms() - Ts;
@@ -969,7 +972,10 @@
     launch(st, k_round_count, n_st, ra);
     U3 *rcap3 = A.get<U3>("r.c3", n_st), *rsc3 = A.get<U3>("r.s3", n_st);
     launch(st, k_pack3, n_st, (const uint64_t *)rcap[0], (const uint64_t *)rcap[1], (const uint64_t *)rcap[2], n_st, rcap3);
-    const U3 q3 = excl_scan_u3(E, rcap3, rsc3, n_st, "r");
+    uint64_t *tfl = A.get<uint64_t>("r.tfl", n_st), *tfp = A.get<uint64_t>("r.tfp", n_st);
+    launch(st, k_touch_flags, n_st, (const uint64_t *)rcap[2], n_st, tfl);
+    dev_scan_u64(E, tfl, tfp, n_st, st, "tfl");
+    const U3 q3 = n_st ? excl_scan_u3(E, rcap3, rsc3, n_st, "r", tfl + n_st - 1, tfp + n_st - 1, &ra.n_ids) : U3{0, 0, 0};
     const uint64_t qt = q3.a + q3.b + q3.c;
     heap_reserve(qt);
     for (DRows *R : {&sv[0], &sv[1], &sv[2], &lv}) { R->key = heap_k; R->val = heap_v; }
@@ -989,10 +995,8 @@
     ra.tmpv = A.get<Fe>("r.tmpv", 2 * (q3.c + 1));
     MK.mark("count");
     {
-      uint64_t *tfl = A.get<uint64_t>("r.tfl", n_st), *tfp = A.get<uint64_t>("r.tfp", n_st);
       uint32_t *tids = A.get<uint32_t>("r.touch_ids", n_st);
-      launch(st, k_touch_flags, n_st, (const uint64_t *)rcap[2], n_st, tfl);
-      ra.n_ids = excl_scan_u64(E, tfl, tfp, n_st, "tfl");
+      if (ra.n_ids > n_st) throw RsError(RS_E_INTERNAL, "round: touched rows out of range");
       if (ra.n_ids) launch(st, k_scatter_ids, n_st, (const uint64_t *)tfl, (const uint64_t *)tfp, n_st, tids);
       ra.ids = tids;
       HC(hipMemsetAsync(ra.turn, 0xff, 4 * n_st, st));
@@ -1230,8 +1234,82 @@
     return nn;
   }
 
+  void assemble_fused(const DRows &lcv, const uint32_t *keep_ids, uint32_t *const (&x_ids)[2], uint64_t n_keep, const uint64_t (&n_x)[2],
+                      uint32_t *zero_len, uint64_t *tots, uint64_t *h_tots) {
+    const char *nm[3] = {"out.a", "out.b", "out.c"};
+    const uint64_t m = n_keep + n_x[0] + n_x[1];
+    OutRows R{};
+    for (int q = 0; q < 3; ++q) {
+      R.st[q] = sv[q];
+      E->fin_parts[q] = sv[q];
+      E->fin_xq[0][q] = lv;
+      E->fin_xq[1][q] = lcv;
+      if (q < 2) E->fin_xq[0][q].len = E->fin_xq[1][q].len = zero_len;
+    }
+    R.xl = lv;
+    R.xc = lcv;
+    R.keep = keep_ids;
+    R.xl_ids = x_ids[0];
+    R.xc_ids = x_ids[1];
+    R.n_keep = n_keep;
+    R.n_xl = n_x[0];
+    R.n_xc = n_x[1];
+    R.nl_of = st_ids;
+    R.early = so_early;
+    R.dirty = so_dirty;
+    R.eoff = so_eoff;
+    R.lc_snap_n = E->lc_snap_n;
+    R.lc_snap_base = E->lc_snap_base;
+    R.base = U3{E->snap_e[0], E->snap_e[1], E->snap_e[2]};
+    U3 *late = A.get<U3>("fin.late3", m), *lptr = A.get<U3>("fin.lptr3", m), *beg = A.get<U3>("fin.beg3", m);
+    U3 *jf = A.get<U3>("fin.jf3", m), *jpos = A.get<U3>("fin.jpos3", m);
+    uint32_t *len32[3];
+    for (int q = 0; q < 3; ++q) len32[q] = A.get<uint32_t>(std::string(nm[q]) + ".len32", m + 1);
+    if (m) {
+      launch_capped(st, k_out_late3, m, 1024, R, m, late, (unsigned long long *)(tots + 11));
+      dev_scan_u3(E, late, lptr, m, st, "late");
+      launch(st, k_scan_total_u3, 1, (const U3 *)late, (const U3 *)lptr, m, tots + 5);
+      launch(st, k_out_layout3, m, R, m, (const U3 *)lptr, len32[0], len32[1], len32[2], beg, jf);
+      dev_scan_u3(E, jf, jpos, m, st, "jump");
+      launch(st, k_scan_total_u3, 1, (const U3 *)jf, (const U3 *)jpos, m, tots + 8);
+    }
+    HC(hipMemcpyAsync(h_tots + 5, tots + 5, 8 * 9, hipMemcpyDeviceToHost, st));
+    HC(hipStreamSynchronize(st));
+    uint64_t *jtab[3];
+    bool any_j = false;
+    for (int q = 0; q < 3; ++q) {
+      const uint64_t L = h_tots[5 + q], nj = h_tots[8 + q];
+      if (nj > m) throw RsError(RS_E_INTERNAL, "final assembly: jump count out of range");
+      E->out_ext[q] = E->snap_e[q] + L;
+      E->out_njump[q] = nj;
+      E->out_nnz[q] = h_tots[11 + q];
+      jtab[q] = A.get<uint64_t>(std::string(nm[q]) + ".jtab", nj + 1);
+      any_j |= nj != 0;
+    }
+    if (any_j) launch(st, k_out_jtab3, m, (const U3 *)beg, (const U3 *)jf, (const U3 *)jpos, m, jtab[0], jtab[1], jtab[2]);
+    for (int q = 0; q < 3; ++q) {
+      const uint64_t base = E->snap_e[q], ext = E->out_ext[q], L = ext - base;
+      const std::string xc = std::string(nm[q]) + ".xcol", xv = std::string(nm[q]) + ".xval";
+      if (A.cap_bytes(xc) < 4 * ext || A.cap_bytes(xv) < 32 * ext) snap_join(E);
+      A.grow_keep<uint32_t>(xc, ext, base, E->stc, st);
+      A.grow_keep<uint64_t>(xv, 4 * ext, 4 * base, E->stc, st);
+      uint32_t *col = A.get<uint32_t>(xc, ext);
+      uint64_t *val = A.get<uint64_t>(xv, 4 * ext);
+      if (!L) continue;
+      E->kg[2].run(st, 30 * m + 72 * L, [&] {
+        launch(st, k_gather_late_all, m, E->F, R, q, m, (const U3 *)lptr, col + base, val + 4 * base);
+      });
+    }
+  }
+
   void assemble() {
     Tf = now_ms();
+    if (g_prof_env) {
+      HC(hipStreamSynchronize(st));
+      std::lock_guard<std::mutex> lk(E->snap_m);
+      E->asm_t0_ms = now_ms();
+      E->asm_open = E->snap_open;
+    }
     const DRows lcv = lc.view(A);
     if (lv.n) launch(st, k_mark_keys, lv.n, lv, nlmap);
     if (lcv.n) launch(st, k_mark_keys, lcv.n, lcv, nlmap);
@@ -1240,55 +1318,55 @@
     uint64_t *kept64 = A.get<uint64_t>("fin.kept64", S);
     uint64_t *rank = A.get<uint64_t>("fin.rank", S);
     int32_t *l2w = A.get<int32_t>("fin.l2w", S);
-    launch(st, k_kept, S, (const uint8_t *)d_deleted, (const uint8_t *)d_forb, (const uint8_t *)nlmap, kept, S);
-    launch(st, k_u32_to_u64, S, (const uint32_t *)kept, kept64, S);
-    E->n_wires = excl_scan_u64(E, kept64, rank, S, "kept");
+    uint64_t *tots = A.get<uint64_t>("fin.tots", 14);
+    uint64_t *h_tots = (uint64_t *)pin_get(E, kPinRead, kPinRb);
+    HC(hipMemsetAsync(tots, 0, 8 * 14, st));
+    launch(st, k_kept_count, S, (const uint8_t *)d_deleted, (const uint8_t *)d_forb, (const uint8_t *)nlmap, kept, kept64, S,
+           E->n_pub_out + 1, E->n_pub_out + E->n_pub_in + E->n_priv_in, (unsigned long long *)(tots + 1));
+    dev_scan_u64(E, kept64, rank, S, st, "kept");
+    launch(st, k_scan_total_u64, 1, (const uint64_t *)kept64, (const uint64_t *)rank, S, tots + 0);
     launch(st, k_l2w, S, (const uint32_t *)kept, (const uint64_t *)rank, l2w, S);
+    Comm *CMf = E->comm.get();
+    const bool shard = E->snap_on && CMf && CMf->world > 1;
+    const bool fused = E->snap_on && !shard;
     {
-      uint64_t lo = E->n_pub_out + 1, hi = E->n_pub_out + E->n_pub_in + E->n_priv_in;
-      uint64_t del_in = 0;
-      if (hi >= lo && lo < S) {
-        uint64_t cnt = std::min<uint64_t>(hi, S - 1) - lo + 1;
-        std::vector<uint32_t> k(cnt);
-        HC(hipMemcpyAsync(k.data(), kept + lo, 4 * cnt, hipMemcpyDeviceToHost, st));
-        HC(hipStreamSynchronize(st));
-        for (uint32_t x : k) del_in += x ? 0 : 1;
-      }
-      E->npiw = E->n_priv_in - del_in;
-    }
-    {
+      const DRows xsrc[2] = {lv, lcv};
       uint64_t *nef = A.get<uint64_t>("fin.nef", n_st), *nep = A.get<uint64_t>("fin.nep", n_st);
-      uint64_t n_keep = 0;
-      if (n_st) {
-        launch(st, k_nonempty_flags, n_st, (const uint32_t *)sv[0].len, (const uint32_t *)sv[1].len, (const uint32_t *)sv[2].len, n_st, nef);
-        n_keep = excl_scan_u64(E, nef, nep, n_st, "ne");
-      }
+      uint64_t *xf[2], *xp[2];
+      for (int x = 0; x < 2; ++x) {
+        xf[x] = A.get<uint64_t>(x ? "fin.xf1" : "fin.xf0", xsrc[x].n);
+        xp[x] = A.get<uint64_t>(x ? "fin.xp1" : "fin.xp0", xsrc[x].n);
+      }
+      const uint64_t n_cand = n_st + lv.n + lcv.n;
+      if (n_cand) launch(st, k_nonempty_flags3, n_cand, sv[0], sv[1], sv[2], n_st, lv, lcv, nef, xf[0], xf[1]);
+      dev_scan_u64(E, nef, nep, n_st, st, "ne");
+      launch(st, k_scan_total_u64, 1, (const uint64_t *)nef, (const uint64_t *)nep, n_st, tots + 2);
+      for (int x = 0; x < 2; ++x) {
+        dev_scan_u64(E, xf[x], xp[x], xsrc[x].n, st, x ? "xf1" : "xf0");
+        launch(st, k_scan_total_u64, 1, (const uint64_t *)xf[x], (const uint64_t *)xp[x], xsrc[x].n, tots + 3 + x);
+      }
+      HC(hipMemcpyAsync(h_tots, tots, 8 * 5, hipMemcpyDeviceToHost, st));
+      HC(hipStreamSynchronize(st));
+      E->n_wires = h_tots[0];
+      E->npiw = E->n_priv_in - h_tots[1];
+      const uint64_t n_keep = h_tots[2];
+      uint64_t n_x[2] = {h_tots[3], h_tots[4]}, x_at[2];
       uint32_t *keep_ids = A.get<uint32_t>("fin.keep", n_keep);
-      if (n_keep) launch(st, k_scatter_ids, n_st, (const uint64_t *)nef, (const uint64_t *)nep, n_st, keep_ids);
-      const DRows xsrc[2] = {lv, lcv};
+      uint32_t *x_ids[2] = {A.get<uint32_t>("fin.lvids", lv.n), A.get<uint32_t>("fin.lcids", lcv.n)};
+      if (n_keep > n_st || n_x[0] > lv.n || n_x[1] > lcv.n) throw RsError(RS_E_INTERNAL, "final assembly: row counts out of range");
+      if (n_cand)
+        launch(st, k_scatter_ids3, n_cand, (const uint64_t *)nef, (const uint64_t *)nep, n_st, (const uint64_t *)xf[0],
+               (const uint64_t *)xp[0], lv.n, (const uint64_t *)xf[1], (const uint64_t *)xp[1], lcv.n, keep_ids, x_ids[0], x_ids[1]);
       const uint64_t zn = std::max<uint64_t>(lv.n, lcv.n);
       uint32_t *zero_len = A.get<uint32_t>("fin.zlen", zn);
       if (zn) HC(hipMemsetAsync(zero_len, 0, 4 * zn, st));
-      uint32_t *x_ids[2];
-      uint64_t n_x[2] = {0, 0}, x_at[2];
-      for (int x = 0; x < 2; ++x) {
-        const DRows &V = xsrc[x];
-        x_ids[x] = A.get<uint32_t>(x ? "fin.lcids" : "fin.lvids", V.n);
-        if (!V.n) continue;
-        uint64_t *lf = A.get<uint64_t>("fin.xf", V.n), *lp = A.get<uint64_t>("fin.xp", V.n);
-        launch(st, k_nonempty_flags, V.n, (const uint32_t *)zero_len, (const uint32_t *)zero_len, (const uint32_t *)V.len, V.n, lf);
-        n_x[x] = excl_scan_u64(E, lf, lp, V.n, "xf");
-        launch(st, k_scatter_ids, V.n, (const uint64_t *)lf, (const uint64_t *)lp, V.n, x_ids[x]);
-      }
       x_at[0] = n_keep;
       x_at[1] = n_keep + n_x[0];
       const uint64_t n_out = n_keep + n_x[0] + n_x[1];
-      if (n_keep > n_st || n_x[0] > lv.n || n_x[1] > lcv.n) throw RsError(RS_E_INTERNAL, "final assembly: row counts out of range");
       E->out_n_dev = n_out;
       const DRows *parts[3] = {&sv[0], &sv[1], &sv[2]};
       const char *nm[3] = {"out.a", "out.b", "out.c"};
-      Comm *CMf = E->comm.get();
-      const bool shard = E->snap_on && CMf && CMf->world > 1;
+      if (fused) assemble_fused(lcv, keep_ids, x_ids, n_keep, n_x, zero_len, tots, h_tots);
       uint64_t k_lo = 0, k_hi = n_keep;
       bool with_x = true;
       if (shard) {
@@ -1310,7 +1388,8 @@
       const uint64_t xl_at[2] = {own, own + (with_x ? n_x[0] : 0)};
       const uint64_t xl_n[2] = {with_x ? n_x[0] : 0, with_x ? n_x[1] : 0};
       const uint64_t m_loc = own + xl_n[0] + xl_n[1];
-      for (int q = 0; q < 3; ++q) {
+      E->csr_rows_ready = !fused;
+      for (int q = 0; q < 3 && !fused; ++q) {
         uint64_t *lens = A.get<uint64_t>(std::string(nm[q]) + ".lens", n_out + 1);
         uint64_t *ptr = A.get<uint64_t>(std::string(nm[q]) + ".ptr", n_out + 1);
         if (n_keep) launch(st, k_row_lens, n_keep, *parts[q], (const uint32_t *)keep_ids, n_keep, lens);
@@ -1399,6 +1478,14 @@
       E->fin_gen = A.gen;
       if (!E->snap_on) ensure_csr(E);
     }
+    if (g_prof_env) {
+      HC(hipStreamSynchronize(st));
+      std::lock_guard<std::mutex> lk(E->snap_m);
+      E->asm_end_ms = now_ms();
+      fprintf(stderr, "[rs-prof] final assembly: %.2f ms (device done); the result stream had %d copies unfinished at its start, "
+                      "%d at its end (its last copy was done %.2f ms before the end)\n",
+              E->asm_end_ms - E->asm_t0_ms, E->asm_open, E->snap_open, E->asm_end_ms - E->snap_last_ms);
+    }
   }
 
   void finish() {
```
